# heimrih/polar_code

Hardware: AMD Instinct MI355X
Metric: decoded frames/sec, P(128,64)+CRC24 SCL L=8 @ Eb/N0=5 dB; FER match (higher is better)
Workload: dtype f64

## Files before the change

include/polar_scl.h:

```cpp
#ifndef POLAR_SCL_H
#define POLAR_SCL_H

#include <stdint.h>

#ifdef __cplusplus
extern "C" {
#endif

#define PSCL_ABI_VERSION 1

#define PSCL_OK 0
#define PSCL_EINVAL -1
#define PSCL_EDEVICE -2
#define PSCL_ENOMEM -3
#define PSCL_EPRUNED -4
#define PSCL_EUNSUP -5

#define PSCL_MAX_N 1024
#define PSCL_MAX_L 32
#define PSCL_MAX_CRC 32
#define PSCL_WORDS(K) (((K) + 63) / 64)

#define PSCL_FLAG_CRC_PASS 0x80u
#define PSCL_FLAG_IDX_MASK 0x3fu

#define PSCL_CNT_FRAMES 0
#define PSCL_CNT_FRAME_ERR 1
#define PSCL_CNT_BIT_ERR 2
#define PSCL_CNT_PAYLOAD_ERR 3
#define PSCL_CNT_PAYLOAD_BIT 4
#define PSCL_CNT_RETRIES 5
#define PSCL_CNT_ESCALATED 6
#define PSCL_NCOUNT 8

typedef struct pscl_handle pscl_handle;

const char* pscl_last_error(void);

int pscl_abi_version(void);

const char* pscl_build_hash(void);

int pscl_device_count(void);

int pscl_create(pscl_handle** out, int device, int N, const int32_t* info_set, int K, int L,
                uint64_t crc_poly);
int pscl_destroy(pscl_handle* h);

int pscl_set_stream(pscl_handle* h, void* hip_stream);
void* pscl_get_stream(pscl_handle* h);
int pscl_sync(pscl_handle* h);

int pscl_decode(pscl_handle* h, const double* llr, int64_t B, const int8_t* forced, int32_t* n_paths,
                int8_t* best_bits, uint8_t* crc_pass, int32_t* best_idx, double* metrics, int8_t* cands,
                double* info_llrs);

int pscl_sc_decode(pscl_handle* h, const double* llr, int64_t B, int8_t* bits);

int pscl_decode_device(pscl_handle* h, const double* d_llr, int64_t B, const uint64_t* d_force,
                       uint64_t* d_best, uint8_t* d_flags, double* d_metrics, uint64_t* d_cands,
                       double* d_info_llrs, const uint64_t* d_ref, int k_payload, int64_t* d_counters);

int pscl_channel_device(pscl_handle* h, uint64_t seed, uint32_t stream_id, double ebno_db, double rate,
                        int k_payload, int64_t frame0, int64_t B, double* d_llr, uint64_t* d_msg);

int pscl_uncoded_device(pscl_handle* h, uint64_t seed, uint32_t stream_id, double ebno_db, int k_payload,
                        int64_t frame0, int64_t B, int64_t* d_counters);

int pscl_set_rate_match(pscl_handle* h, int E);

int pscl_path_llrs_device(pscl_handle* h, const double* d_llr, int64_t B, const uint64_t* d_bits, double* d_out);

int pscl_set_beta(pscl_handle* h, const double* beta);

int pscl_dlscl_device(pscl_handle* h, const double* d_llr, int64_t B, int retries, uint64_t* d_best,
                      uint8_t* d_flags, int32_t* d_attempts, int32_t* d_tried, int tried_stride,
                      const uint64_t* d_ref, int k_payload, int64_t* d_counters_scl, int64_t* d_counters_dl);

int pscl_adaptive_device(pscl_handle* h, const double* d_llr, int64_t B, uint64_t* d_best, uint8_t* d_flags,
                         uint8_t* d_stage, const uint64_t* d_ref, int k_payload, int64_t* d_counters,
                         int64_t* n_escalated);

int pscl_sc_device(pscl_handle* h, const double* d_llr, int64_t B, uint64_t* d_best, uint8_t* d_flags,
                   uint8_t* d_stage, const uint64_t* d_ref, int k_payload, int64_t* d_counters);
int pscl_escalate_device(pscl_handle* h, const double* d_llr, int64_t B, uint64_t* d_best, uint8_t* d_flags,
                         uint8_t* d_stage, const uint64_t* d_ref, int k_payload, int64_t* d_counters,
                         int64_t* n_escalated);

int pscl_adaptive_async_device(pscl_handle* h, const double* d_llr, int64_t B, uint64_t* d_best, uint8_t* d_flags,
                               uint8_t* d_stage, const uint64_t* d_ref, int k_payload, int64_t* d_counters,
                               int32_t* d_n_escalated);

int pscl_f32_available(pscl_handle* h);
int pscl_decode_device_f32(pscl_handle* h, const float* d_llr, int64_t B, uint64_t* d_best, uint8_t* d_flags,
                           const uint64_t* d_ref, int k_payload, int64_t* d_counters);
int pscl_sc_device_f32(pscl_handle* h, const float* d_llr, int64_t B, uint64_t* d_best, uint8_t* d_flags,
                       uint8_t* d_stage, const uint64_t* d_ref, int k_payload, int64_t* d_counters);
int pscl_escalate_device_f32(pscl_handle* h, const float* d_llr, int64_t B, uint64_t* d_best, uint8_t* d_flags,
                             uint8_t* d_stage, const uint64_t* d_ref, int k_payload, int64_t* d_counters,
                             int64_t* n_escalated);
int pscl_adaptive_async_device_f32(pscl_handle* h, const float* d_llr, int64_t B, uint64_t* d_best, uint8_t* d_flags,
                                   uint8_t* d_stage, const uint64_t* d_ref, int k_payload, int64_t* d_counters,
                                   int32_t* d_n_escalated);

int pscl_simulate_adaptive_device(pscl_handle* h, uint64_t seed, uint32_t stream_id, double ebno_db, double rate,
                                  int k_payload, int64_t frame0, int64_t B, int include_uncoded, int64_t* d_counters);
int pscl_simulate_adaptive(pscl_handle* h, uint64_t seed, uint32_t stream_id, double ebno_db, double rate,
                           int k_payload, int64_t frame0, int64_t B, int include_uncoded, int64_t* counters);

int pscl_adaptive_stats(pscl_handle* h, int64_t* screened, int64_t* exact, int64_t* host_waits, int reset);

int pscl_retry_device(pscl_handle* h, const double* d_llr, int64_t B, int retries, uint64_t* d_best, uint8_t* d_flags,
                      uint8_t* d_stage, int32_t* d_attempts, int32_t* d_tried, int tried_stride, const uint64_t* d_ref,
                      int k_payload, int64_t* d_counters_dl);

int pscl_adaptive_dlscl_device(pscl_handle* h, const double* d_llr, int64_t B, int retries, uint64_t* d_best,
                               uint8_t* d_flags, uint8_t* d_stage, int32_t* d_attempts, int32_t* d_tried,
                               int tried_stride, const uint64_t* d_ref, int k_payload, int64_t* d_counters,
                               int32_t* d_n_escalated);

int pscl_simulate_adaptive_dl_device(pscl_handle* h, uint64_t seed, uint32_t stream_id, double ebno_db, double rate,
                                     int k_payload, int64_t frame0, int64_t B, int retries, int include_uncoded,
                                     int64_t* d_counters);
int pscl_simulate_adaptive_dl(pscl_handle* h, uint64_t seed, uint32_t stream_id, double ebno_db, double rate,
                              int k_payload, int64_t frame0, int64_t B, int retries, int include_uncoded,
                              int64_t* counters);

int pscl_simulate(pscl_handle* h, uint64_t seed, uint32_t stream_id, double ebno_db, double rate, int k_payload,
                  int64_t frame0, int64_t B, int retries, int include_uncoded, int64_t* counters);

int pscl_simulate_device(pscl_handle* h, uint64_t seed, uint32_t stream_id, double ebno_db, double rate, int k_payload,
                         int64_t frame0, int64_t B, int retries, int include_uncoded, int64_t* d_counters);

int pscl_device_alloc(pscl_handle* h, void** d_ptr, int64_t bytes);
int pscl_device_free(pscl_handle* h, void* d_ptr);
int pscl_memcpy_htod(pscl_handle* h, void* d_dst, const void* src, int64_t bytes);
int pscl_memcpy_dtoh(pscl_handle* h, void* dst, const void* d_src, int64_t bytes);
int pscl_memset_device(pscl_handle* h, void* d_dst, int value, int64_t bytes);

int pscl_set_screening(pscl_handle* h, int enable);

int pscl_screening_count(pscl_handle* h, int64_t* count);

int pscl_set_pipelined(pscl_handle* h, int enable);
int pscl_join(pscl_handle* h);

#define PSCL_TUNE_DL_SCREEN 1
#define PSCL_TUNE_DL_CHUNKS 2
#define PSCL_TUNE_DL_SPLIT 3
#define PSCL_TUNE_SIDE_PRIORITY 4
#define PSCL_TUNE_POST_GRID 5
#define PSCL_TUNE_RETRY_WPG 6
#define PSCL_TUNE_DL_LANE 7
#define PSCL_TUNE_DL_SCREEN_MIN 8
#define PSCL_TUNE_DL_RETRY_LANE 9
#define PSCL_TUNE_POST_PAIRS 10
#define PSCL_TUNE_DL_STREAMS 11
#define PSCL_TUNE_TX_FUSED 12
#define PSCL_TUNE_DL_FUSED_POST 13
#define PSCL_TUNE_POST_EPW 14
#define PSCL_TUNE_LANE_EXACT 15
#define PSCL_TUNE_DL_WARM_APX 16
#define PSCL_TUNE_DL_TAIL 17
#define PSCL_TUNE_ADAPT_GRID 18
#define PSCL_TUNE_COUNT 19
int pscl_set_tuning(pscl_handle* h, int knob, int64_t value);

int pscl_softplus_tails_device(pscl_handle* h, const double* d_v, int64_t n, double* d_exact, double* d_apx);

int pscl_tail_abs_scan_device(pscl_handle* h, uint32_t lo, uint32_t hi, uint64_t* d_out);

int pscl_tail2_scan_device(pscl_handle* h, uint32_t lo, uint32_t hi, uint64_t* d_out);

int pscl_timing_enable(pscl_handle* h, int enable);
int pscl_timing_read(pscl_handle* h, int64_t* launches, double* total_ms);
int pscl_timing_read_split(pscl_handle* h, int64_t* main_launches, double* main_ms, int64_t* side_launches,
                           double* side_ms);

int pscl_host_stats(pscl_handle* h, double* call_ms, double* wait_ms, int64_t* calls, int reset);

int pscl_path_stats(pscl_handle* h, int64_t* fused_post_rounds, int64_t* post_rounds, int64_t* fused_tx_blocks,
                    int64_t* post_epw4_launches, int64_t* lane_exact_launches);

int pscl_decode_cpu(int N, const int32_t* info_set, int K, int L, uint64_t crc_poly, const double* llr, int64_t B,
                    const int8_t* forced, int32_t* n_paths, int8_t* best_bits, uint8_t* crc_pass, int32_t* best_idx,
                    double* metrics, int8_t* cands, double* info_llrs, int threads);

int pscl_decode_adaptive_cpu(int N, const int32_t* info_set, int K, int L, uint64_t crc_poly, const double* llr,
                             int64_t B, int8_t* best_bits, uint8_t* crc_pass, int32_t* best_idx, uint8_t* stage,
                             int threads);

int pscl_launch_info(pscl_handle* h, int64_t B, int* waves_per_wg, int64_t* grid, int* lds_bytes);

#ifdef __cplusplus
}
#endif

#endif
```

polar_code_amd/_native.py:

```python
from __future__ import annotations

import ctypes as C
import functools
import importlib.util
import os
import sys
import threading
from pathlib import Path

import numpy as np

LIB_PATH = Path(os.environ.get("PSCL_LIB_PATH") or Path(__file__).resolve().parent / "libpolar_mi355x.so")

PSCL_OK = 0
PSCL_EINVAL = -1
PSCL_EDEVICE = -2
PSCL_ENOMEM = -3
PSCL_EPRUNED = -4
PSCL_EUNSUP = -5
PSCL_MAX_N = 1024
PSCL_REPLAY_MAX_N = 128
PSCL_MAX_L = 32
PSCL_FLAG_CRC_PASS = 0x80
PSCL_FLAG_IDX_MASK = 0x3F
PSCL_NCOUNT = 8
CNT_FRAMES, CNT_FRAME_ERR, CNT_BIT_ERR, CNT_PAYLOAD_ERR, CNT_PAYLOAD_BIT, CNT_RETRIES, CNT_ESCALATED = range(7)

EXPORTS = (
    "pscl_last_error", "pscl_abi_version", "pscl_device_count", "pscl_create", "pscl_destroy",
    "pscl_set_stream", "pscl_get_stream", "pscl_sync", "pscl_decode", "pscl_sc_decode",
    "pscl_decode_device", "pscl_channel_device", "pscl_device_alloc", "pscl_device_free",
    "pscl_memcpy_htod", "pscl_memcpy_dtoh", "pscl_memset_device", "pscl_timing_enable",
    "pscl_timing_read", "pscl_launch_info", "pscl_set_rate_match", "pscl_set_beta", "pscl_dlscl_device",
    "pscl_path_llrs_device", "pscl_uncoded_device", "pscl_simulate", "pscl_set_screening", "pscl_build_hash",
    "pscl_screening_count", "pscl_softplus_tails_device", "pscl_set_pipelined", "pscl_join",
    "pscl_tail_abs_scan_device", "pscl_tail2_scan_device", "pscl_set_tuning", "pscl_timing_read_split", "pscl_decode_cpu",
    "pscl_host_stats", "pscl_path_stats",
    "pscl_simulate_device", "pscl_adaptive_device", "pscl_decode_adaptive_cpu",
    "pscl_sc_device", "pscl_escalate_device",
    "pscl_adaptive_async_device", "pscl_simulate_adaptive", "pscl_simulate_adaptive_device", "pscl_adaptive_stats",
    "pscl_retry_device", "pscl_adaptive_dlscl_device", "pscl_simulate_adaptive_dl", "pscl_simulate_adaptive_dl_device",
    "pscl_f32_available", "pscl_decode_device_f32", "pscl_sc_device_f32", "pscl_escalate_device_f32",
    "pscl_adaptive_async_device_f32",
)

TUNE = {"dl_screen": 1, "dl_chunks": 2, "dl_split": 3, "side_priority": 4, "post_grid": 5, "retry_wpg": 6, "dl_lane": 7, "dl_screen_min": 8, "dl_retry_lane": 9, "post_pairs": 10, "dl_streams": 11, "tx_fused": 12,
        "dl_fused_post": 13, "post_epw": 14, "lane_exact": 15, "dl_warm_apx": 16, "dl_tail": 17, "adapt_grid": 18}

_vp, _i32, _i64, _u64, _dbl = C.c_void_p, C.c_int32, C.c_int64, C.c_uint64, C.c_double


class PolarNativeError(RuntimeError):
    """Device/runtime failure inside libpolar_mi355x.so."""


def _bind_hip_runtime() -> None:
    if os.environ.get("PSCL_HIP_RUNTIME", "") == "system" or "torch" in sys.modules:
        return
    spec = importlib.util.find_spec("torch")
    if spec is None or not spec.origin:
        return
    cand = Path(spec.origin).parent / "lib" / "libamdhip64.so"
    if cand.exists():
        C.CDLL(str(cand), mode=C.RTLD_GLOBAL)


def _check_fresh() -> None:
    from . import build

    if not all((build.CSRC / s).exists() for s in build.HIP_DEPS):
        return
    want, got = build.source_hash(), build.library_hash(LIB_PATH)
    if got != want:
        raise PolarNativeError(
            f"{LIB_PATH} is stale (built from sources {got}, tree has {want}): "
            "run `python -m polar_code_amd.build`")


@functools.lru_cache(maxsize=1)
def lib() -> C.CDLL:
    _bind_hip_runtime()
    if not LIB_PATH.exists():
        raise PolarNativeError(
            f"{LIB_PATH} not built: run `python -m polar_code_amd.build` (hipcc, gfx950). "
            "There is no CPU fallback for the decoder.")
    if not os.environ.get("PSCL_LIB_PATH"):
        _check_fresh()
    L = C.CDLL(str(LIB_PATH))
    P = C.POINTER
    sig = {
        "pscl_last_error": (C.c_char_p, []),
        "pscl_abi_version": (C.c_int, []),
        "pscl_build_hash": (C.c_char_p, []),
        "pscl_screening_count": (C.c_int, [_vp, P(_i64)]),
        "pscl_set_pipelined": (C.c_int, [_vp, C.c_int]),
        "pscl_join": (C.c_int, [_vp]),
        "pscl_softplus_tails_device": (C.c_int, [_vp, _vp, _i64, _vp, _vp]),
        "pscl_tail_abs_scan_device": (C.c_int, [_vp, C.c_uint32, C.c_uint32, _vp]),
        "pscl_tail2_scan_device": (C.c_int, [_vp, C.c_uint32, C.c_uint32, _vp]),
        "pscl_set_tuning": (C.c_int, [_vp, C.c_int, _i64]),
        "pscl_simulate_device": (C.c_int, [_vp, _u64, C.c_uint32, _dbl, _dbl, C.c_int, _i64, _i64, C.c_int, C.c_int,
                                           _vp]),
        "pscl_decode_cpu": (C.c_int, [C.c_int, P(_i32), C.c_int, C.c_int, _u64, _vp, _i64, _vp, _vp, _vp, _vp, _vp, _vp,
                                      _vp, _vp, C.c_int]),
        "pscl_adaptive_device": (C.c_int, [_vp, _vp, _i64, _vp, _vp, _vp, _vp, C.c_int, _vp, P(_i64)]),
        "pscl_sc_device": (C.c_int, [_vp, _vp, _i64, _vp, _vp, _vp, _vp, C.c_int, _vp]),
        "pscl_escalate_device": (C.c_int, [_vp, _vp, _i64, _vp, _vp, _vp, _vp, C.c_int, _vp, P(_i64)]),
        "pscl_decode_adaptive_cpu": (C.c_int, [C.c_int, P(_i32), C.c_int, C.c_int, _u64, _vp, _i64, _vp, _vp, _vp, _vp,
                                               C.c_int]),
        "pscl_adaptive_async_device": (C.c_int, [_vp, _vp, _i64, _vp, _vp, _vp, _vp, C.c_int, _vp, _vp]),
        "pscl_f32_available": (C.c_int, [_vp]),
        "pscl_decode_device_f32": (C.c_int, [_vp, _vp, _i64, _vp, _vp, _vp, C.c_int, _vp]),
        "pscl_sc_device_f32": (C.c_int, [_vp, _vp, _i64, _vp, _vp, _vp, _vp, C.c_int, _vp]),
        "pscl_escalate_device_f32": (C.c_int, [_vp, _vp, _i64, _vp, _vp, _vp, _vp, C.c_int, _vp, P(_i64)]),
        "pscl_adaptive_async_device_f32": (C.c_int, [_vp, _vp, _i64, _vp, _vp, _vp, _vp, C.c_int, _vp, _vp]),
        "pscl_simulate_adaptive_device": (C.c_int, [_vp, _u64, C.c_uint32, _dbl, _dbl, C.c_int, _i64, _i64, C.c_int, _vp]),
        "pscl_simulate_adaptive": (C.c_int, [_vp, _u64, C.c_uint32, _dbl, _dbl, C.c_int, _i64, _i64, C.c_int, _vp]),
        "pscl_adaptive_stats": (C.c_int, [_vp, P(_i64), P(_i64), P(_i64), C.c_int]),
        "pscl_retry_device": (C.c_int, [_vp, _vp, _i64, C.c_int, _vp, _vp, _vp, _vp, _vp, C.c_int, _vp, C.c_int, _vp]),
        "pscl_adaptive_dlscl_device": (C.c_int, [_vp, _vp, _i64, C.c_int, _vp, _vp, _vp, _vp, _vp, C.c_int, _vp, C.c_int,
                                                 _vp, _vp]),
        "pscl_simulate_adaptive_dl_device": (C.c_int, [_vp, _u64, C.c_uint32, _dbl, _dbl, C.c_int, _i64, _i64, C.c_int,
                                                       C.c_int, _vp]),
        "pscl_simulate_adaptive_dl": (C.c_int, [_vp, _u64, C.c_uint32, _dbl, _dbl, C.c_int, _i64, _i64, C.c_int, C.c_int,
                                                _vp]),
        "pscl_timing_read_split": (C.c_int, [_vp, P(_i64), P(_dbl), P(_i64), P(_dbl)]),
        "pscl_host_stats": (C.c_int, [_vp, P(_dbl), P(_dbl), P(_i64), C.c_int]),
        "pscl_path_stats": (C.c_int, [_vp, P(_i64), P(_i64), P(_i64), P(_i64), P(_i64)]),
        "pscl_device_count": (C.c_int, []),
        "pscl_create": (C.c_int, [P(_vp), C.c_int, C.c_int, P(_i32), C.c_int, C.c_int, _u64]),
        "pscl_destroy": (C.c_int, [_vp]),
        "pscl_set_stream": (C.c_int, [_vp, _vp]),
        "pscl_get_stream": (_vp, [_vp]),
        "pscl_sync": (C.c_int, [_vp]),
        "pscl_decode": (C.c_int, [_vp, _vp, _i64, _vp, _vp, _vp, _vp, _vp, _vp, _vp, _vp]),
        "pscl_sc_decode": (C.c_int, [_vp, _vp, _i64, _vp]),
        "pscl_decode_device": (C.c_int, [_vp, _vp, _i64, _vp, _vp, _vp, _vp, _vp, _vp, _vp, C.c_int, _vp]),
        "pscl_channel_device": (C.c_int, [_vp, _u64, C.c_uint32, _dbl, _dbl, C.c_int, _i64, _i64, _vp, _vp]),
        "pscl_device_alloc": (C.c_int, [_vp, P(_vp), _i64]),
        "pscl_device_free": (C.c_int, [_vp, _vp]),
        "pscl_memcpy_htod": (C.c_int, [_vp, _vp, _vp, _i64]),
        "pscl_memcpy_dtoh": (C.c_int, [_vp, _vp, _vp, _i64]),
        "pscl_memset_device": (C.c_int, [_vp, _vp, C.c_int, _i64]),
        "pscl_timing_enable": (C.c_int, [_vp, C.c_int]),
        "pscl_set_screening": (C.c_int, [_vp, C.c_int]),
        "pscl_timing_read": (C.c_int, [_vp, P(_i64), P(_dbl)]),
        "pscl_launch_info": (C.c_int, [_vp, _i64, P(C.c_int), P(_i64), P(C.c_int)]),
        "pscl_set_rate_match": (C.c_int, [_vp, C.c_int]),
        "pscl_set_beta": (C.c_int, [_vp, _vp]),
        "pscl_path_llrs_device": (C.c_int, [_vp, _vp, _i64, _vp, _vp]),
        "pscl_uncoded_device": (C.c_int, [_vp, _u64, C.c_uint32, _dbl, C.c_int, _i64, _i64, _vp]),
        "pscl_simulate": (C.c_int, [_vp, _u64, C.c_uint32, _dbl, _dbl, C.c_int, _i64, _i64, C.c_int, C.c_int, _vp]),
        "pscl_dlscl_device": (C.c_int, [_vp, _vp, _i64, C.c_int, _vp, _vp, _vp, _vp, C.c_int, _vp, C.c_int, _vp,
                                        _vp]),
    }
    for name, (res, args) in sig.items():
        if os.environ.get("PSCL_LIB_PATH") and not hasattr(L, name):
            continue
        fn = getattr(L, name)
        fn.restype = res
        fn.argtypes = args
    return L


def build_hash() -> str:
    fn = getattr(lib(), "pscl_build_hash", None)
    return fn().decode() if fn is not None else ""


def last_error() -> str:
    return lib().pscl_last_error().decode(errors="replace")


def check(rc: int) -> None:
    if rc == PSCL_OK:
        return
    msg = last_error()
    if rc == PSCL_EINVAL:
        raise ValueError(msg)
    if rc == PSCL_EPRUNED:
        raise RuntimeError("All paths pruned during decoding")
    if rc == PSCL_EUNSUP:
        raise NotImplementedError(msg)
    raise PolarNativeError(f"libpolar_mi355x error {rc}: {msg}")


def device_count() -> int:
    n = lib().pscl_device_count()
    if n < 0:
        raise PolarNativeError(last_error())
    return n


def _ptr(a: np.ndarray | None):
    return None if a is None else a.ctypes.data


def poly_value(crc) -> int:
    if crc is None:
        return 0
    if isinstance(crc, (int, np.integer)):
        return int(crc)
    if not crc:
        raise ValueError("CRC polynomial string must be non-empty")
    return int(str(crc), 16)


class Decoder:

    def __init__(self, N: int, info_set, L: int, crc=None, device: int = 0):
        info = np.ascontiguousarray(np.asarray(info_set).astype(np.int32).ravel())
        self.N, self.K, self.L = int(N), int(info.size), int(L)
        self.info_set = info
        self.crc_poly = poly_value(crc)
        self.crc_deg = max(self.crc_poly.bit_length() - 1, 0)
        self.W = (self.K + 63) // 64 if self.K else 1
        self.device = int(device)
        h = _vp()
        check(lib().pscl_create(C.byref(h), self.device, self.N, info.ctypes.data_as(C.POINTER(_i32)), self.K,
                                self.L, self.crc_poly))
        self._hraw = h
        self._lock = threading.Lock()
        self.E = 0
        self._beta = None

    def set_rate_match(self, E: int) -> None:
        check(lib().pscl_set_rate_match(self._h, int(E)))
        self.E = int(E)

    @property
    def _h(self):
        h = getattr(self, "_hraw", None)
        if h is None:
            raise RuntimeError("Decoder is closed (close(), or release_decoders() on a get_decoder() handle)")
        return h

    @property
    def handle(self):
        return self._h

    @property
    def closed(self) -> bool:
        return getattr(self, "_hraw", None) is None

    def close(self) -> None:
        if getattr(self, "_hraw", None):
            lib().pscl_destroy(self._hraw)
            self._hraw = None

    def __del__(self):
        try:
            self.close()
        except Exception:
            pass

    def decode(self, llr: np.ndarray, forced: np.ndarray | None = None, *, want_metrics=True,
               want_cands=True, want_info_llrs=True):
        llr = np.ascontiguousarray(llr, dtype=np.float64)
        if llr.ndim == 1:
            llr = llr[None, :]
        B = llr.shape[0]
        if llr.shape[1] != (self.E or self.N):
            raise ValueError("Channel LLR length must be a power of two" if not self.E
                             else f"expected {self.E} rate-matched LLRs per frame")
        if forced is not None:
            forced = np.ascontiguousarray(forced, dtype=np.int8).reshape(B, self.K)
        out = {
            "n_paths": np.zeros(B, np.int32),
            "best_bits": np.zeros((B, self.K), np.int8),
            "crc_pass": np.zeros(B, np.uint8),
            "best_idx": np.zeros(B, np.int32),
            "metrics": np.full((B, self.L), np.nan) if want_metrics else None,
            "cands": np.zeros((B, self.L, self.K), np.int8) if want_cands else None,
            "info_llrs": np.full((B, self.L, self.K), np.nan) if want_info_llrs else None,
        }
        with self._lock:
            check(lib().pscl_decode(self._h, _ptr(llr), B, _ptr(forced), _ptr(out["n_paths"]),
                                    _ptr(out["best_bits"]), _ptr(out["crc_pass"]), _ptr(out["best_idx"]),
                                    _ptr(out["metrics"]), _ptr(out["cands"]), _ptr(out["info_llrs"])))
        out["crc_pass"] = out["crc_pass"].astype(bool)
        return out

    def sc_decode(self, llr: np.ndarray) -> np.ndarray:
        llr = np.ascontiguousarray(llr, dtype=np.float64)
        if llr.ndim == 1:
            llr = llr[None, :]
        bits = np.zeros((llr.shape[0], self.K), np.int8)
        with self._lock:
            check(lib().pscl_sc_decode(self._h, _ptr(llr), llr.shape[0], _ptr(bits)))
        return bits

    def set_stream(self, stream_ptr: int | None) -> None:
        check(lib().pscl_set_stream(self._h, stream_ptr))

    def decode_device(self, d_llr: int, B: int, *, d_force=0, d_best=0, d_flags=0, d_metrics=0, d_cands=0,
                      d_info_llrs=0, d_ref=0, k_payload=0, d_counters=0) -> None:
        check(lib().pscl_decode_device(self._h, d_llr, B, d_force or None, d_best or None, d_flags or None,
                                       d_metrics or None, d_cands or None, d_info_llrs or None, d_ref or None,
                                       int(k_payload), d_counters or None))

# ... 128 lines not shown
            d_flags = mem.alloc(max(B, 8))
            d_stage = mem.alloc(max(B, 8))
            if B:
                mem.upload(d_llr, llr)
            self.sc_device(d_llr, B, d_best=d_best, d_flags=d_flags, d_stage=d_stage)
            if escalate:
                n = self.escalate_device(d_llr, B, d_best=d_best, d_flags=d_flags, d_stage=d_stage)
            words = mem.download(d_best, max(B * self.W * 8, 8), np.uint64)[:B * self.W].reshape(B, self.W)
            flags = mem.download(d_flags, max(B, 8), np.uint8)[:B]
            stage = mem.download(d_stage, max(B, 8), np.uint8)[:B]
        j = np.arange(self.K)
        bits = ((words[:, j >> 6] >> (j & 63).astype(np.uint64)) & np.uint64(1)).astype(np.int8)
        return {"best_bits": bits, "crc_pass": (flags & PSCL_FLAG_CRC_PASS) != 0,
                "best_idx": (flags & PSCL_FLAG_IDX_MASK).astype(np.int32), "stage": stage.copy(), "n_escalated": n}

    def decode_sc(self, llr: np.ndarray):
        out = self._staged_host(llr, escalate=False)
        return out["best_bits"], out["crc_pass"]

    def decode_staged(self, llr: np.ndarray) -> dict:
        return self._staged_host(llr, escalate=True)

    def channel_device(self, seed: int, stream_id: int, ebno_db: float, rate: float, k_payload: int, frame0: int,
                       B: int, d_llr: int, d_msg: int = 0) -> None:
        check(lib().pscl_channel_device(self._h, int(seed) & (2**64 - 1), int(stream_id) & 0xFFFFFFFF,
                                        float(ebno_db), float(rate), int(k_payload), int(frame0), int(B), d_llr,
                                        d_msg or None))

    def path_llrs_device(self, d_llr: int, B: int, d_bits: int, d_out: int) -> None:
        with self._lock:
            check(lib().pscl_path_llrs_device(self._h, d_llr, int(B), d_bits, d_out))

    def path_llrs(self, llr: np.ndarray, bits: np.ndarray) -> np.ndarray:
        llr = np.ascontiguousarray(llr, dtype=np.float64)
        if llr.ndim == 1:
            llr = llr[None, :]
        B = llr.shape[0]
        words = np.zeros((B, self.W), np.uint64)
        bits = np.asarray(bits, dtype=np.uint64).reshape(B, self.K)
        for j in range(self.K):
            words[:, j >> 6] |= bits[:, j] << np.uint64(j & 63)
        with DeviceArena(self) as mem:
            d_llr = mem.alloc(llr.nbytes)
            d_bits = mem.alloc(words.nbytes)
            d_out = mem.alloc(max(B * self.K * 8, 8))
            mem.upload(d_llr, llr)
            mem.upload(d_bits, words)
            self.path_llrs_device(d_llr, B, d_bits, d_out)
            return mem.download(d_out, B * self.K * 8, np.float64).reshape(B, self.K)

    def set_beta(self, beta: np.ndarray | None) -> None:
        if beta is None:
            if self._beta is not None:
                check(lib().pscl_set_beta(self._h, None))
            self._beta = None
            return
        b = np.asarray(beta)
        if b.ndim != 2 or b.shape[0] != b.shape[1] or b.shape[0] != self.K:
            raise ValueError("beta must be a square matrix matching abs_l0 length")
        b = np.ascontiguousarray(b, dtype=np.float64)
        if self._beta is not None and np.array_equal(self._beta, b):
            return
        check(lib().pscl_set_beta(self._h, _ptr(b)))
        self._beta = b.copy()

    def dlscl_device(self, d_llr: int, B: int, retries: int, *, beta=None, d_best: int, d_flags: int,
                     d_attempts=0, d_tried=0, tried_stride=0, d_ref=0, k_payload=0, d_counters_scl=0,
                     d_counters_dl=0) -> None:
        self.set_beta(beta)
        with self._lock:
            check(lib().pscl_dlscl_device(self._h, d_llr, int(B), int(retries), d_best, d_flags, d_attempts or None,
                                          d_tried or None, int(tried_stride), d_ref or None, int(k_payload),
                                          d_counters_scl or None, d_counters_dl or None))

    def retry_device(self, d_llr: int, B: int, retries: int, *, beta=None, d_best: int, d_flags: int, d_stage=0,
                     d_attempts=0, d_tried=0, tried_stride=0, d_ref=0, k_payload=0, d_counters_dl=0) -> None:
        self.set_beta(beta)
        with self._lock:
            check(lib().pscl_retry_device(self._h, d_llr or None, int(B), int(retries), d_best or None, d_flags or None,
                                          d_stage or None, d_attempts or None, d_tried or None, int(tried_stride),
                                          d_ref or None, int(k_payload), d_counters_dl or None))

    def adaptive_dlscl_device(self, d_llr: int, B: int, retries: int, *, beta=None, d_best: int, d_flags: int,
                              d_stage=0, d_attempts=0, d_tried=0, tried_stride=0, d_ref=0, k_payload=0, d_counters=0,
                              d_n_escalated=0) -> None:
        self.set_beta(beta)
        with self._lock:
            check(lib().pscl_adaptive_dlscl_device(self._h, d_llr or None, int(B), int(retries), d_best or None,
                                                   d_flags or None, d_stage or None, d_attempts or None, d_tried or None,
                                                   int(tried_stride), d_ref or None, int(k_payload), d_counters or None,
                                                   d_n_escalated or None))

    def uncoded_device(self, seed: int, stream_id: int, ebno_db: float, k_payload: int, frame0: int, B: int,
                       d_counters: int) -> None:
        check(lib().pscl_uncoded_device(self._h, int(seed) & (2**64 - 1), int(stream_id) & 0xFFFFFFFF,
                                        float(ebno_db), int(k_payload), int(frame0), int(B), d_counters))

    def sync(self) -> None:
        check(lib().pscl_sync(self._h))

    def simulate(self, seed: int, stream_id: int, ebno_db: float, rate: float, k_payload: int, frame0: int, B: int,
                 retries: int, include_uncoded: bool = False) -> np.ndarray:
        out = np.zeros((3, PSCL_NCOUNT), np.int64)
        with self._lock:
            check(lib().pscl_simulate(self._h, int(seed) & (2**64 - 1), int(stream_id) & 0xFFFFFFFF, float(ebno_db),
                                      float(rate), int(k_payload), int(frame0), int(B), int(retries),
                                      int(bool(include_uncoded)), out.ctypes.data))
        return out

    def simulate_device(self, seed: int, stream_id: int, ebno_db: float, rate: float, k_payload: int, frame0: int,
                        B: int, retries: int, include_uncoded: bool, d_counters: int) -> None:
        with self._lock:
            check(lib().pscl_simulate_device(self._h, int(seed) & (2**64 - 1), int(stream_id) & 0xFFFFFFFF,
                                             float(ebno_db), float(rate), int(k_payload), int(frame0), int(B),
                                             int(retries), int(bool(include_uncoded)), d_counters))

    def simulate_adaptive(self, seed: int, stream_id: int, ebno_db: float, rate: float, k_payload: int, frame0: int,
                          B: int, include_uncoded: bool = False) -> np.ndarray:
        out = np.zeros((3, PSCL_NCOUNT), np.int64)
        with self._lock:
            check(lib().pscl_simulate_adaptive(self._h, int(seed) & (2**64 - 1), int(stream_id) & 0xFFFFFFFF,
                                               float(ebno_db), float(rate), int(k_payload), int(frame0), int(B),
                                               int(bool(include_uncoded)), out.ctypes.data))
        return out

    def simulate_adaptive_device(self, seed: int, stream_id: int, ebno_db: float, rate: float, k_payload: int,
                                 frame0: int, B: int, include_uncoded: bool, d_counters: int) -> None:
        with self._lock:
            check(lib().pscl_simulate_adaptive_device(self._h, int(seed) & (2**64 - 1), int(stream_id) & 0xFFFFFFFF,
                                                      float(ebno_db), float(rate), int(k_payload), int(frame0), int(B),
                                                      int(bool(include_uncoded)), d_counters or None))

    def simulate_adaptive_dl(self, seed: int, stream_id: int, ebno_db: float, rate: float, k_payload: int, frame0: int,
                             B: int, retries: int, include_uncoded: bool = False) -> np.ndarray:
        out = np.zeros((4, PSCL_NCOUNT), np.int64)
        with self._lock:
            check(lib().pscl_simulate_adaptive_dl(self._h, int(seed) & (2**64 - 1), int(stream_id) & 0xFFFFFFFF,
                                                  float(ebno_db), float(rate), int(k_payload), int(frame0), int(B),
                                                  int(retries), int(bool(include_uncoded)), out.ctypes.data))
        return out

    def simulate_adaptive_dl_device(self, seed: int, stream_id: int, ebno_db: float, rate: float, k_payload: int,
                                    frame0: int, B: int, retries: int, include_uncoded: bool, d_counters: int) -> None:
        with self._lock:
            check(lib().pscl_simulate_adaptive_dl_device(self._h, int(seed) & (2**64 - 1), int(stream_id) & 0xFFFFFFFF,
                                                         float(ebno_db), float(rate), int(k_payload), int(frame0), int(B),
                                                         int(retries), int(bool(include_uncoded)), d_counters or None))

    def screening_count(self) -> int:
        n = _i64()
        check(lib().pscl_screening_count(self._h, C.byref(n)))
        return int(n.value)

    def softplus_tails(self, v: np.ndarray):
        v = np.ascontiguousarray(v, dtype=np.float64).ravel()
        with DeviceArena(self) as mem:
            d_v, d_e, d_a = mem.alloc(v.nbytes), mem.alloc(v.nbytes), mem.alloc(v.nbytes)
            mem.upload(d_v, v)
            check(lib().pscl_softplus_tails_device(self._h, d_v, v.size, d_e, d_a))
            return mem.download(d_e, v.nbytes, np.float64), mem.download(d_a, v.nbytes, np.float64)

    def tail_abs_scan(self, lo: int = 0, hi: int = 0x7F800000, bits: bool = False):
        fn = lib().pscl_tail2_scan_device if bits else lib().pscl_tail_abs_scan_device
        with DeviceArena(self) as mem:
            d = mem.alloc(16)
            mem.memset(d, 0, 16)
            check(fn(self._h, int(lo), int(hi), d))
            out = mem.download(d, 16, np.uint64)
        err = float(out[:1].view(np.float64)[0])
        x32 = float(np.array([int(out[1]) & 0xFFFFFFFF], np.uint32).view(np.float32)[0])
        return err, x32

    def set_pipelined(self, on: bool = True, depth: int = 2) -> None:
        if not 1 <= int(depth) <= 4:
            raise ValueError(f"pipelined depth must be 1..4 (got {depth})")
        check(lib().pscl_set_pipelined(self._h, (int(depth) if depth > 2 else 1) if on else 0))

    def join(self) -> None:
        check(lib().pscl_join(self._h))

    def set_tuning(self, **knobs) -> None:
        for k, v in knobs.items():
            if k not in TUNE:
                raise ValueError(f"unknown tuning knob {k!r}")
            check(lib().pscl_set_tuning(self._h, TUNE[k], int(v)))
            tun = self.__dict__.setdefault("_tuning", {})
            tun[k] = int(v)

    def get_tuning(self) -> dict:
        return dict(self.__dict__.get("_tuning", {}))

    def set_screening(self, on: bool = True) -> None:
        check(lib().pscl_set_screening(self._h, 1 if on else 0))

    def timing_enable(self, on: bool = True) -> None:
        check(lib().pscl_timing_enable(self._h, 1 if on else 0))

    def timing_read(self):
        n, ms = _i64(), _dbl()
        check(lib().pscl_timing_read(self._h, C.byref(n), C.byref(ms)))
        return int(n.value), float(ms.value)

    def timing_read_split(self):
        n0, t0, n1, t1 = _i64(), _dbl(), _i64(), _dbl()
        check(lib().pscl_timing_read_split(self._h, C.byref(n0), C.byref(t0), C.byref(n1), C.byref(t1)))
        return (int(n0.value), float(t0.value)), (int(n1.value), float(t1.value))

    def host_stats(self, reset: bool = False):
        c, w, n = _dbl(), _dbl(), _i64()
        check(lib().pscl_host_stats(self._h, C.byref(c), C.byref(w), C.byref(n), 1 if reset else 0))
        return float(c.value), float(w.value), int(n.value)

    def path_stats(self) -> dict:
        a, b, c, d, x = _i64(), _i64(), _i64(), _i64(), _i64()
        check(lib().pscl_path_stats(self._h, C.byref(a), C.byref(b), C.byref(c), C.byref(d), C.byref(x)))
        return {"fused_post_rounds": int(a.value), "post_rounds": int(b.value), "fused_tx_blocks": int(c.value),
                "post_epw4_launches": int(d.value), "lane_exact_launches": int(x.value)}

    def launch_info(self, B: int):
        w, g, lds = C.c_int(), _i64(), C.c_int()
        check(lib().pscl_launch_info(self._h, int(B), C.byref(w), C.byref(g), C.byref(lds)))
        return int(w.value), int(g.value), int(lds.value)


class CpuDecoder:

    def __init__(self, N: int, info_set, L: int, crc=None, threads: int = 0):
        info = np.ascontiguousarray(np.asarray(info_set).astype(np.int32).ravel())
        self.N, self.K, self.L = int(N), int(info.size), int(L)
        self.info_set = info
        self.crc_poly = poly_value(crc)
        self.crc_deg = max(self.crc_poly.bit_length() - 1, 0)
        self.W = (self.K + 63) // 64 if self.K else 1
        self.E = 0
        self.device = "cpu"
        self.threads = int(threads or os.environ.get("PSCL_CPU_THREADS", "0") or 0)
        if self.N < 2 or self.N & (self.N - 1) or self.N > PSCL_MAX_N:
            raise ValueError("Channel LLR length must be a power of two")
        if self.crc_poly and self.K <= self.crc_deg:
            raise ValueError("Message too short for the provided CRC polynomial")

    def decode(self, llr: np.ndarray, forced: np.ndarray | None = None, *, want_metrics=True,
               want_cands=True, want_info_llrs=True):
        llr = np.ascontiguousarray(llr, dtype=np.float64)
        if llr.ndim == 1:
            llr = llr[None, :]
        B = llr.shape[0]
        if llr.shape[1] != self.N:
            raise ValueError("Channel LLR length must be a power of two")
        if forced is not None:
            forced = np.ascontiguousarray(forced, dtype=np.int8).reshape(B, self.K)
            if np.any((forced < -1) | (forced > 1)):
                raise ValueError("force_info_bits entries must be -1, 0, or 1")
        out = {
            "n_paths": np.zeros(B, np.int32),
            "best_bits": np.zeros((B, self.K), np.int8),
            "crc_pass": np.zeros(B, np.uint8),
            "best_idx": np.zeros(B, np.int32),
            "metrics": np.full((B, self.L), np.nan) if want_metrics else None,
            "cands": np.zeros((B, self.L, self.K), np.int8) if want_cands else None,
            "info_llrs": np.full((B, self.L, self.K), np.nan) if want_info_llrs else None,
        }
        check(lib().pscl_decode_cpu(self.N, self.info_set.ctypes.data_as(C.POINTER(_i32)), self.K, self.L,
                                    self.crc_poly, _ptr(llr), B, _ptr(forced), _ptr(out["n_paths"]),
                                    _ptr(out["best_bits"]), _ptr(out["crc_pass"]), _ptr(out["best_idx"]),
                                    _ptr(out["metrics"]), _ptr(out["cands"]), _ptr(out["info_llrs"]), self.threads))
        out["crc_pass"] = out["crc_pass"].astype(bool)
        return out

    def decode_adaptive(self, llr: np.ndarray) -> dict:
        llr = np.ascontiguousarray(llr, dtype=np.float64)
        if llr.ndim == 1:
            llr = llr[None, :]
        B = llr.shape[0]
        if llr.shape[1] != self.N:
            raise ValueError("Channel LLR length must be a power of two")
        bits = np.zeros((B, self.K), np.int8)
        ok, idx, stage = np.zeros(B, np.uint8), np.zeros(B, np.int32), np.zeros(B, np.uint8)
        check(lib().pscl_decode_adaptive_cpu(self.N, self.info_set.ctypes.data_as(C.POINTER(_i32)), self.K, self.L,
                                             self.crc_poly, _ptr(llr), B, _ptr(bits), _ptr(ok), _ptr(idx), _ptr(stage),
                                             self.threads))
        return {"best_bits": bits, "crc_pass": ok.astype(bool), "best_idx": idx, "stage": stage,
                "n_escalated": int(np.count_nonzero(stage == 2))}

    def sync(self) -> None:
        pass

    def close(self) -> None:
        pass


_CACHE: dict = {}
_CACHE_LOCK = threading.Lock()


def get_decoder(N: int, info_set, L: int, crc=None, device: int = 0, E: int = 0, slot: int = 0) -> Decoder:
    info = np.asarray(info_set).astype(np.int64).ravel()
    cpu = isinstance(device, str) and device == "cpu"
    key = (int(N), info.tobytes(), int(L), poly_value(crc), "cpu" if cpu else int(device), int(E), int(slot))
    with _CACHE_LOCK:
        dec = _CACHE.get(key)
        if dec is None:
            if len(_CACHE) > 64:
                _CACHE.clear()
            if cpu:
                if E:
                    raise NotImplementedError("the CPU decoder takes internal (de-rate-matched) LLRs")
                dec = _CACHE[key] = CpuDecoder(N, info, L, crc)
                return dec
            dec = Decoder(N, info, L, crc, device)
            if E:
                dec.set_rate_match(E)
            _CACHE[key] = dec
        return dec


def release_decoders() -> None:
    with _CACHE_LOCK:
        decs = list(_CACHE.values())
        _CACHE.clear()
    for d in decs:
        d.close()


class DeviceArena:

    def __init__(self, dec: Decoder):
        self.dec = dec
        self.ptrs: list[int] = []

    def __enter__(self) -> "DeviceArena":
        return self

    def __exit__(self, *exc) -> None:
        self.dec.sync()
        for p in self.ptrs:
            lib().pscl_device_free(self.dec.handle, p)
        self.ptrs.clear()

    def alloc(self, nbytes: int) -> int:
        p = _vp()
        check(lib().pscl_device_alloc(self.dec.handle, C.byref(p), int(nbytes)))
        self.ptrs.append(p.value)
        return p.value

    def memset(self, d_ptr: int, value: int, nbytes: int) -> None:
        check(lib().pscl_memset_device(self.dec.handle, d_ptr, int(value), int(nbytes)))

    def upload(self, d_ptr: int, arr: np.ndarray) -> None:
        arr = np.ascontiguousarray(arr)
        check(lib().pscl_memcpy_htod(self.dec.handle, d_ptr, arr.ctypes.data, arr.nbytes))

    def download(self, d_ptr: int, nbytes: int, dtype) -> np.ndarray:
        out = np.empty(int(nbytes) // np.dtype(dtype).itemsize, dtype=dtype)
        check(lib().pscl_memcpy_dtoh(self.dec.handle, out.ctypes.data, d_ptr, out.nbytes))
        return out
```

polar_code_amd/csrc/capi.cpp:

```cpp
#include <hip/hip_runtime.h>
#include <math.h>

#include <cmath>
#include <stdarg.h>
#include <stdint.h>
#include <stdio.h>
#include <stdlib.h>
#include <string.h>

#include <chrono>
#include <string>
#include <utility>
#include <vector>

#include "polar_scl.h"
#include "scl_kernels.h"

namespace {

thread_local std::string g_err;

int fail(int code, const char* fmt, ...) {
    char buf[512];
    va_list ap;
    va_start(ap, fmt);
    vsnprintf(buf, sizeof(buf), fmt, ap);
    va_end(ap);
    g_err = buf;
    return code;
}

#define HIP_TRY(expr)                                                                     \
    do {                                                                                  \
        hipError_t _e = (expr);                                                           \
        if (_e != hipSuccess)                                                             \
            return fail(_e == hipErrorOutOfMemory ? PSCL_ENOMEM : PSCL_EDEVICE, "%s: %s", \
                        #expr, hipGetErrorString(_e));                                    \
    } while (0)

#ifndef PSCL_BUILD_HASH
#define PSCL_BUILD_HASH "unhashed"
#endif
__attribute__((used)) const char kBuildHash[] = "PSCL_BUILD_HASH=" PSCL_BUILD_HASH;

const uint64_t kExpTable[256] = {
#include "exp_table.inc"
};

int poly_degree(uint64_t poly) {
    int len = 0;
    for (uint64_t v = poly; v; v >>= 1) len++;
    return len - 1;
}

uint32_t crc_remainder(const std::vector<uint8_t>& in, uint64_t poly, int deg) {
    std::vector<uint8_t> buf(in);
    const int len = (int)buf.size();
    for (int i = 0; i + deg < len; ++i) {
        if (!buf[i]) continue;
        for (int k = 0; k <= deg; ++k) buf[i + k] ^= (uint8_t)((poly >> (deg - k)) & 1);
    }
    uint32_t r = 0;
    for (int i = 0; i < deg; ++i)
        if (buf[len - deg + i]) r |= 1u << i;
    return r;
}

struct DevBuf {
    void* p = nullptr;
    size_t n = 0;
};

}

struct pscl_dl_call {
    const double* d_llr = nullptr;
    int64_t B = 0;
    int rounds = 0;
    uint64_t* d_best = nullptr;
    uint8_t* d_flags = nullptr;
    int32_t* d_attempts = nullptr;
    int32_t* d_tried = nullptr;
    int tried_stride = 0;
    const uint64_t* d_ref = nullptr;
    int k_payload = 0;
    int64_t* d_counters_dl = nullptr;
    int64_t nch = 1, cap = 0;
    int nsplit = 2, pbase = 0;
    bool pipe = false;
    int mode = 0;
    uint8_t* d_stage = nullptr;
};

constexpr int kDlPar = 4;
constexpr int kChainSets = 2, kChainStreams = 2 * kChainSets;

struct pscl_handle {
    int device = 0;
    int N = 0, n = 0, K = 0, L = 0, W = 1, crc_deg = 0;
    uint64_t crc_poly = 0;
    uint64_t info_mask[2] = {0, 0};
    std::vector<uint64_t> info_words;
    uint64_t* d_info_words = nullptr;
    std::vector<int32_t> info_set;
    std::vector<uint32_t> check_cols;
    std::vector<uint32_t> attach_cols;
    hipStream_t own_stream = nullptr;
    hipStream_t stream = nullptr;
    uint32_t* d_check_cols = nullptr;
    uint32_t* d_attach_cols = nullptr;
    int32_t* d_info_set = nullptr;
    uint64_t* d_exp_table = nullptr;
    int rm_E = 0;
    int32_t* d_rm_src = nullptr;
    int32_t* d_rm_order = nullptr;
    DevBuf scratch[160];
    hipStream_t retry_stream[kChainStreams] = {};
    hipStream_t side_stream[kChainStreams] = {};
    hipStream_t stash_pipe = nullptr, stash_retry[kChainStreams] = {}, stash_side[kChainStreams] = {};
    hipEvent_t ev_scr[kChainStreams] = {}, ev_def[kChainStreams] = {};
    hipEvent_t ev_base[kDlPar] = {}, ev_retry[kDlPar] = {}, ev_join[kChainSets] = {};
    int32_t* h_count = nullptr;
    int32_t* h_adapt = nullptr;
    double* d_beta = nullptr;
    float* d_beta32g[2] = {nullptr, nullptr};
    std::vector<float> beta32g_host;
    double beta_absmax = 0.0;
    std::vector<double> beta_host;
    uint64_t* d_epi = nullptr;
    uint64_t* d_xtab = nullptr;
    uint32_t* d_crctab = nullptr;
    int epi_words = 0;
    bool timing = false;
    bool screen = true;
    bool screened = false;
    int screened_slot = 36;
    bool pipelined = false;
    hipStream_t pipe_stream = nullptr;
    hipEvent_t ev_pscr[2] = {nullptr, nullptr}, ev_px[2] = {nullptr, nullptr};
    bool px_pending[2] = {false, false};
    int pipe_par = 0;
    hipStream_t tail_stream = nullptr;
    hipEvent_t ev_tscr[2] = {nullptr, nullptr}, ev_tail[2] = {nullptr, nullptr};
    bool tail_pending[2] = {false, false};
    hipEvent_t ev_dl[kDlPar] = {};
    bool dl_pending[kDlPar] = {};
    int dl_par = 0;
    int dl_back = 2;
    pscl_dl_call dl_defer;
    int dl_last_mode = 0;
    bool dl_defer_valid = false;
    std::vector<hipEvent_t> ev_pool;
    std::vector<uint8_t> ev_main;
    size_t ev_used = 0;
    int64_t tune[PSCL_TUNE_COUNT] = {};
    double host_call_ms = 0.0, host_wait_ms = 0.0;
    int64_t host_calls = 0;
    int64_t n_fpost_rounds = 0, n_post_rounds = 0, n_fused_tx = 0, n_post_epw4 = 0, n_lane_exact = 0;
    hipStream_t ad_stream = nullptr;
    hipEvent_t ev_adc[2] = {nullptr, nullptr}, ev_ad[2] = {nullptr, nullptr};
    bool ad_pending[2] = {false, false};
    int ad_par = 0;
    int64_t n_regrow = 0;
    int64_t n_ad_screened = 0, n_ad_exact = 0, n_ad_waits = 0;
};

namespace {

void quiesce(pscl_handle* h);

int ensure(pscl_handle* h, int slot, size_t bytes, void** out) {
    DevBuf& b = h->scratch[slot];
    if (b.n < bytes) {
        if (b.p) {
            quiesce(h);
            hipFree(b.p);
            h->n_regrow++;
        }
        b.p = nullptr;
        b.n = 0;
        size_t want = bytes + bytes / 2;
        if (want < 4096) want = 4096;
        HIP_TRY(hipMalloc(&b.p, want));
        b.n = want;
    }
    *out = b.p;
    return PSCL_OK;
}

int set_device(pscl_handle* h) {
    HIP_TRY(hipSetDevice(h->device));
    return PSCL_OK;
}

int dl_enqueue_deferred(pscl_handle* h, bool beside = false);

int join_pipe(pscl_handle* h, int what = 3) {
    if (what & 2) {
        const int rc = dl_enqueue_deferred(h);
        if (rc) return rc;
    }
    for (int p = 0; p < 2; ++p)
        if ((what & 2) && h->tail_pending[p]) {
            HIP_TRY(hipStreamWaitEvent(h->stream, h->ev_tail[p], 0));
            h->tail_pending[p] = false;
        }
    for (int p = 0; p < 2; ++p)
        if ((what & 1) && !(what & 8) && h->ad_pending[p]) {
            HIP_TRY(hipStreamWaitEvent(h->stream, h->ev_ad[p], 0));
            h->ad_pending[p] = false;
        }
    for (int p = 0; p < kDlPar; ++p) {
        if ((what & 1) && p < 2 && h->px_pending[p]) {
            HIP_TRY(hipStreamWaitEvent(h->stream, h->ev_px[p], 0));
            h->px_pending[p] = false;
        }
        if ((what & 2) && h->dl_pending[p]) {
            HIP_TRY(hipStreamWaitEvent(h->stream, h->ev_dl[p], 0));
            h->dl_pending[p] = false;
        }
    }
    return PSCL_OK;
}

void quiesce(pscl_handle* h) {
    if (h->pipe_stream) hipStreamSynchronize(h->pipe_stream);
    if (h->tail_stream) hipStreamSynchronize(h->tail_stream);
    if (h->ad_stream) hipStreamSynchronize(h->ad_stream);
    for (int i = 0; i < kChainStreams; ++i) {
        if (h->retry_stream[i]) hipStreamSynchronize(h->retry_stream[i]);
        if (h->side_stream[i]) hipStreamSynchronize(h->side_stream[i]);
    }
}

void drop_side_streams(pscl_handle* h) {
    quiesce(h);
    if (h->stash_pipe) hipStreamDestroy(h->stash_pipe);
    h->stash_pipe = nullptr;
    for (int i = 0; i < kChainStreams; ++i) {
        if (h->stash_retry[i]) hipStreamDestroy(h->stash_retry[i]);
        if (h->stash_side[i]) hipStreamDestroy(h->stash_side[i]);
        h->stash_retry[i] = h->stash_side[i] = nullptr;
    }
    if (h->pipe_stream) hipStreamDestroy(h->pipe_stream);
    h->pipe_stream = nullptr;
    if (h->tail_stream) hipStreamDestroy(h->tail_stream);
    h->tail_stream = nullptr;
    if (h->ad_stream) hipStreamDestroy(h->ad_stream);
    h->ad_stream = nullptr;
    for (int i = 0; i < kChainStreams; ++i) {
        if (h->retry_stream[i]) hipStreamDestroy(h->retry_stream[i]);
        if (h->side_stream[i]) hipStreamDestroy(h->side_stream[i]);
        h->retry_stream[i] = h->side_stream[i] = nullptr;
    }
}

hipError_t create_priority_stream(pscl_handle* h, hipStream_t* s) {
    int least = 0, greatest = 0;
    if (hipDeviceGetStreamPriorityRange(&least, &greatest) != hipSuccess) greatest = least = 0;
    const bool plain = h->tune[PSCL_TUNE_SIDE_PRIORITY] == 1;
    return hipStreamCreateWithPriority(s, hipStreamNonBlocking, h->pipelined && !plain ? greatest : least);
}

int enter(pscl_handle* h) {
    const int rc = set_device(h);
    return rc ? rc : join_pipe(h);
}

void fill_decode_params(const pscl_handle* h, pscl_decode_params& P, int hist) {
    memset(&P, 0, sizeof(P));
    P.N = h->N;
    P.n = h->n;
    P.K = h->K;
    P.L = h->L;
    P.W = h->W;
    P.info_mask[0] = h->info_mask[0];
    P.info_mask[1] = h->info_mask[1];
    P.info_words = h->d_info_words;
    P.crc_cols = h->d_check_cols;
    P.info_set = h->d_info_set;
    P.has_crc = h->crc_poly != 0;
    P.exp_table = h->d_exp_table;
    P.epi_table = h->d_epi;
    P.epi_words = h->epi_words;
    P.rm_E = h->rm_E;
    P.rm_src = h->d_rm_src;
    pscl_decode_layout(P, hist);
}

int with_count_slots(pscl_handle* h, pscl_decode_params& P, int hist, int slot, hipStream_t st) {
    P.cpart = nullptr;
    const int64_t slots = pscl_decode_count_slots(P, hist);
    if (slots <= 0) return PSCL_OK;
    void* d;
    const size_t had = h->scratch[slot].n;
    const int rc = ensure(h, slot, (size_t)slots * 16, &d);
    if (rc) return rc;
    if (h->scratch[slot].n != had) HIP_TRY(hipMemsetAsync(d, 0, h->scratch[slot].n, st));
    P.cpart = (int32_t*)d;
    return PSCL_OK;
}

#ifndef PSCL_LANE_EXACT_DEFAULT
#define PSCL_LANE_EXACT_DEFAULT 0
#endif
bool lane_exact_on(const pscl_handle* h) {
    const int64_t lx = h->tune[PSCL_TUNE_LANE_EXACT];
    return lx == 1 || lx == 3 || (lx == 0 && PSCL_LANE_EXACT_DEFAULT);
}

const char* f32_unsupported(const pscl_handle* h) {
    if (h->N != PSCL_FAST_N) return "float32 rows are decoded at N = 128 only";
    if (h->L != 4 && h->L != 8) return "float32 rows are decoded at L = 4 and 8 only";
    if (!h->screen) return "float32 rows need the screening decode (pscl_set_screening is off)";
    if (h->tune[PSCL_TUNE_LANE_EXACT] == 3 || lane_exact_on(h))
        return "PSCL_TUNE_LANE_EXACT selects the exact lane-per-path instance, which has no float32 form";
    pscl_decode_params P;
    fill_decode_params(h, P, 0);
    if (!pscl_f32_decode_available(P))
        return h->rm_E ? "float32 rate-matched rows are decoded for the compiled-in (128,88) code only"
                       : "float32 plain rows are decoded for the compiled-in (128,64) code only (runtime information set)";
    return nullptr;
}

int launch_decode(pscl_handle* h, const pscl_decode_params& P0, int hist, hipStream_t st = nullptr, int scr_slot = 38,
                  bool pipe = false, hipStream_t tail = nullptr, int tail_par = 0) {
    if (!st) st = h->stream;
    pscl_decode_params P = P0;
    if (P.long_mode) {
        void* d_scr;
        const int rc = ensure(h, scr_slot, (size_t)pscl_decode_grid(P) * (size_t)P.long_block_bytes, &d_scr);
        if (rc) return rc;
        P.long_scratch = (unsigned char*)d_scr;
    }
    hipEvent_t e0 = nullptr, e1 = nullptr;
    if (h->timing) {
        while (h->ev_pool.size() < h->ev_used + 2) {
            hipEvent_t e;
            HIP_TRY(hipEventCreate(&e));
            h->ev_pool.push_back(e);
        }
        e0 = h->ev_pool[h->ev_used];
        e1 = h->ev_pool[h->ev_used + 1];
        if (h->ev_main.size() < h->ev_pool.size() / 2) h->ev_main.resize(h->ev_pool.size() / 2);
        h->ev_main[h->ev_used / 2] = st == h->stream ? 1 : 0;
        h->ev_used += 2;
        HIP_TRY(hipEventRecord(e0, st));
    }
    pscl_decode_params T = P;
    T.apx = 1;
    const int64_t lx = h->tune[PSCL_TUNE_LANE_EXACT];
    const bool screen = h->screen && lx != 3 && !hist && !P.metrics && !P.cands && !P.force && !P.sc_hard && !P.fidx &&
                        !P.d_count &&
                        (P.fast ? (pscl_screening_available(P) != 0 || pscl_lane_long128_available(T) != 0)
                                : pscl_lane_long_available(T) != 0);
    hipError_t err;
    if (!(screen && pipe)) {
        const int rc = join_pipe(h, 1);
        if (rc) return rc;
    }
    if (screen) {
        void *d_cnt, *d_list;
        int rc;
        const int p = pipe ? h->pipe_par : 0;
        const bool tl = tail && !pipe;
        const int s_cnt = tl ? (tail_par ? 126 : 124) : (p ? 64 : 36), s_list = tl ? (tail_par ? 127 : 125) : (p ? 65 : 37);
        if (tl && h->tail_pending[tail_par]) {
            if (h->scratch[s_list].n < (size_t)P.B * 8) HIP_TRY(hipEventSynchronize(h->ev_tail[tail_par]));
            HIP_TRY(hipStreamWaitEvent(st, h->ev_tail[tail_par], 0));
            h->tail_pending[tail_par] = false;
        }
        if (pipe) {
            if (!h->pipe_stream) HIP_TRY(create_priority_stream(h, &h->pipe_stream));
            if (!h->ev_pscr[0]) {
                for (int i = 0; i < 2; ++i) {
                    HIP_TRY(hipEventCreateWithFlags(&h->ev_pscr[i], hipEventDisableTiming));
                    HIP_TRY(hipEventCreateWithFlags(&h->ev_px[i], hipEventDisableTiming));
                }
            }
            if (h->px_pending[p]) {
                if (h->scratch[s_list].n < (size_t)P.B * 8) HIP_TRY(hipEventSynchronize(h->ev_px[p]));
                HIP_TRY(hipStreamWaitEvent(st, h->ev_px[p], 0));
                h->px_pending[p] = false;
            }
            h->pipe_par ^= 1;
        }
        if ((rc = ensure(h, s_cnt, 4, &d_cnt))) return rc;
        if ((rc = ensure(h, s_list, (size_t)P.B * 8, &d_list))) return rc;
        HIP_TRY(hipMemsetAsync(d_cnt, 0, 4, st));
        pscl_decode_params S = P;
        S.apx = 1;
        pscl_decode_layout(S, hist);
        S.amb_list = (int64_t*)d_list;
        S.amb_count = (int32_t*)d_cnt;
        if ((rc = with_count_slots(h, S, hist, tl ? 70 + tail_par : (pipe ? 92 + p : 92), st))) return rc;
        S.tx_upart = nullptr;
        if (S.tx && S.tx_unc_counters) {
            const int64_t slots = pscl_decode_count_slots(S, hist);
            void* du;
            const size_t had = h->scratch[94].n;
            if ((rc = ensure(h, 94, (size_t)(slots > 0 ? slots : 1) * 16, &du))) return rc;
            if (h->scratch[94].n != had) HIP_TRY(hipMemsetAsync(du, 0, h->scratch[94].n, st));
            S.tx_upart = (int32_t*)du;
        }
        err = pscl_launch_decode(S, hist, st);
        if (err == hipSuccess && S.tx_upart)
            err = pscl_launch_count_reduce(S.tx_upart, pscl_decode_count_slots(S, hist), S.tx_unc_counters, st);
        if (err == hipSuccess && S.tx)
            err = pscl_launch_tx_rows(S, (const int64_t*)d_list, (const int32_t*)d_cnt, S.B, S.tx_rows, S.tx_frame0, st);
        h->screened = true;
        h->screened_slot = s_cnt;
#ifdef PSCL_APX_ABLATE
        static const bool screen_only = getenv("PSCL_DIAG_SCREEN_ONLY") && atoi(getenv("PSCL_DIAG_SCREEN_ONLY")) == 1;
#else
        constexpr bool screen_only = false;
#endif
        if (err == hipSuccess && S.cpart && ((!pipe && !tl) || screen_only))
            err = pscl_launch_count_reduce(S.cpart, pscl_decode_count_slots(S, hist), S.counters, st);
        if (err == hipSuccess && !screen_only) {
            pscl_decode_params X = P;
            X.tx = 0;
            X.fidx = (const int64_t*)d_list;
            X.d_count = (const int32_t*)d_cnt;
            X.out_by_row = 1;
            X.lane_exact = lane_exact_on(h) ? 1 : 0;
            X.grid_cap = (int64_t)256 * 16 / (pscl_decode_wpg(X) > 0 ? pscl_decode_wpg(X) : 1);
            if (tl) {
                if (h->timing) HIP_TRY(hipEventRecord(e1, st));
                HIP_TRY(hipEventRecord(h->ev_tscr[tail_par], st));
                HIP_TRY(hipStreamWaitEvent(tail, h->ev_tscr[tail_par], 0));
                if (!hist && pscl_lane_exact_available(X)) h->n_lane_exact++;
                err = pscl_launch_decode(X, hist, tail);
                if (err == hipSuccess && S.cpart)
                    err = pscl_launch_count_reduce(S.cpart, pscl_decode_count_slots(S, hist), S.counters, tail);
                if (err != hipSuccess) return fail(PSCL_EDEVICE, "decode kernel launch: %s", hipGetErrorString(err));
                return PSCL_OK;
            }
            if (pipe) {
                if (h->timing) HIP_TRY(hipEventRecord(e1, st));
                HIP_TRY(hipEventRecord(h->ev_pscr[p], st));
                HIP_TRY(hipStreamWaitEvent(h->pipe_stream, h->ev_pscr[p], 0));
                if (!hist && pscl_lane_exact_available(X)) h->n_lane_exact++;
                err = pscl_launch_decode(X, hist, h->pipe_stream);
                if (err == hipSuccess && S.cpart)
                    err = pscl_launch_count_reduce(S.cpart, pscl_decode_count_slots(S, hist), S.counters, h->pipe_stream);
                if (err != hipSuccess) return fail(PSCL_EDEVICE, "decode kernel launch: %s", hipGetErrorString(err));
                HIP_TRY(hipEventRecord(h->ev_px[p], h->pipe_stream));
                h->px_pending[p] = true;
                return PSCL_OK;
            }
            if (!hist && pscl_lane_exact_available(X)) h->n_lane_exact++;
            err = pscl_launch_decode(X, hist, st);
        }
    } else {
        if (lx == 3) P.lane_exact = 1;
        const int rc = with_count_slots(h, P, hist, 92, st);
        if (rc) return rc;
        if (!hist && pscl_lane_exact_available(P)) h->n_lane_exact++;
        err = pscl_launch_decode(P, hist, st);
        if (err == hipSuccess && P.cpart) err = pscl_launch_count_reduce(P.cpart, pscl_decode_count_slots(P, hist), P.counters, st);
        if (err == hipSuccess && tail && !pipe) {
            HIP_TRY(hipEventRecord(h->ev_tscr[tail_par], st));
            HIP_TRY(hipStreamWaitEvent(tail, h->ev_tscr[tail_par], 0));
        }
    }
    if (err != hipSuccess) return fail(PSCL_EDEVICE, "decode kernel launch: %s", hipGetErrorString(err));
    if (h->timing) HIP_TRY(hipEventRecord(e1, st));
    return PSCL_OK;
}

}

extern "C" {

const char* pscl_last_error(void) { return g_err.c_str(); }

int pscl_abi_version(void) { return PSCL_ABI_VERSION; }

const char* pscl_build_hash(void) { return kBuildHash + 16; }

int pscl_device_count(void) {
    int n = 0;
    hipError_t e = hipGetDeviceCount(&n);
    if (e == hipErrorNoDevice) return 0;
    if (e != hipSuccess) return fail(PSCL_EDEVICE, "hipGetDeviceCount: %s", hipGetErrorString(e));
    return n;
}

int pscl_create(pscl_handle** out, int device, int N, const int32_t* info_set, int K, int L, uint64_t crc_poly) {
    if (!out) return fail(PSCL_EINVAL, "out is NULL");
    *out = nullptr;
    if (N <= 1 || (N & (N - 1))) return fail(PSCL_EINVAL, "Channel LLR length must be a power of two");
    if (N > PSCL_MAX_N) return fail(PSCL_EUNSUP, "N=%d exceeds PSCL_MAX_N=%d", N, PSCL_MAX_N);
    if (L <= 0) return fail(PSCL_EINVAL, "List size M must be positive");
    if (L > PSCL_MAX_L) return fail(PSCL_EUNSUP, "list size %d exceeds PSCL_MAX_L=%d", L, PSCL_MAX_L);
    if (K < 0 || K > N || (K > 0 && !info_set)) return fail(PSCL_EINVAL, "info_set must hold 0..N indices");
    pscl_handle tmp;
    tmp.N = N;
    while ((1 << tmp.n) < N) tmp.n++;
    tmp.K = K;
    tmp.L = L;
    tmp.W = K > 64 ? (K + 63) / 64 : 1;
    tmp.crc_poly = crc_poly;
    tmp.info_words.assign((size_t)(N >= 64 ? N / 64 : 1), 0ULL);
    for (int i = 0; i < K; ++i) {
        int p = info_set[i];
        if (p < 0 || p >= N) return fail(PSCL_EINVAL, "info_set indices out of range");
        uint64_t bit = 1ULL << (p & 63);
        if (tmp.info_words[(size_t)(p >> 6)] & bit) return fail(PSCL_EUNSUP, "duplicate info_set index %d", p);
        tmp.info_words[(size_t)(p >> 6)] |= bit;
        if (p < PSCL_FAST_N) tmp.info_mask[p >> 6] |= bit;
        tmp.info_set.push_back(p);
    }
    for (int i = 1; i < K; ++i)
        if (tmp.info_set[i] < tmp.info_set[i - 1]) return fail(PSCL_EUNSUP, "info_set must be sorted ascending");
    tmp.check_cols.assign((size_t)(K > 0 ? K : 1), 0u);
    if (crc_poly) {
        tmp.crc_deg = poly_degree(crc_poly);
        if (tmp.crc_deg <= 0) return fail(PSCL_EINVAL, "Polynomial degree must be positive");
        if (tmp.crc_deg > PSCL_MAX_CRC) return fail(PSCL_EUNSUP, "CRC degree %d > %d", tmp.crc_deg, PSCL_MAX_CRC);
        if (K <= tmp.crc_deg) return fail(PSCL_EINVAL, "Message too short for the provided CRC polynomial");
        for (int jj = 0; jj < K; ++jj) {
            std::vector<uint8_t> e((size_t)K, 0);
            e[(size_t)jj] = 1;
            tmp.check_cols[(size_t)jj] = crc_remainder(e, crc_poly, tmp.crc_deg);
        }
        const int kp = K - tmp.crc_deg;
        tmp.attach_cols.assign((size_t)(kp > 0 ? kp : 1), 0u);
        for (int jj = 0; jj < kp; ++jj) {
            std::vector<uint8_t> e((size_t)(kp + tmp.crc_deg), 0);
            e[(size_t)jj] = 1;
            tmp.attach_cols[(size_t)jj] = crc_remainder(e, crc_poly, tmp.crc_deg);
        }
    } else {
        tmp.attach_cols.assign((size_t)(K > 0 ? K : 1), 0u);
    }
    int ndev = 0;
    hipError_t e = hipGetDeviceCount(&ndev);
    if (e != hipSuccess || ndev == 0)
        return fail(PSCL_EDEVICE, "no HIP device available (%s)", e == hipSuccess ? "0 devices" : hipGetErrorString(e));
    if (device < 0 || device >= ndev) return fail(PSCL_EINVAL, "device %d out of range (%d devices)", device, ndev);
    pscl_handle* h = new pscl_handle(tmp);
    h->device = device;
    int rc = set_device(h);
    if (rc) {
        delete h;
        return rc;
    }
#define CREATE_TRY(expr)                                                         \
    do {                                                                         \
        hipError_t _e = (expr);                                                  \
        if (_e != hipSuccess) {                                                  \
            int _c = fail(PSCL_EDEVICE, "%s: %s", #expr, hipGetErrorString(_e)); \
            pscl_destroy(h);                                                     \
            return _c;                                                           \
        }                                                                        \
    } while (0)
    CREATE_TRY(hipStreamCreateWithFlags(&h->own_stream, hipStreamNonBlocking));
    h->stream = h->own_stream;
    CREATE_TRY(hipMalloc(&h->d_check_cols, h->check_cols.size() * 4));
    CREATE_TRY(hipMalloc(&h->d_attach_cols, h->attach_cols.size() * 4));
    CREATE_TRY(hipMalloc(&h->d_info_set, (size_t)(K > 0 ? K : 1) * 4));
    CREATE_TRY(hipMalloc(&h->d_exp_table, sizeof(kExpTable)));
    CREATE_TRY(hipMalloc(&h->d_info_words, h->info_words.size() * 8));
    CREATE_TRY(hipMemcpy(h->d_info_words, h->info_words.data(), h->info_words.size() * 8, hipMemcpyHostToDevice));
    CREATE_TRY(hipMemcpy(h->d_check_cols, h->check_cols.data(), h->check_cols.size() * 4, hipMemcpyHostToDevice));
    CREATE_TRY(hipMemcpy(h->d_attach_cols, h->attach_cols.data(), h->attach_cols.size() * 4, hipMemcpyHostToDevice));
    if (K > 0) CREATE_TRY(hipMemcpy(h->d_info_set, h->info_set.data(), (size_t)K * 4, hipMemcpyHostToDevice));
    CREATE_TRY(hipMemcpy(h->d_exp_table, kExpTable, sizeof(kExpTable), hipMemcpyHostToDevice));
    {
        std::vector<int32_t> order((size_t)N), src((size_t)N);
        const int nb = (N + 31) / 32;
        for (int k = 0; k < N; ++k) order[(size_t)k] = N >= 32 ? (k % 32) * nb + k / 32 : k;
        for (int k = 0; k < N; ++k) src[(size_t)order[(size_t)k]] = k;
        CREATE_TRY(hipMalloc(&h->d_rm_src, (size_t)N * 4));
        CREATE_TRY(hipMalloc(&h->d_rm_order, (size_t)N * 4));
        CREATE_TRY(hipMemcpy(h->d_rm_src, src.data(), (size_t)N * 4, hipMemcpyHostToDevice));
        CREATE_TRY(hipMemcpy(h->d_rm_order, order.data(), (size_t)N * 4, hipMemcpyHostToDevice));
    }
    {
        const int k4 = (K + 3) / 4, nby = N > 128 ? N / 8 : 16;
        std::vector<uint8_t> epi((size_t)nby * 256 + (size_t)k4 * 16 * 4, 0);
        for (int k = 0; k < nby; ++k)
            for (int v = 0; v < 256; ++v) {
                int c = 0, cntb = 0;
                for (int t = 0; t < 8; ++t) {
                    const int p = 8 * k + t;
                    if (p < N && ((h->info_words[p >> 6] >> (p & 63)) & 1ULL)) {
                        if ((v >> t) & 1) c |= 1 << cntb;
                        cntb++;
                    }
                }
                epi[(size_t)k * 256 + v] = (uint8_t)c;
            }
        uint32_t* syn = reinterpret_cast<uint32_t*>(epi.data() + (size_t)nby * 256);
        for (int m = 0; m < k4; ++m)
            for (int v = 0; v < 16; ++v) {
                uint32_t acc = 0;
                for (int t = 0; t < 4; ++t)
                    if (4 * m + t < K && ((v >> t) & 1)) acc ^= h->check_cols[(size_t)(4 * m + t)];
                syn[m * 16 + v] = acc;
// ... 327 lines not shown
namespace {
int sc_device_impl(pscl_handle* h, const double* d_llr, bool f32, int64_t B, uint64_t* d_best, uint8_t* d_flags,
                   uint8_t* d_stage, const uint64_t* d_ref, int k_payload, int64_t* d_counters) {
    if (!h) return fail(PSCL_EINVAL, "NULL handle");
    if (B < 0) return fail(PSCL_EINVAL, "B must be >= 0");
    if (d_ref && !d_counters) return fail(PSCL_EINVAL, "d_ref given without d_counters");
    if (k_payload < 0 || k_payload > h->K) return fail(PSCL_EINVAL, "k_payload out of range");
    if (h->N < 32) return fail(PSCL_EUNSUP, "the SC stage is implemented for N = 32 .. %d (N = %d)", PSCL_MAX_N, h->N);
    if (h->rm_E && h->N != PSCL_FAST_N)
        return fail(PSCL_EUNSUP, "the SC stage takes rate-matched rows at N = %d only (N = %d)", PSCL_FAST_N, h->N);
    if (f32 && h->N != PSCL_FAST_N)
        return fail(PSCL_EUNSUP, "float32 rows: the SC stage takes N = %d only (N = %d)", PSCL_FAST_N, h->N);
    if (B == 0) return PSCL_OK;
    if (!d_llr || !d_best || !d_flags) return fail(PSCL_EINVAL, "d_llr, d_best and d_flags are required");
    int rc = enter(h);
    if (rc) return rc;
    if ((rc = launch_sc_stage(h, d_llr, B, d_best, d_flags, d_stage, f32))) return rc;
    return count_final(h, d_best, d_flags, B, d_ref, k_payload, d_counters, 0);
}
}

int pscl_sc_device(pscl_handle* h, const double* d_llr, int64_t B, uint64_t* d_best, uint8_t* d_flags,
                   uint8_t* d_stage, const uint64_t* d_ref, int k_payload, int64_t* d_counters) {
    return sc_device_impl(h, d_llr, false, B, d_best, d_flags, d_stage, d_ref, k_payload, d_counters);
}

int pscl_sc_device_f32(pscl_handle* h, const float* d_llr, int64_t B, uint64_t* d_best, uint8_t* d_flags,
                       uint8_t* d_stage, const uint64_t* d_ref, int k_payload, int64_t* d_counters) {
    return sc_device_impl(h, (const double*)d_llr, true, B, d_best, d_flags, d_stage, d_ref, k_payload, d_counters);
}

namespace {
int escalate_device_impl(pscl_handle* h, const double* d_llr, bool f32, int64_t B, uint64_t* d_best, uint8_t* d_flags,
                         uint8_t* d_stage, const uint64_t* d_ref, int k_payload, int64_t* d_counters,
                         int64_t* n_escalated) {
    if (!h) return fail(PSCL_EINVAL, "NULL handle");
    if (n_escalated) *n_escalated = 0;
    if (B < 0) return fail(PSCL_EINVAL, "B must be >= 0");
    if (!h->crc_poly) return fail(PSCL_EINVAL, "escalation needs a CRC (without one every SC result passes)");
    if (d_ref && !d_counters) return fail(PSCL_EINVAL, "d_ref given without d_counters");
    if (k_payload < 0 || k_payload > h->K) return fail(PSCL_EINVAL, "k_payload out of range");
    if (B == 0) return PSCL_OK;
    if (!d_llr || !d_best || !d_flags) return fail(PSCL_EINVAL, "d_llr, d_best and d_flags are required");
    if (B > INT32_MAX) return fail(PSCL_EUNSUP, "B exceeds 2^31-1");
    if (f32) {
        if (const char* why = f32_unsupported(h)) return fail(PSCL_EUNSUP, "%s", why);
    }
    int rc = enter(h);
    if (rc) return rc;
    int64_t n = 0;
    if ((rc = escalate_failed(h, d_llr, B, d_best, d_flags, d_stage, &n, f32))) return rc;
    if (n_escalated) *n_escalated = n;
    return count_final(h, d_best, d_flags, B, d_ref, k_payload, d_counters, n);
}
}

int pscl_escalate_device(pscl_handle* h, const double* d_llr, int64_t B, uint64_t* d_best, uint8_t* d_flags,
                         uint8_t* d_stage, const uint64_t* d_ref, int k_payload, int64_t* d_counters,
                         int64_t* n_escalated) {
    return escalate_device_impl(h, d_llr, false, B, d_best, d_flags, d_stage, d_ref, k_payload, d_counters, n_escalated);
}

int pscl_escalate_device_f32(pscl_handle* h, const float* d_llr, int64_t B, uint64_t* d_best, uint8_t* d_flags,
                             uint8_t* d_stage, const uint64_t* d_ref, int k_payload, int64_t* d_counters,
                             int64_t* n_escalated) {
    return escalate_device_impl(h, (const double*)d_llr, true, B, d_best, d_flags, d_stage, d_ref, k_payload, d_counters,
                                n_escalated);
}

namespace {

constexpr int kAdSlot[2] = {128, 132};

int adaptive_begin(pscl_handle* h, bool pipe, int* par) {
    const int q = pipe ? h->ad_par : 0;
    if (pipe) {
        if (!h->pipe_stream) HIP_TRY(create_priority_stream(h, &h->pipe_stream));
        if (!h->ad_stream) HIP_TRY(create_priority_stream(h, &h->ad_stream));
        for (int i = 0; i < 2; ++i) {
            if (!h->ev_adc[i]) HIP_TRY(hipEventCreateWithFlags(&h->ev_adc[i], hipEventDisableTiming));
            if (!h->ev_ad[i]) HIP_TRY(hipEventCreateWithFlags(&h->ev_ad[i], hipEventDisableTiming));
        }
        h->ad_par ^= 1;
    }
    if (h->ad_pending[q]) {
        HIP_TRY(hipStreamWaitEvent(h->stream, h->ev_ad[q], 0));
        h->ad_pending[q] = false;
    }
    *par = q;
    return PSCL_OK;
}

int adaptive_escalate_enqueue(pscl_handle* h, int q, bool pipe, const double* d_llr, int64_t B, uint64_t* d_best,
                              uint8_t* d_flags, const uint64_t* d_ref, int k_payload, int64_t* d_counters,
                              int32_t* d_n_escalated, bool f32 = false) {
    hipStream_t s = h->stream;
    const int base = kAdSlot[q];
    const int64_t regrown = h->n_regrow;
    hipError_t e;
    int rc;
    void *d_cnt, *d_list, *d_amb;
    if ((rc = ensure(h, base, 128, &d_cnt))) return rc;
    if ((rc = ensure(h, base + 1, (size_t)B * 8, &d_list))) return rc;
    if ((rc = ensure(h, base + 2, (size_t)B * 8, &d_amb))) return rc;
    int32_t* const amb_cnt = (int32_t*)d_cnt;
    int32_t* const esc_cnt = amb_cnt + 16;
    pscl_decode_params P;
    fill_decode_params(h, P, 0);
    P.llr = d_llr;
    P.B = B;
    P.best = d_best;
    P.flags = d_flags;
    P.fidx = (const int64_t*)d_list;
    P.d_count = esc_cnt;
    P.out_by_row = 1;
    P.f32 = f32 ? 1 : 0;
    if (pscl_decode_wpg(P) < 1) return fail(PSCL_EUNSUP, "LDS budget exceeded (L=%d, K=%d)", h->L, h->K);
    pscl_decode_params S = P;
    S.apx = 1;
    pscl_decode_layout(S, 0);
    S.amb_list = (int64_t*)d_amb;
    S.amb_count = amb_cnt;
    S.grid_cap = h->tune[PSCL_TUNE_ADAPT_GRID];
    const bool screen = h->screen && h->tune[PSCL_TUNE_LANE_EXACT] != 3 &&
                        (S.long_mode ? pscl_lane_long_available(S) != 0
                                     : (pscl_lane_available(S) != 0 || pscl_lane_long128_available(S) != 0));
    pscl_decode_params X = P;
    X.lane_exact = lane_exact_on(h) ? 1 : 0;
    X.grid_cap = (int64_t)256 * 16 / (pscl_decode_wpg(X) > 0 ? pscl_decode_wpg(X) : 1);
    if (screen) {
        X.fidx = (const int64_t*)d_amb;
        X.d_count = amb_cnt;
    }
    if (X.long_mode) {
        void* d_scr;
        if ((rc = ensure(h, base + 3, (size_t)pscl_decode_grid(X) * (size_t)X.long_block_bytes, &d_scr))) return rc;
        X.long_scratch = (unsigned char*)d_scr;
    }
    h->n_ad_waits += h->n_regrow - regrown;
    HIP_TRY(hipMemsetAsync(d_cnt, 0, 128, s));
    if ((e = pscl_launch_dl_compact(d_flags, B, 0, (int64_t*)d_list, nullptr, esc_cnt, s)) != hipSuccess)
        return fail(PSCL_EDEVICE, "dl_compact launch: %s", hipGetErrorString(e));
    hipStream_t t = s;
    if (pipe) {
        t = q ? h->ad_stream : h->pipe_stream;
        HIP_TRY(hipEventRecord(h->ev_adc[q], s));
        HIP_TRY(hipStreamWaitEvent(t, h->ev_adc[q], 0));
    }
    if (screen) {
        if ((e = pscl_launch_decode(S, 0, t)) != hipSuccess)
            return fail(PSCL_EDEVICE, "row-list decode launch: %s", hipGetErrorString(e));
        h->screened = true;
        h->screened_slot = base;
        h->n_ad_screened++;
    } else {
        h->n_ad_exact++;
    }
    if (pscl_lane_exact_available(X)) h->n_lane_exact++;
    if ((e = pscl_launch_decode(X, 0, t)) != hipSuccess)
        return fail(PSCL_EDEVICE, "decode kernel launch: %s", hipGetErrorString(e));
    if (d_ref && (e = pscl_launch_dl_count(d_best, d_flags, d_ref, B, h->W, k_payload, d_counters, t)) != hipSuccess)
        return fail(PSCL_EDEVICE, "dl_count launch: %s", hipGetErrorString(e));
    if ((d_ref || d_n_escalated) &&
        (e = pscl_launch_publish_count(esc_cnt, d_ref ? d_counters : nullptr, PSCL_CNT_ESCALATED, d_n_escalated, t)) != hipSuccess)
        return fail(PSCL_EDEVICE, "counter launch: %s", hipGetErrorString(e));
    if (pipe) {
        HIP_TRY(hipEventRecord(h->ev_ad[q], t));
        h->ad_pending[q] = true;
    }
    return PSCL_OK;
}

int adaptive_async_args(pscl_handle* h, int64_t B, int k_payload) {
    if (!h) return fail(PSCL_EINVAL, "NULL handle");
    if (B < 0) return fail(PSCL_EINVAL, "B must be >= 0");
    if (!h->crc_poly) return fail(PSCL_EINVAL, "adaptive decoding needs a CRC (without one every SC result passes)");
    if (k_payload < 0 || k_payload > h->K) return fail(PSCL_EINVAL, "k_payload out of range");
    if (h->N < 32) return fail(PSCL_EUNSUP, "the SC stage is implemented for N = 32 .. %d (N = %d)", PSCL_MAX_N, h->N);
    if (h->rm_E && h->N != PSCL_FAST_N)
        return fail(PSCL_EUNSUP, "the SC stage takes rate-matched rows at N = %d only (N = %d)", PSCL_FAST_N, h->N);
    if (B > INT32_MAX) return fail(PSCL_EUNSUP, "B exceeds 2^31-1");
    return PSCL_OK;
}

}

namespace {
int adaptive_async_impl(pscl_handle* h, const double* d_llr, bool f32, int64_t B, uint64_t* d_best, uint8_t* d_flags,
                        uint8_t* d_stage, const uint64_t* d_ref, int k_payload, int64_t* d_counters,
                        int32_t* d_n_escalated) {
    int rc = adaptive_async_args(h, B, k_payload);
    if (rc) return rc;
    if (d_ref && !d_counters) return fail(PSCL_EINVAL, "d_ref given without d_counters");
    if (B > 0 && (!d_llr || !d_best || !d_flags)) return fail(PSCL_EINVAL, "d_llr, d_best and d_flags are required");
    if (f32) {
        if (const char* why = f32_unsupported(h)) return fail(PSCL_EUNSUP, "%s", why);
    }
    const bool pipe = h->pipelined;
    if ((rc = set_device(h)) || (rc = join_pipe(h, pipe ? 3 + 8 : 3))) return rc;
    if (B == 0) {
        if (d_n_escalated) HIP_TRY(hipMemsetAsync(d_n_escalated, 0, 4, h->stream));
        return PSCL_OK;
    }
    int q = 0;
    if ((rc = adaptive_begin(h, pipe, &q))) return rc;
    if ((rc = launch_sc_stage(h, d_llr, B, d_best, d_flags, d_stage, f32))) return rc;
    return adaptive_escalate_enqueue(h, q, pipe, d_llr, B, d_best, d_flags, d_ref, k_payload, d_counters, d_n_escalated, f32);
}
}

int pscl_adaptive_async_device(pscl_handle* h, const double* d_llr, int64_t B, uint64_t* d_best, uint8_t* d_flags,
                               uint8_t* d_stage, const uint64_t* d_ref, int k_payload, int64_t* d_counters,
                               int32_t* d_n_escalated) {
    return adaptive_async_impl(h, d_llr, false, B, d_best, d_flags, d_stage, d_ref, k_payload, d_counters, d_n_escalated);
}

int pscl_adaptive_async_device_f32(pscl_handle* h, const float* d_llr, int64_t B, uint64_t* d_best, uint8_t* d_flags,
                                   uint8_t* d_stage, const uint64_t* d_ref, int k_payload, int64_t* d_counters,
                                   int32_t* d_n_escalated) {
    return adaptive_async_impl(h, (const double*)d_llr, true, B, d_best, d_flags, d_stage, d_ref, k_payload, d_counters,
                               d_n_escalated);
}

int pscl_adaptive_stats(pscl_handle* h, int64_t* screened, int64_t* exact, int64_t* host_waits, int reset) {
    if (!h) return fail(PSCL_EINVAL, "NULL handle");
    if (screened) *screened = h->n_ad_screened;
    if (exact) *exact = h->n_ad_exact;
    if (host_waits) *host_waits = h->n_ad_waits;
    if (reset) h->n_ad_screened = h->n_ad_exact = h->n_ad_waits = 0;
    return PSCL_OK;
}

int pscl_join(pscl_handle* h) {
    if (!h) return fail(PSCL_EINVAL, "NULL handle");
    int rc = set_device(h);
    if (rc) return rc;
    return join_pipe(h);
}

int pscl_set_pipelined(pscl_handle* h, int enable) {
    if (!h) return fail(PSCL_EINVAL, "NULL handle");
    int rc = set_device(h);
    if (rc) return rc;
    if ((rc = join_pipe(h))) return rc;
    if (enable < 0 || enable > kDlPar) return fail(PSCL_EINVAL, "pipelined depth %d out of range 0..%d", enable, kDlPar);
    if (h->pipelined != (enable != 0)) {
        quiesce(h);
        std::swap(h->pipe_stream, h->stash_pipe);
        for (int i = 0; i < kChainStreams; ++i) {
            std::swap(h->retry_stream[i], h->stash_retry[i]);
            std::swap(h->side_stream[i], h->stash_side[i]);
        }
    }
    h->pipelined = enable != 0;
    h->dl_back = enable >= 2 ? enable : 2;
    return PSCL_OK;
}

int pscl_set_tuning(pscl_handle* h, int knob, int64_t value) {
    if (!h) return fail(PSCL_EINVAL, "NULL handle");
    static const int64_t lim[PSCL_TUNE_COUNT][2] = {{0, 0}, {0, 2}, {0, 64}, {0, 2}, {0, 1}, {0, 4096}, {0, PSCL_MAX_WAVES_PER_WG}, {0, 2},
                                                    {0, (int64_t)1 << 30}, {0, 2}, {0, 32}, {0, 3}, {0, 2}, {0, 2}, {0, 4}, {0, 3}, {0, 2}, {0, 1},
                                                    {0, (int64_t)1 << 20}};
    if (knob < 1 || knob >= PSCL_TUNE_COUNT) return fail(PSCL_EINVAL, "unknown tuning knob %d", knob);
    if (value < lim[knob][0] || value > lim[knob][1] || (knob == PSCL_TUNE_POST_GRID && value && value < 16))
        return fail(PSCL_EINVAL, "tuning knob %d: value %lld out of range", knob, (long long)value);
    if (knob == PSCL_TUNE_POST_EPW && value != 0 && value != 2 && value != 4)
        return fail(PSCL_EINVAL, "tuning knob %d: value %lld out of range", knob, (long long)value);
    int rc = set_device(h);
    if (rc) return rc;
    if ((rc = join_pipe(h))) return rc;
    if (knob == PSCL_TUNE_SIDE_PRIORITY && h->tune[knob] != value) drop_side_streams(h);
    h->tune[knob] = value;
    return PSCL_OK;
}

int pscl_path_llrs_device(pscl_handle* h, const double* d_llr, int64_t B, const uint64_t* d_bits, double* d_out) {
    if (!h) return fail(PSCL_EINVAL, "NULL handle");
    if (B < 0) return fail(PSCL_EINVAL, "B must be >= 0");
    if (B == 0) return PSCL_OK;
    if (!d_llr || !d_bits || !d_out) return fail(PSCL_EINVAL, "d_llr, d_bits and d_out are required");
    if (h->N > PSCL_FAST_N) return fail(PSCL_EUNSUP, "decision-LLR replay supports N <= %d", PSCL_FAST_N);
    if (B > INT32_MAX) return fail(PSCL_EUNSUP, "B exceeds 2^31-1");
    int rc = enter(h);
    if (rc) return rc;
    void *d_cnt, *d_rows;
    if ((rc = ensure(h, 25, 8, &d_cnt))) return rc;
    if ((rc = ensure(h, 26, (size_t)B * 8, &d_rows))) return rc;
    const int32_t nb = (int32_t)B;
    HIP_TRY(hipMemcpyAsync(d_cnt, &nb, 4, hipMemcpyHostToDevice, h->stream));
    hipError_t e = pscl_launch_iota64((int64_t*)d_rows, B, h->stream);
    if (e != hipSuccess) return fail(PSCL_EDEVICE, "iota launch: %s", hipGetErrorString(e));
    pscl_replay_params Rp;
    memset(&Rp, 0, sizeof(Rp));
    Rp.llr = d_llr;
    Rp.N = h->N;
    Rp.n = h->n;
    Rp.K = h->K;
    Rp.W = h->W;
    Rp.rm_E = h->rm_E;
    Rp.rm_src = h->d_rm_src;
    Rp.info_mask[0] = h->info_mask[0];
    Rp.info_mask[1] = h->info_mask[1];
    Rp.count = (const int32_t*)d_cnt;
    Rp.act = (const int64_t*)d_rows;
    Rp.bits = d_bits;
    Rp.bits_by_row = 1;
    Rp.out = d_out;
    if ((e = pscl_launch_replay(Rp, B, h->stream)) != hipSuccess)
        return fail(PSCL_EDEVICE, "replay launch: %s", hipGetErrorString(e));
    HIP_TRY(hipStreamSynchronize(h->stream));
    return PSCL_OK;
}

int pscl_set_beta(pscl_handle* h, const double* beta) {
    if (!h) return fail(PSCL_EINVAL, "NULL handle");
    int rc = enter(h);
    if (rc) return rc;
    if (!beta) {
        if (h->d_beta) HIP_TRY(hipFree(h->d_beta));
        h->d_beta = nullptr;
        for (int i = 0; i < 2; ++i) {
            if (h->d_beta32g[i]) HIP_TRY(hipFree(h->d_beta32g[i]));
            h->d_beta32g[i] = nullptr;
        }
        return PSCL_OK;
    }
    if (h->K == 0) return fail(PSCL_EINVAL, "beta must be a square matrix matching abs_l0 length");
    const size_t n = (size_t)h->K * h->K;
    if (!h->d_beta) HIP_TRY(hipMalloc(&h->d_beta, n * 8));
    HIP_TRY(hipStreamSynchronize(h->stream));
    h->beta_host.assign(beta, beta + n);
    HIP_TRY(hipMemcpyAsync(h->d_beta, h->beta_host.data(), n * 8, hipMemcpyHostToDevice, h->stream));
    if (h->K == 64) {
        const int K = h->K;
        h->beta32g_host.assign(2 * n, 0.0f);
        for (int gi = 0; gi < 2; ++gi) {
            const int G = gi ? 4 : 8, NC = K / G;
            for (int k = 0; k < K; ++k)
                for (int pp = 0; pp < G; ++pp)
                    for (int i = 0; i < NC; ++i)
                        h->beta32g_host[(size_t)gi * n + ((size_t)k * G + pp) * NC + i] = (float)beta[(size_t)k * K + pp + G * i];
            if (!h->d_beta32g[gi]) HIP_TRY(hipMalloc(&h->d_beta32g[gi], n * 4));
            HIP_TRY(hipMemcpyAsync(h->d_beta32g[gi], h->beta32g_host.data() + (size_t)gi * n, n * 4, hipMemcpyHostToDevice,
                                   h->stream));
        }
    }
    double mx = 0.0;
    bool nan = false;
    for (size_t i = 0; i < n; ++i) {
        const double a = fabs(beta[i]);
        if (std::isnan(a))
            nan = true;
        else if (a > mx)
            mx = a;
    }
    h->beta_absmax = nan ? INFINITY : mx;
    return PSCL_OK;
}

#ifndef PSCL_DL_FUSED_POST_DEFAULT
#define PSCL_DL_FUSED_POST_DEFAULT 0
#endif
namespace {
struct DlState {
    int64_t* act;
    int32_t* bcnt;
    int32_t *list0, *list1;
    uint64_t *tried, *force, *warm_u, *ob;
    int32_t* nt;
    double* warm_metric;
    uint8_t* of;
    int32_t *dcnt, *dlist;
    uint64_t* ob2;
    uint8_t* of2;
};

#ifndef PSCL_DL_WARM_APX_DEFAULT
#define PSCL_DL_WARM_APX_DEFAULT 1
#endif

hipError_t launch_post(pscl_handle* h, const pscl_post_params& Q, int64_t A, hipStream_t s) {
    if (pscl_post_epw(Q) == 4) h->n_post_epw4++;
    return pscl_launch_dl_post(Q, A, s);
}

int dl_retry_chunk(pscl_handle* h, const DlState& S, int A, int rounds, const double* d_llr, uint64_t* d_best,
                   uint8_t* d_flags, int32_t* d_attempts, int32_t* d_tried, int tried_stride, int64_t* d_cnt_dl,
                   hipStream_t st, hipStream_t side, hipEvent_t ev_s, hipEvent_t ev_d, bool narrow, bool beside) {
    const int K = h->K, W = h->W;
    hipError_t e;
    const size_t bstride = (size_t)PSCL_DL_NSEG * PSCL_DL_CSTRIDE;
    HIP_TRY(hipMemsetAsync(S.bcnt, 0, (size_t)(rounds + 1) * bstride * 4, st));
    pscl_post_params Q;
    memset(&Q, 0, sizeof(Q));
    Q.llr = d_llr;
    Q.N = h->N;
    Q.n = h->n;
    Q.K = K;
    Q.W = W;
    Q.rm_E = h->rm_E;
    Q.rm_src = h->d_rm_src;
    Q.info_mask[0] = h->info_mask[0];
    Q.info_mask[1] = h->info_mask[1];
    Q.info_set = h->d_info_set;
    Q.exp_table = h->d_exp_table;
    Q.rounds = rounds;
    Q.narrow = narrow ? 1 : 0;
    Q.grid_cap = h->tune[PSCL_TUNE_POST_GRID];
    Q.pairs = h->tune[PSCL_TUNE_POST_PAIRS];
    Q.epw = (int)h->tune[PSCL_TUNE_POST_EPW];
    Q.cap = A;
    Q.act = S.act;
    Q.tried = S.tried;
    Q.ntried = S.nt;
    Q.beta = h->d_beta;
// ... 950 lines not shown
    }
    return PSCL_OK;
}
}

int pscl_simulate_adaptive_device(pscl_handle* h, uint64_t seed, uint32_t stream_id, double ebno_db, double rate,
                                  int k_payload, int64_t frame0, int64_t B, int include_uncoded, int64_t* d_counters) {
    int rc = adaptive_async_args(h, B < 0 ? B : 0, k_payload);
    if (rc) return rc;
    if (!d_counters) return fail(PSCL_EINVAL, "d_counters is NULL");
    if (frame0 < 0) return fail(PSCL_EINVAL, "B and frame0 must be >= 0");
    if (B == 0) return PSCL_OK;
    if ((rc = enter(h))) return rc;
    return simulate_adaptive_enqueue(h, seed, stream_id, ebno_db, rate, k_payload, frame0, B, include_uncoded, d_counters);
}

int pscl_simulate_adaptive(pscl_handle* h, uint64_t seed, uint32_t stream_id, double ebno_db, double rate,
                           int k_payload, int64_t frame0, int64_t B, int include_uncoded, int64_t* counters) {
    int rc = adaptive_async_args(h, B < 0 ? B : 0, k_payload);
    if (rc) return rc;
    if (!counters) return fail(PSCL_EINVAL, "counters is NULL");
    if (frame0 < 0) return fail(PSCL_EINVAL, "B and frame0 must be >= 0");
    memset(counters, 0, sizeof(int64_t) * 3 * PSCL_NCOUNT);
    if (B == 0) return PSCL_OK;
    if ((rc = enter(h))) return rc;
    void* d_cnt;
    if ((rc = ensure(h, 140, sizeof(int64_t) * 3 * PSCL_NCOUNT, &d_cnt))) return rc;
    HIP_TRY(hipMemsetAsync(d_cnt, 0, sizeof(int64_t) * 3 * PSCL_NCOUNT, h->stream));
    if ((rc = simulate_adaptive_enqueue(h, seed, stream_id, ebno_db, rate, k_payload, frame0, B, include_uncoded,
                                        (int64_t*)d_cnt)))
        return rc;
    HIP_TRY(hipMemcpyAsync(counters, d_cnt, sizeof(int64_t) * 3 * PSCL_NCOUNT, hipMemcpyDeviceToHost, h->stream));
    HIP_TRY(hipStreamSynchronize(h->stream));
    return PSCL_OK;
}

namespace {
int channel_launch(pscl_handle* h, uint64_t seed, uint32_t stream_id, double ebno_db, double rate, int k_payload,
                   int64_t frame0, int64_t B, double* d_llr, uint64_t* d_msg, int64_t* d_unc, bool no_enter) {
    if (!h) return fail(PSCL_EINVAL, "NULL handle");
    if (B < 0 || frame0 < 0) return fail(PSCL_EINVAL, "B and frame0 must be >= 0");
    if (B == 0) return PSCL_OK;
    if (!d_llr) return fail(PSCL_EINVAL, "d_llr is NULL");
    if (!(rate > 0)) return fail(PSCL_EINVAL, "rate must be positive");
    if (k_payload + h->crc_deg != h->K || k_payload < 0)
        return fail(PSCL_EINVAL, "k_payload (%d) + crc degree (%d) must equal K (%d)", k_payload, h->crc_deg, h->K);
    int rc = no_enter ? set_device(h) : enter(h);
    if (rc) return rc;
    pscl_channel_params P;
    memset(&P, 0, sizeof(P));
    P.seed = seed;
    P.stream_id = stream_id;
    P.N = h->N;
    P.K = h->K;
    P.W = h->W;
    P.k_payload = k_payload;
    P.crc_deg = h->crc_deg;
    P.xtab = h->d_xtab;
    P.crctab = h->d_crctab;
    const double ebno = pow(10.0, ebno_db / 10.0);
    P.noise_var = 1.0 / (2.0 * rate * ebno);
    P.sigma = sqrt(P.noise_var);
    P.llr_scale = 2.0 / P.noise_var;
    P.frame0 = frame0;
    P.B = B;
    P.llr = d_llr;
    P.msg = d_msg;
    P.rm_E = h->rm_E;
    P.rm_order = h->d_rm_order;
    if (d_unc) {
        P.unc_counters = d_unc;
        P.unc_sigma = sqrt(1.0 / (2.0 * ebno));
    }
    hipError_t e = pscl_launch_channel(P, h->stream);
    if (e != hipSuccess) return fail(PSCL_EDEVICE, "channel kernel launch: %s", hipGetErrorString(e));
    return PSCL_OK;
}
}

int pscl_channel_device(pscl_handle* h, uint64_t seed, uint32_t stream_id, double ebno_db, double rate, int k_payload,
                        int64_t frame0, int64_t B, double* d_llr, uint64_t* d_msg) {
    return channel_launch(h, seed, stream_id, ebno_db, rate, k_payload, frame0, B, d_llr, d_msg, nullptr);
}

int pscl_set_rate_match(pscl_handle* h, int E) {
    if (!h) return fail(PSCL_EINVAL, "NULL handle");
    if (E < 0) return fail(PSCL_EINVAL, "E must be >= 0");
    if (E > 0 && E > h->N && h->N < 32)
        return fail(PSCL_EUNSUP, "repetition (E > N) needs N >= 32 (sub-block interleaver without padding)");
    if (E == h->rm_E) return PSCL_OK;
    const int rc = enter(h);
    if (rc) return rc;
    h->rm_E = E;
    return PSCL_OK;
}

int pscl_device_alloc(pscl_handle* h, void** d_ptr, int64_t bytes) {
    if (!h || !d_ptr || bytes < 0) return fail(PSCL_EINVAL, "bad arguments");
    int rc = enter(h);
    if (rc) return rc;
    HIP_TRY(hipMalloc(d_ptr, (size_t)(bytes > 0 ? bytes : 1)));
    return PSCL_OK;
}

int pscl_device_free(pscl_handle* h, void* d_ptr) {
    if (!h) return fail(PSCL_EINVAL, "NULL handle");
    int rc = enter(h);
    if (rc) return rc;
    HIP_TRY(hipStreamSynchronize(h->stream));
    quiesce(h);
    if (d_ptr) HIP_TRY(hipFree(d_ptr));
    return PSCL_OK;
}

int pscl_memcpy_htod(pscl_handle* h, void* d_dst, const void* src, int64_t bytes) {
    if (!h) return fail(PSCL_EINVAL, "NULL handle");
    int rc = enter(h);
    if (rc) return rc;
    HIP_TRY(hipMemcpyAsync(d_dst, src, (size_t)bytes, hipMemcpyHostToDevice, h->stream));
    HIP_TRY(hipStreamSynchronize(h->stream));
    return PSCL_OK;
}

int pscl_memcpy_dtoh(pscl_handle* h, void* dst, const void* d_src, int64_t bytes) {
    if (!h) return fail(PSCL_EINVAL, "NULL handle");
    int rc = enter(h);
    if (rc) return rc;
    HIP_TRY(hipMemcpyAsync(dst, d_src, (size_t)bytes, hipMemcpyDeviceToHost, h->stream));
    HIP_TRY(hipStreamSynchronize(h->stream));
    return PSCL_OK;
}

int pscl_memset_device(pscl_handle* h, void* d_dst, int value, int64_t bytes) {
    if (!h) return fail(PSCL_EINVAL, "NULL handle");
    int rc = enter(h);
    if (rc) return rc;
    HIP_TRY(hipMemsetAsync(d_dst, value, (size_t)bytes, h->stream));
    return PSCL_OK;
}

int pscl_set_screening(pscl_handle* h, int enable) {
    if (!h) return fail(PSCL_EINVAL, "NULL handle");
    h->screen = enable != 0;
    return PSCL_OK;
}

int pscl_screening_count(pscl_handle* h, int64_t* count) {
    if (!h || !count) return fail(PSCL_EINVAL, "bad arguments");
    *count = 0;
    if (!h->screened || !h->scratch[h->screened_slot].p) return PSCL_OK;
    int rc = enter(h);
    if (rc) return rc;
    int32_t c = 0;
    HIP_TRY(hipMemcpyAsync(&c, h->scratch[h->screened_slot].p, 4, hipMemcpyDeviceToHost, h->stream));
    HIP_TRY(hipStreamSynchronize(h->stream));
    *count = c;
    return PSCL_OK;
}

int pscl_softplus_tails_device(pscl_handle* h, const double* d_v, int64_t n, double* d_exact, double* d_apx) {
    if (!h) return fail(PSCL_EINVAL, "NULL handle");
    if (n < 0) return fail(PSCL_EINVAL, "n must be >= 0");
    if (n == 0) return PSCL_OK;
    if (!d_v || !d_exact || !d_apx) return fail(PSCL_EINVAL, "d_v, d_exact and d_apx are required");
    int rc = enter(h);
    if (rc) return rc;
    hipError_t e = pscl_launch_softplus_tails(d_v, n, h->d_exp_table, d_exact, d_apx, h->stream);
    if (e != hipSuccess) return fail(PSCL_EDEVICE, "softplus tails launch: %s", hipGetErrorString(e));
    return PSCL_OK;
}

namespace {
int tail_scan(pscl_handle* h, uint32_t lo, uint32_t hi, uint64_t* d_out, int bits) {
    if (!h) return fail(PSCL_EINVAL, "NULL handle");
    if (!d_out) return fail(PSCL_EINVAL, "d_out is required");
    if (lo > hi) return fail(PSCL_EINVAL, "lo > hi");
    int rc = enter(h);
    if (rc) return rc;
    hipError_t e =
        pscl_launch_tail_abs_scan(lo, hi, h->d_exp_table, reinterpret_cast<unsigned long long*>(d_out), h->stream, bits);
    if (e != hipSuccess) return fail(PSCL_EDEVICE, "tail scan launch: %s", hipGetErrorString(e));
    return PSCL_OK;
}
}

int pscl_tail_abs_scan_device(pscl_handle* h, uint32_t lo, uint32_t hi, uint64_t* d_out) {
    return tail_scan(h, lo, hi, d_out, 0);
}

int pscl_tail2_scan_device(pscl_handle* h, uint32_t lo, uint32_t hi, uint64_t* d_out) {
    return tail_scan(h, lo, hi, d_out, 1);
}

int pscl_timing_enable(pscl_handle* h, int enable) {
    if (!h) return fail(PSCL_EINVAL, "NULL handle");
    h->timing = enable != 0;
    h->ev_used = 0;
    return PSCL_OK;
}

int pscl_timing_read_split(pscl_handle* h, int64_t* main_launches, double* main_ms, int64_t* side_launches,
                           double* side_ms) {
    if (!h) return fail(PSCL_EINVAL, "NULL handle");
    int rc = enter(h);
    if (rc) return rc;
    HIP_TRY(hipStreamSynchronize(h->stream));
    quiesce(h);
    double tot[2] = {0.0, 0.0};
    int64_t cnt[2] = {0, 0};
    for (size_t i = 0; i + 1 < h->ev_used; i += 2) {
        float ms = 0.f;
        HIP_TRY(hipEventElapsedTime(&ms, h->ev_pool[i], h->ev_pool[i + 1]));
        const int m = h->ev_main[i / 2] ? 0 : 1;
        tot[m] += ms;
        ++cnt[m];
    }
    if (main_launches) *main_launches = cnt[0];
    if (main_ms) *main_ms = tot[0];
    if (side_launches) *side_launches = cnt[1];
    if (side_ms) *side_ms = tot[1];
    return PSCL_OK;
}

int pscl_timing_read(pscl_handle* h, int64_t* launches, double* total_ms) {
    if (!h || !launches || !total_ms) return fail(PSCL_EINVAL, "bad arguments");
    int64_t n0 = 0, n1 = 0;
    double t0 = 0.0, t1 = 0.0;
    const int rc = pscl_timing_read_split(h, &n0, &t0, &n1, &t1);
    if (rc) return rc;
    *launches = n0 + n1;
    *total_ms = t0 + t1;
    return PSCL_OK;
}

int pscl_host_stats(pscl_handle* h, double* call_ms, double* wait_ms, int64_t* calls, int reset) {
    if (!h) return fail(PSCL_EINVAL, "NULL handle");
    if (call_ms) *call_ms = h->host_call_ms;
    if (wait_ms) *wait_ms = h->host_wait_ms;
    if (calls) *calls = h->host_calls;
    if (reset) {
        h->host_call_ms = h->host_wait_ms = 0.0;
        h->host_calls = 0;
    }
    return PSCL_OK;
}

int pscl_path_stats(pscl_handle* h, int64_t* fused_post_rounds, int64_t* post_rounds, int64_t* fused_tx_blocks,
                    int64_t* post_epw4_launches, int64_t* lane_exact_launches) {
    if (!h) return fail(PSCL_EINVAL, "NULL handle");
    if (lane_exact_launches) *lane_exact_launches = h->n_lane_exact;
    if (post_epw4_launches) *post_epw4_launches = h->n_post_epw4;
    if (fused_post_rounds) *fused_post_rounds = h->n_fpost_rounds;
    if (post_rounds) *post_rounds = h->n_post_rounds;
    if (fused_tx_blocks) *fused_tx_blocks = h->n_fused_tx;
    return PSCL_OK;
}

int pscl_launch_info(pscl_handle* h, int64_t B, int* waves_per_wg, int64_t* grid, int* lds_bytes) {
    if (!h) return fail(PSCL_EINVAL, "NULL handle");
    pscl_decode_params P;
    fill_decode_params(h, P, 0);
    P.B = B;
    if (waves_per_wg) *waves_per_wg = pscl_decode_wpg(P);
    if (grid) *grid = pscl_decode_grid(P);
    if (lds_bytes) *lds_bytes = pscl_decode_lds(P, 0);
    return PSCL_OK;
}

}
```

polar_code_amd/csrc/scl128_lane.hip:

```cpp
#ifndef PSCL_LANE_REMAP
#define PSCL_LANE_REMAP 0
#endif
#if PSCL_LANE_REMAP
#define PSCL_LANE_FRAME_MIRROR 0x140
#endif
#include "scl_lane.h"

#ifdef PSCL_LANE_F32_UNIT
using lane_llr_t = float;
#define scl_lane_kernel scl_lane_kernel_f32
#else
using lane_llr_t = double;
#endif

namespace {

#ifndef PSCL_LANE_REG56
#define PSCL_LANE_REG56 1
#endif

#ifndef PSCL_LANE_FRES8
#define PSCL_LANE_FRES8 8
#endif
#ifndef PSCL_LANE_FRES4
#define PSCL_LANE_FRES4 24
#endif

template <int LMAX>
struct LaneLayout {
    static constexpr int G = LMAX;
    static constexpr int F = 64 / G;
    static constexpr int LOG_G = __builtin_ctz(G);
    static constexpr int OFF3 = 0;
    static constexpr int OFF4 = OFF3 + 16 * LMAX;
    static constexpr int OFF5 = OFF4 + 8 * LMAX;
    static constexpr int OFF6 = OFF5 + 4 * LMAX;
    static constexpr int OFFX = PSCL_LANE_REG56 ? OFF4 : OFF6;
    static constexpr int RAW = PSCL_LANE_REG56 ? OFF5 : OFF6 + 2 * LMAX;
    static constexpr int FRES = LMAX == 8 ? PSCL_LANE_FRES8 : PSCL_LANE_FRES4;
    static constexpr int FSTRIDE = RAW + (((FRES - RAW) % 32) + 32) % 32;
    static constexpr int FSTRIDE_FS = FSTRIDE >= 128 ? FSTRIDE : FSTRIDE + 32;
    static constexpr int FSTRIDE_EX = FSTRIDE + 8;
};

__device__ __forceinline__ uint64_t flip_order_key(double q) {
    if (q == 0.0) q = 0.0;
    const uint64_t u = pscl_asu64(q);
    return (u >> 63) ? ~u : (u | 0x8000000000000000ULL);
}

#ifndef PSCL_LANE_CREG4
#define PSCL_LANE_CREG4 1
#endif

#ifndef PSCL_LANE_ABL
#define PSCL_LANE_ABL 0
#endif

#ifndef PSCL_LANE_WAVES_PER_EU
#define PSCL_LANE_WAVES_PER_EU 2
#endif

#ifndef PSCL_LANE_U0T
#define PSCL_LANE_U0T 1
#endif
#ifndef PSCL_LANE_GSPLIT
#define PSCL_LANE_GSPLIT 1
#endif

__device__ __forceinline__ void tx_frame_words(const pscl_decode_params& P, uint64_t fr, uint64_t (&m)[2],
                                               uint64_t (&raw)[2], uint64_t (&x)[2]) {
    const u32x4 rb = philox4x32(u32x4{(uint32_t)fr, (uint32_t)(fr >> 32), 0xffffffffu, 0u}, P.tx_k0, P.tx_k1);
    raw[0] = ((uint64_t)rb.y << 32) | rb.x;
    raw[1] = ((uint64_t)rb.w << 32) | rb.z;
    const int kp = P.tx_kp, nbp = (kp + 7) >> 3, nb = (P.K + 7) >> 3;
    m[0] = kp >= 64 ? raw[0] : (raw[0] & ((1ULL << kp) - 1));
    m[1] = kp > 64 ? (raw[1] & ((kp >= 128) ? ~0ULL : ((1ULL << (kp - 64)) - 1))) : 0;
    uint32_t rem = 0;
    for (int k = 0; k < nbp; ++k) rem ^= P.tx_crctab[k * 256 + (uint32_t)((m[k >> 3] >> (8 * (k & 7))) & 255u)];
    if (P.tx_crc_deg) {
        const uint64_t rw = (uint64_t)rem;
        if (kp < 64) {
            m[0] |= rw << kp;
            if (kp + P.tx_crc_deg > 64) m[1] |= rw >> (64 - kp);
        } else {
            m[1] |= rw << (kp - 64);
        }
    }
    x[0] = x[1] = 0;
    for (int k = 0; k < nb; ++k) {
        const uint32_t v = (uint32_t)((m[k >> 3] >> (8 * (k & 7))) & 255u);
        x[0] ^= P.tx_xtab[(k * 256 + v) * 2];
        x[1] ^= P.tx_xtab[(k * 256 + v) * 2 + 1];
    }
}

#ifndef PSCL_FS_WAVES
#define PSCL_FS_WAVES 3
#endif
#ifndef PSCL_TX_WAVES
#define PSCL_TX_WAVES 3
#endif
template <int LMAX, int CODE, bool FS = false, bool TXF = false, bool FP = false, bool EX = false, bool RL = false>
__global__ void __launch_bounds__(64, TXF ? (LMAX == 8 ? PSCL_TX_WAVES : 2)
                                           : (FS && !FP && !EX && LMAX == 8) ? PSCL_FS_WAVES : PSCL_LANE_WAVES_PER_EU)
scl_lane_kernel(const pscl_decode_params P) {
    static_assert(LMAX == 4 || LMAX == 8, "the lane-per-path decoder is built for L = 4 and 8");
    static_assert(!TXF || (!FS && CODE == 1), "fused TX: plain decodes of the (128,64) code");
    static_assert(!FP || (FS && CODE == 1), "fused post pass: the FS instance of the (128,64) code");
    static_assert(!EX || (!TXF && !FP), "the exact instance: plain re-decodes and forced-bit retry decodes");
    static_assert(!RL || (!FS && !TXF && !FP && !EX), "the row-list form: plain screening decodes");
    using Ly = LaneLayout<LMAX>;
    constexpr int G = Ly::G, F = Ly::F, LOG_G = Ly::LOG_G;
    constexpr int EPL = 16 / G;
    constexpr uint32_t GM = (1u << G) - 1u;
    constexpr int K = kSpecK[CODE], PW = (K + 63) / 64;
    constexpr uint64_t info0 = kSpecInfo[CODE][0], info1 = kSpecInfo[CODE][1];
    extern __shared__ __attribute__((aligned(16))) unsigned char smem[];
    double* const A = reinterpret_cast<double*>(smem);
    const int lane = threadIdx.x & 63;
    constexpr bool REMAP = PSCL_LANE_REMAP && G == 8 && !EX;
    const int rq = (lane >> 2) & 3, inner = (rq == 1 || rq == 2) ? 1 : 0;
    const int fl = REMAP ? 2 * (lane >> 4) + inner : lane >> LOG_G;
    const int p = REMAP ? (lane & 3) + 4 * (rq & 1) : lane & (G - 1);
    const int lane_lo = REMAP ? (lane & ~15) + (inner ? 8 : 0) : lane & ~(G - 1);
    const int lane_hi = REMAP ? (lane & ~15) + (inner ? 4 : 12) : lane_lo + 4;
    auto lane_of = [&](uint32_t q) -> int { return REMAP ? (q < 4u ? lane_lo + (int)q : lane_hi + (int)q - 4) : lane_lo + (int)q; };
    double* const Af = A + fl * (FP ? Ly::FSTRIDE_FS : EX ? Ly::FSTRIDE_EX : Ly::FSTRIDE);
    int* const sl = reinterpret_cast<int*>(Af + Ly::FSTRIDE);
    const uint8_t* const GT = reinterpret_cast<const uint8_t*>(P.epi_table);
    const uint32_t* const ST = reinterpret_cast<const uint32_t*>(GT + 16 * 256);
    auto hiw = [](double m) { return (uint32_t)(pscl_asu64(m) >> 32); };
    constexpr bool BITS = !FS && !EX && PSCL_LANE_BITS;
    constexpr bool PLAIN = !FS && !EX && !TXF;
    constexpr bool U0T = PLAIN && PSCL_LANE_U0T;
    constexpr bool GSPLIT = PLAIN && PSCL_LANE_GSPLIT && (LMAX == 8 || PSCL_LANE_CREG4);
    constexpr double MARGIN = BITS ? PSCL_TAIL2_MARGIN : PSCL_TAIL_ABS_MARGIN;
    auto hiw_up = [&](double m) {
        double r;
        asm("v_fma_f64 %0, %1, %2, %3" : "=v"(r) : "v"(m), "s"(1.0 + 0x1p-40), "v"(MARGIN));
        return hiw(r);
    };
    auto frame_bits = [&](uint64_t m) -> uint32_t {
        if constexpr (REMAP) return ((uint32_t)(m >> lane_lo) & 15u) | (((uint32_t)(m >> lane_hi) & 15u) << 4);
        return (uint32_t)(m >> lane_lo) & GM;
    };

    int cfe = 0, cbe = 0, cpe = 0, cpb = 0;
    int tufe = 0, tube = 0;
    int pdecodes = 0;
    int bpre[PSCL_DL_NSEG + 1];
    int64_t Bn = P.B;
    if constexpr (FS) {
        const int64_t tot = pscl_bucket_prefix(P.bcount, P.bcap, bpre);
        Bn = tot < P.B ? tot : P.B;
    } else if constexpr (EX) {
        if (P.d_count) Bn = *P.d_count < P.B ? (int64_t)*P.d_count : P.B;
    } else if constexpr (RL) {
        Bn = *P.d_count < P.B ? (int64_t)*P.d_count : P.B;
    }
    for (int64_t f0 = (int64_t)blockIdx.x * F; f0 < Bn; f0 += (int64_t)gridDim.x * F) {
        const int64_t fi = f0 + fl;
        const bool fvalid = fi < Bn;
        const int64_t fsafe = fvalid ? fi : f0;
        int64_t f = fi, frow = fsafe;
        int seg0 = 0;
        if constexpr (FS) {
            f = pscl_elist_entry(P, fsafe, bpre);
            seg0 = pscl_bucket_of(f0, bpre);
            frow = P.fidx[f];
        } else if constexpr (EX) {
            if (P.fidx) frow = P.fidx[fsafe];
        } else if constexpr (RL) {
            frow = P.fidx[fsafe];
        }
        constexpr bool RM = CODE == 2;
        const lane_llr_t* chan = reinterpret_cast<const lane_llr_t*>(P.llr) + frow * (RM ? (int64_t)P.rm_E : (int64_t)kN);
        auto chan_at = [&](int i) -> double { return RM ? nr_stage(chan, P.rm_src[i], P.rm_E, kN) : (double)chan[i]; };
        constexpr bool CREG = G == 8 || PSCL_LANE_CREG4 || TXF;
        double c[8 * EPL];
        uint64_t tm[2] = {0, 0}, traw[2] = {0, 0}, tx[2] = {0, 0};
        const uint64_t tfr = TXF ? (uint64_t)(P.tx_frame0 + fsafe) : 0ULL;
        if constexpr (TXF) tx_frame_words(P, tfr, tm, traw, tx);
        auto gen_chan = [&](double* v, uint64_t fr) {
#pragma unroll
            for (int k = 0; k < EPL; ++k)
#pragma unroll
                for (int j = 0; j < 4; ++j) {
                    const uint32_t blk = (uint32_t)(p + G * k + 16 * j);
                    const u32x4 rn = philox4x32(u32x4{(uint32_t)fr, (uint32_t)(fr >> 32), blk, 0u}, P.tx_k0, P.tx_k1);
                    double z[2];
                    bm_pair(((uint64_t)rn.y << 32) | rn.x, ((uint64_t)rn.w << 32) | rn.z, z[0], z[1]);
#pragma unroll
                    for (int h = 0; h < 2; ++h) {
                        const double sym = ((tx[h] >> blk) & 1ULL) ? -1.0 : 1.0;
                        v[8 * k + j + 4 * h] = (sym + P.tx_sigma * z[h]) * P.tx_scale;
                    }
                    __builtin_amdgcn_sched_barrier(0);
                }
        };
        auto load_chan = [&]() {
            if constexpr (TXF) {
                gen_chan(c, tfr);
                if constexpr (BITS)
#pragma unroll
                    for (int m = 0; m < 8 * EPL; ++m) c[m] = c[m] * PSCL_LOG2E_F64;
            } else {
#pragma unroll
                for (int k = 0; k < EPL; ++k)
#pragma unroll
                    for (int m = 0; m < 8; ++m) c[8 * k + m] = BITS ? chan_at(p + G * k + 16 * m) * PSCL_LOG2E_F64
                                                                    : chan_at(p + G * k + 16 * m);
            }
        };
        load_chan();
        uint32_t ah[4 * EPL];
#pragma unroll
        for (int m = 0; m < 4 * EPL; ++m) {
            ah[m] = GSPLIT ? hiw(c[8 * (m >> 2) + (m & 3)]) : 0u;
            if constexpr (GSPLIT) asm volatile("" : "+v"(ah[m]));
        }
        if constexpr (TXF) {
            if (P.tx_upart) {
                uint32_t berr = 0;
                for (int cb = p; 2 * cb < P.tx_kp; cb += G) {
                    const u32x4 rn = philox4x32(u32x4{(uint32_t)tfr, (uint32_t)(tfr >> 32), 0x40000000u + (uint32_t)cb, 0u},
                                                P.tx_k0, P.tx_k1);
                    double z[2];
                    bm_pair(((uint64_t)rn.y << 32) | rn.x, ((uint64_t)rn.w << 32) | rn.z, z[0], z[1]);
#pragma unroll
                    for (int h = 0; h < 2; ++h) {
                        const int q = 2 * cb + h;
                        if (q < P.tx_kp) {
                            const uint32_t bit = (uint32_t)((traw[q >> 6] >> (q & 63)) & 1ULL);
                            const double y = (bit ? -1.0 : 1.0) + P.tx_unc_sigma * z[h];
                            berr += ((y < 0.0) ? 1u : 0u) != bit ? 1u : 0u;
                        }
                    }
                }
                berr = frame_sum<G>(berr);
                if (fvalid && p == 0) {
                    tufe += berr ? 1 : 0;
                    tube += (int)berr;
                }
            }
        }
        double cs = fabs(c[0]);
#pragma unroll
        for (int m = 1; m < 8 * EPL; ++m) cs = cs + fabs(c[m]);
        uint64_t amb = EX ? 0ULL : wmask(!(cs < (BITS ? PSCL_TAIL2_CHAN_SUM : 0x1p25)));
        const uint64_t vmask = wmask(fvalid);

        double metric = 0.0;
        uint64_t u0 = 0, u1 = 0;
        uint32_t tab = 0;
        uint32_t lastbit = 0;
        double r5[4] = {0.0, 0.0, 0.0, 0.0}, r6[2] = {0.0, 0.0};
        uint64_t fm0 = 0, fm1 = 0, fv0 = 0, fv1 = 0;
        int lcnt = 0;
        if constexpr (FS) {
            const uint64_t* fr = P.force + f * 2 * PW;
            fm0 = fr[0];
            fv0 = fr[PW];
            if (PW > 1) {
                fm1 = fr[1];
                fv1 = fr[PW + 1];
            }
            if (seg0 > 0) {
                metric = P.warm_metric[f * PSCL_DL_NSEG + seg0];
                const int lo = 16 * seg0;
                u0 = P.warm_u[2 * f];
                u1 = P.warm_u[2 * f + 1];
                if (lo < 64) {
                    u0 &= (1ULL << lo) - 1ULL;
                    u1 = 0;
                } else {
                    u1 = lo == 64 ? 0ULL : (u1 & ((1ULL << (lo - 64)) - 1ULL));
                }
            }
        }

        auto phase = [&](auto PC) {
            constexpr int phi = decltype(PC)::value;
            constexpr int t = phi & 15;
            constexpr int start = t ? kn - __builtin_ctz((unsigned)t) : ((phi >> 4) ? 3 - __builtin_ctz((unsigned)(phi >> 4)) : 1);
            constexpr bool is_info = ((phi < 64 ? info0 : info1) >> (phi & 63)) & 1;
            constexpr int jb = phi < 64 ? __builtin_popcountll(info0 & ((1ULL << (phi & 63)) - 1))
                                        : __builtin_popcountll(info0) + __builtin_popcountll(info1 & ((1ULL << (phi & 63)) - 1));
            constexpr int cnt = jb >= LOG_G ? LMAX : (1 << jb);
#ifdef PSCL_PHASE_MARKERS
            asm volatile("; PHASE %0" ::"n"(t));
#endif

            if constexpr (start <= 3 && !(PSCL_LANE_ABL & 4)) {
                constexpr bool r1 = phi >= 64, r2 = (phi >> 5) & 1, r3 = (phi >> 4) & 1;
                if constexpr (!CREG && phi > 0) load_chan();
                uint4* const xs = reinterpret_cast<uint4*>(Af + Ly::OFFX);
                if constexpr (r1 || r2 || r3) {
                    uint64_t X1 = 0;
                    uint32_t X2 = 0, X3 = 0;
                    if constexpr (U0T && phi == 64) u0 = polar_transform64(u0);
                    if (r1) X1 = U0T ? u0 : polar_transform64(u0);
                    if (r2) {
                        constexpr int lo = phi - (phi & 31) - 32;
                        X2 = polar_transform32((uint32_t)((lo >= 64 ? u1 : u0) >> (lo & 63)));
                    }
                    if (r3) {
                        constexpr int lo = phi - 16;
                        X3 = polar_transform16((uint32_t)((lo >= 64 ? u1 : u0) >> (lo & 63)) & 0xffffu);
                    }
                    xs[p] = make_uint4((uint32_t)X1, (uint32_t)(X1 >> 32), X2, (X2 >> 16) | (X3 << 16));
                    wave_lds_fence();
                }
                constexpr bool shared2 = !r1 && !r2;
                double d1l[EPL][4], d2s[EPL][2];
#pragma unroll
                for (int h = 0; h < EPL; ++h) {
#pragma unroll
                    for (int m = 0; m < 4; ++m) d1l[h][m] = r1 ? 0.0 : f_minsum(c[8 * h + m], c[8 * h + m + 4]);
#pragma unroll
                    for (int s2 = 0; s2 < 2; ++s2) d2s[h][s2] = shared2 ? f_minsum(d1l[h][s2], d1l[h][s2 + 2]) : 0.0;
                }
                constexpr int npaths = FS ? LMAX : cnt;
#pragma unroll
                for (int q0 = 0; q0 < npaths; ++q0) {
                    const int q = npaths == LMAX ? ((q0 + p) & (LMAX - 1)) : q0;
                    uint64_t x1 = 0, x23 = 0;
                    if constexpr (r1 || r2 || r3) {
                        const uint4 xv = xs[q];
                        x1 = ((uint64_t)xv.y << 32) | xv.x;
                        x23 = ((uint64_t)xv.w << 32) | xv.z;
                    }
                    double d3[EPL];
#pragma unroll
                    for (int h = 0; h < EPL; ++h) {
                        const uint32_t e = (uint32_t)(p + G * h);
                        const uint64_t s1[2] = {r1 ? x1 << (31u - e) : 0ULL, r1 ? x1 << (15u - e) : 0ULL};
                        const uint64_t s2w = r2 ? x23 << (31u - e) : 0ULL;
                        double d1[4];
#pragma unroll
                        for (int m = 0; m < 4; ++m)
                            d1[m] = !r1 ? d1l[h][m]
                                    : GSPLIT ? g_node_bit31_split(c[8 * h + m], ah[4 * h + m], c[8 * h + m + 4],
                                                                  (uint32_t)(s1[m & 1] >> (32 * (m >> 1))))
                                             : g_node_bit31(c[8 * h + m], c[8 * h + m + 4], (uint32_t)(s1[m & 1] >> (32 * (m >> 1))));
                        double d2[2];
#pragma unroll
                        for (int s2 = 0; s2 < 2; ++s2)
                            d2[s2] = shared2 ? d2s[h][s2]
                                             : (r2 ? g_node_bit31(d1[s2], d1[s2 + 2], (uint32_t)(s2w >> (32 * s2))) : f_minsum(d1[s2], d1[s2 + 2]));
                        d3[h] = r3 ? g_node_wbit(d2[0], d2[1], (uint32_t)(x23 >> 32), e + 16) : f_minsum(d2[0], d2[1]);
                    }
#pragma unroll
                    for (int h = 0; h < EPL / 2; ++h)
                        *reinterpret_cast<double2*>(Af + Ly::OFF3 + ((p + G * h) * LMAX + q) * 2) = make_double2(d3[h], d3[h + EPL / 2]);
                }
                wave_lds_fence();
            }
            if constexpr (start <= 6) {
                uint32_t xsb = 0;
                if constexpr (phi && start >= 4) {
                    constexpr int w = 1 << (kn - start), lo = phi - w;
                    static_assert(phi <= 64 || lo >= 64, "u0 is not read bit-wise after phase 64 (PSCL_LANE_U0T)");
                    xsb = polar_transform8((uint32_t)((lo >= 64 ? u1 : u0) >> (lo & 63)) & ((1u << w) - 1u));
                }
                static_for<3>([&](auto DI) {
                    constexpr int D = 4 + decltype(DI)::value;
                    if constexpr (D >= start) {
// ... 180 lines not shown
                        const uint32_t kg = hiw(mg);
                        bool keep_g, win_b;
                        select_survivors<G, LMAX>(kg, kb, keep_g, win_b);
                        const uint32_t kbu = hiw_up(mb);
                        const uint32_t su = keep_g ? (win_b ? kbu : kgu) : (win_b ? kbu : 0u);
                        const uint32_t nmk = keep_g ? (win_b ? 0xffffffffu : kb) : kg;
                        const uint32_t nsurv = frame_sum<G>((keep_g ? 1u : 0u) + (win_b ? 1u : 0u));
                        const uint32_t smax = frame_max<G>(su), nmin = frame_min<G>(nmk);
                        amb |= wmask(full && !(nsurv == (uint32_t)LMAX && nmin > smax)) & vmask;
                        const uint32_t f8 = frame_bits(wmask(!keep_g)), w8 = frame_bits(wmask(win_b));
                        const uint32_t jj = __builtin_popcount(f8 & ((1u << p) - 1u));
                        const int rsrc = lane_of(nth_set_bit8(w8, jj));
                        if (full && !keep_g) {
                            pull = true;
                            src = rsrc;
                        }
                    }
                }
                if (wmask(pull) != 0) {
                    const uint64_t pubm = pscl_asu64(full ? mb : m1);
                    const uint32_t tw = tab | ((full ? (gbit ^ 1u) : 1u) << 31);
                    const uint64_t pm = shfl_u64(pubm, src);
                    const uint64_t pu0 = shfl_u64(u0, src);
                    const uint64_t pu1 = phi >= 64 ? shfl_u64(u1, src) : 0ULL;
                    const uint32_t ptw = bperm32(tw, src);
                    double q5[4], q6[2];
                    carry(src, q5, q6);
                    if (pull) {
                        nm = pscl_asf64(pm);
                        u0 = pu0;
                        u1 = pu1;
                        tab = ptw & 0x7fffffffu;
                        b = ptw >> 31;
                        take(q5, q6);
                    }
                }
                metric = nm;
                if (phi < 64) u0 |= (uint64_t)b << phi; else u1 |= (uint64_t)b << (phi - 64);
                lastbit = b;
                lcnt += grow ? 1 : 0;
                return;
            }
            if constexpr (cnt < LMAX) {
                const double m0 = gbit ? mb : mg, m1 = gbit ? mg : mb;
                const int src = lane_of((uint32_t)(p & (cnt - 1)));
                const uint32_t b = (p & cnt) ? 1u : 0u;
                const uint64_t pm1 = shfl_u64(pscl_asu64(m1), src);
                metric = b ? pscl_asf64(pm1) : m0;
                u0 = shfl_u64(u0, src);
                if (phi >= 64) u1 = shfl_u64(u1, src);
                tab = bperm32(tab, src);
                double q5[4], q6[2];
                carry(src, q5, q6);
                take(q5, q6);
                if (phi < 64) u0 |= (uint64_t)b << phi; else u1 |= (uint64_t)b << (phi - 64);
                lastbit = b;
                return;
            }
            const uint32_t kgu = hiw_up(mg), kb = hiw(mb);
            const uint32_t mx = frame_max<G>(kgu);
            const bool bad = kb <= mx;
            const uint64_t badm = wmask(bad);
#ifdef PSCL_STATS
            const bool one = (wmask(__builtin_popcount(frame_bits(badm)) > 1) & vmask) == 0;
            if (lane == 0 && P.counters) {
                atomicAdd(reinterpret_cast<unsigned long long*>(P.counters) + ((badm & vmask) == 0 ? 12 : (one ? 13 : 14)), 1ULL);
            }
#endif
            metric = mg;
            uint32_t b = gbit;
            if (!(PSCL_LANE_ABL & 2) && ((badm & vmask) != 0 || (PSCL_LANE_ABL & 1))) {
                const uint32_t bad8 = frame_bits(badm);
                bool pull;
                int src;
#if PSCL_LANE_SWAP
                if (!(PSCL_LANE_ABL & 1) && (wmask(__builtin_popcount(bad8) > 1) & vmask) == 0) {
                    const uint32_t kg = hiw(mg);
                    const uint32_t gmaxh = frame_max<G>(kg);
                    const bool ismax = kg == gmaxh;
                    const uint32_t nmax = frame_sum<G>(ismax ? 1u : 0u);
                    const uint32_t g2u = frame_max<G>(ismax ? 0u : kgu);
                    const uint32_t wu = frame_max<G>(bad ? hiw_up(mb) : 0u);
                    const bool swap = bad8 != 0;
                    amb |= wmask(swap && !(nmax == 1u && g2u < gmaxh && wu < gmaxh)) & vmask;
                    src = lane_of(__builtin_ctz(bad8 | (1u << G)) & (G - 1));
                    pull = swap && ismax;
                } else
#endif
                {
                    const uint32_t kg = hiw(mg);
                    uint32_t rg, rbb;
                    rank_children<G>(kg, kb, rg, rbb);
                    const bool keep_g = rg < (uint32_t)LMAX;
                    const uint32_t f8 = frame_bits(wmask(!keep_g));
                    const uint32_t d = __builtin_popcount(f8);
                    const bool win_b = rbb < d;
                    const uint32_t w8 = frame_bits(wmask(win_b));
#if defined(PSCL_STATS) && PSCL_STATS == 2
                    {
                        const uint32_t dw = frame_sum<G>(win_b ? 1u : 0u);
                        const uint32_t nb = __builtin_popcount(bad8);
                        unsigned long long* C = reinterpret_cast<unsigned long long*>(P.counters);
                        if (p == 0 && fvalid && C) {
                            atomicAdd(C + 16 + (dw > 8u ? 8u : dw), 1ULL);
                            atomicAdd(C + 25 + nb, 1ULL);
                        }
                        uint32_t md = 0;
                        for (uint32_t k = 1; k <= 8; ++k)
                            if (wmask(dw >= k) & vmask) md = k;
                        if (lane == 0 && C) atomicAdd(C + 34 + md, 1ULL);
                    }
#endif
                    const uint32_t kbu = hiw_up(mb);
                    const uint32_t su = keep_g ? (win_b ? kbu : kgu) : (win_b ? kbu : 0u);
                    const uint32_t nm = keep_g ? (win_b ? 0xffffffffu : kb) : kg;
                    const uint32_t smax = frame_max<G>(su), nmin = frame_min<G>(nm);
                    amb |= wmask(!((uint32_t)__builtin_popcount(w8) == d && nmin > smax)) & vmask;
                    const uint32_t j = __builtin_popcount(f8 & ((1u << p) - 1u));
                    src = lane_of(nth_set_bit8(w8, j));
                    pull = !keep_g;
                }
                const int srce = pull ? src : lane;
                const uint64_t pmb = shfl_u64(pscl_asu64(mb), srce);
                const uint32_t ptw = bperm32(tab | ((gbit ^ 1u) << 31), srce);
                u0 = shfl_u64(u0, srce);
                if constexpr (phi >= 64) u1 = shfl_u64(u1, srce);
                tab = ptw & 0x7fffffffu;
                double q5[4], q6[2];
                carry(srce, q5, q6);
                take(q5, q6);
                if (pull) {
                    metric = pscl_asf64(pmb);
                    b = ptw >> 31;
                }
            }
            if (phi < 64) u0 |= (uint64_t)b << phi; else u1 |= (uint64_t)b << (phi - 64);
            lastbit = b;
        };
        if constexpr (FS) {
            auto seg = [&](auto SB) {
                static_for<16>([&](auto TC) { phase(std::integral_constant<int, decltype(SB)::value * 16 + decltype(TC)::value>{}); });
            };
            using std::integral_constant;
            switch (seg0) {
                case 0: seg(integral_constant<int, 0>{}); [[fallthrough]];
                case 1: seg(integral_constant<int, 1>{}); [[fallthrough]];
                case 2: seg(integral_constant<int, 2>{}); [[fallthrough]];
                case 3: seg(integral_constant<int, 3>{}); [[fallthrough]];
                case 4: seg(integral_constant<int, 4>{}); [[fallthrough]];
                case 5: seg(integral_constant<int, 5>{}); [[fallthrough]];
                case 6: seg(integral_constant<int, 6>{}); [[fallthrough]];
                default: seg(integral_constant<int, 7>{});
            }
        } else {
            static_for<kN>([&](auto PC) { phase(PC); });
        }

        auto fused_post = [&](bool x_amb, bool x_live, uint32_t x_keyb, uint32_t x_kbest, uint64_t x_ib0, uint64_t x_ib1,
                              uint64_t x_u0, uint64_t x_u1, int64_t x_frow, int64_t e, bool x_valid) {
            static_assert(!REMAP, "the fused post pass assumes frames of G consecutive lanes");
            const pscl_post_params& Q = P.fp;
            constexpr int NC = K / G;
            const uint32_t fl = (x_kbest < (uint32_t)LMAX ? PSCL_FLAG_CRC_PASS : 0u) | (x_kbest & (uint32_t)(LMAX - 1));
            const bool mine = x_valid && !x_amb;
            int nt = 0;
            uint64_t t0 = 0, t1 = 0;
            if (mine) {
                nt = Q.ntried[e];
                t0 = Q.tried[2 * e];
                t1 = Q.tried[2 * e + 1];
            }
            const uint32_t bfb = frame_bits(wmask(x_live && x_keyb == x_kbest));
            const int bsrc = lane_lo + (bfb ? __builtin_ctz(bfb) : 0);
            const uint64_t bi0 = shfl_u64(x_ib0, bsrc), bi1 = PW > 1 ? shfl_u64(x_ib1, bsrc) : 0ULL;
            const uint64_t bu0 = shfl_u64(x_u0, bsrc), bu1 = shfl_u64(x_u1, bsrc);
            if (mine && p == 0) {
                Q.best[x_frow * PW] = bi0;
                if (PW > 1) Q.best[x_frow * PW + 1] = bi1;
                Q.flags[x_frow] = (uint8_t)fl;
                if (Q.attempts) Q.attempts[x_frow] = nt + 1;
                ++pdecodes;
            }
            const bool more = mine && !(fl & PSCL_FLAG_CRC_PASS) && nt < Q.rounds;
            if (wmask(more) == 0) return;
            wave_lds_fence();
            {
                const double* crow = P.llr + x_frow * kN;
#pragma unroll
                for (int j = 0; j < kN / G; ++j) Af[p + G * j] = crow[p + G * j];
            }
            wave_lds_fence();
            auto stage = [](uint64_t x, int st) {
                const uint64_t M = st == 1 ? 0x5555555555555555ULL : st == 2 ? 0x3333333333333333ULL
                                 : st == 4 ? 0x0f0f0f0f0f0f0f0fULL : st == 8 ? 0x00ff00ff00ff00ffULL
                                 : st == 16 ? 0x0000ffff0000ffffULL : 0x00000000ffffffffULL;
                return x ^ ((x >> st) & M);
            };
            uint64_t X0 = bu0, X1 = bu1;
#pragma unroll
            for (int mm = 1; mm < kn; ++mm) {
                X0 = stage(X0, 1 << (mm - 1));
                X1 = stage(X1, 1 << (mm - 1));
            }
            static_for<kn>([&](auto DC) {
                constexpr int lw2 = kn - 1 - decltype(DC)::value, w2 = 1 << lw2;
                const bool act_l = w2 >= G || (p & w2) == 0;
                if (act_l) {
#pragma unroll 2
                    for (int j = 0; j < kN / G; ++j) {
                        const int q = p + G * j;
                        if (w2 >= G && (q & w2)) continue;
                        const double a = Af[q], b = Af[q + w2];
                        const uint32_t bit = (uint32_t)(((q >> 6) ? X1 : X0) >> (q & 63)) & 1u;
                        Af[q] = f_minsum(a, b);
                        Af[q + w2] = g_node(a, b, bit);
                    }
                }
                wave_lds_fence();
                if constexpr (lw2 > 0) {
                    X0 = stage(X0, w2 >> 1);
                    X1 = stage(X1, w2 >> 1);
                }
            });
            float qv[NC];
            double as = 0.0;
            uint64_t bk = ~0ULL;
            int bj = 0x7fffffff;
            auto seen_j = [&](int j) { return (((j < 64 ? t0 : t1) >> (j & 63)) & 1ULL) != 0; };
            auto argmin = [&]() {
                bk = ~0ULL;
                bj = 0x7fffffff;
#pragma unroll
                for (int i = 0; i < NC; ++i) {
                    const int j = p + G * i;
                    const uint64_t key = seen_j(j) ? ~0ULL : flip_order_key((double)qv[i]);
                    if (key < bk) {
                        bk = key;
                        bj = j;
                    }
                }
#pragma unroll
                for (int sft = 1; sft < G; sft <<= 1) {
                    const uint64_t ok = shfl_u64(bk, lane ^ sft);
                    const int oj = __shfl(bj, lane ^ sft);
                    if (ok < bk || (ok == bk && oj < bj)) {
                        bk = ok;
                        bj = oj;
                    }
                }
            };
            auto argmin_exact = [&]() {
                bk = ~0ULL;
                bj = 0x7fffffff;
#pragma unroll 1
                for (int i = 0; i < NC; ++i) {
                    const int j = p + G * i;
                    double qx = 0.0;
#pragma unroll 1
                    for (int k = 0; k < K; ++k) qx = qx + fabs(Af[Q.info_set[k]]) * Q.beta[k * K + j];
                    const uint64_t key = seen_j(j) ? ~0ULL : flip_order_key(qx);
                    if (key < bk) {
                        bk = key;
                        bj = j;
                    }
                }
#pragma unroll
                for (int sft = 1; sft < G; sft <<= 1) {
                    const uint64_t ok = shfl_u64(bk, lane ^ sft);
                    const int oj = __shfl(bj, lane ^ sft);
                    if (ok < bk || (ok == bk && oj < bj)) {
                        bk = ok;
                        bj = oj;
                    }
                }
            };
            if (Q.beta) {
                typedef float f2 __attribute__((ext_vector_type(2)));
                constexpr int CB = NC < 8 ? NC : 8;
                const f2* bg = reinterpret_cast<const f2*>(P.fp_beta32g) + p * (NC / 2);
#pragma unroll
                for (int cb = 0; cb < NC / CB; ++cb) {
                    f2 acc[CB / 2];
#pragma unroll
                    for (int i = 0; i < CB / 2; ++i) acc[i] = (f2){0.0f, 0.0f};
#pragma unroll 2
                    for (int k = 0; k < K; ++k) {
                        const double ad = fabs(Af[Q.info_set[k]]);
                        if (cb == 0) as = as + ad;
                        const float a32 = (float)ad;
#pragma unroll
                        for (int i = 0; i < CB / 2; ++i)
                            acc[i] = __builtin_elementwise_fma((f2){a32, a32}, bg[k * G * (NC / 2) + cb * (CB / 2) + i], acc[i]);
                    }
#pragma unroll
                    for (int i = 0; i < CB / 2; ++i) {
                        qv[cb * CB + 2 * i] = acc[i].x;
                        qv[cb * CB + 2 * i + 1] = acc[i].y;
                    }
                }
                argmin();
                const double gk = (4.0 * (double)K + 8.0) * 0x1p-53;
                const double e2 = (as < 0x1p100 && as * Q.beta_absmax < 0x1p100)
                                      ? 2.04 * (as * Q.beta_absmax * (((double)K + 2.01) * 0x1p-24 + 0.5 * gk)
                                                + (double)K * 0x1p-149 + as * 0x1p-150 + (double)K * Q.beta_absmax * 0x1p-150)
                                      : __builtin_inf();
                double qmine = qv[0];
// ... 88 lines not shown
                if (mm == 0) continue;
                int base = 0;
                if (lane == (int)__builtin_ctzll(mm)) base = atomicAdd(Q.out_count + sg * PSCL_DL_CSTRIDE, __popcll(mm));
                base = __shfl(base, (int)__builtin_ctzll(mm));
                if ((mm >> lane) & 1ULL)
                    Q.out_list[(int64_t)sg * Q.cap + base + __popcll(mm & ((1ULL << lane) - 1ULL))] = (int32_t)e;
            }
            wave_lds_fence();
        };
        uint64_t tfr2 = tfr;
        if constexpr (TXF) {
            asm volatile("" : "+v"(tfr2));
            tx_frame_words(P, tfr2, tm, traw, tx);
        }
        uint64_t ib0 = 0, ib1 = 0;
        if constexpr (U0T) u0 = polar_transform64(u0);
        {
            int off = 0;
#pragma unroll
            for (int k = 0; k < 16; ++k) {
                const uint32_t byte = (uint32_t)(((k < 8 ? u0 : u1) >> (8 * (k & 7))) & 255u);
                const uint64_t cb = (PSCL_LANE_ABL & 8) ? (uint64_t)byte : GT[k * 256 + byte];
                if (off < 64) {
                    ib0 |= cb << off;
                    if (off > 56) ib1 |= cb >> (64 - off);
                } else {
                    ib1 |= cb << (off - 64);
                }
                off += __builtin_popcount((uint32_t)(((k < 8 ? info0 : info1) >> (8 * (k & 7))) & 255u));
            }
        }
        uint32_t syn = 0;
        if (P.has_crc) {
            constexpr int k4 = (K + 3) >> 2;
#pragma unroll
            for (int m = 0; m < k4; ++m)
                syn ^= (PSCL_LANE_ABL & 8) ? (uint32_t)(((m < 16 ? ib0 : ib1) >> (4 * (m & 15))) & 15u) << m
                                           : ST[m * 16 + (uint32_t)(((m < 16 ? ib0 : ib1) >> (4 * (m & 15))) & 15u)];
        }
        const bool live = !FS || p < (1 << lcnt);
        const uint32_t kh = live ? hiw(metric) : 0xffffffffu, ku = live ? hiw_up(metric) : 0xffffffffu;
        uint32_t r = 0;
        bool near = false;
        auto cmp_perm = [&](uint32_t oh, uint32_t ou) {
            r += oh < kh ? 1u : 0u;
            near = near || !(ku < oh || ou < kh);
        };
        if constexpr (EX) {
            r = (uint32_t)p;
        } else {
            cmp_perm(dpp32<kQX1>(kh), dpp32<kQX1>(ku));
            cmp_perm(dpp32<kQX2>(kh), dpp32<kQX2>(ku));
            cmp_perm(dpp32<kQX3>(kh), dpp32<kQX3>(ku));
            if constexpr (G == 8) {
                const uint32_t mh = dpp32<kFMIR>(kh), mu = dpp32<kFMIR>(ku);
                cmp_perm(mh, mu);
                cmp_perm(dpp32<kQX1>(mh), dpp32<kQX1>(mu));
                cmp_perm(dpp32<kQX2>(mh), dpp32<kQX2>(mu));
                cmp_perm(dpp32<kQX3>(mh), dpp32<kQX3>(mu));
            }
        }
        amb |= wmask(near && live) & vmask;
        const bool famb = frame_bits(amb) != 0;
        if (famb && p == 0 && fvalid) {
            if constexpr (FS) {
                const int fseg = (FP || P.warm_apx) ? 0 : pscl_bucket_of(fsafe, bpre);
                const int slot = atomicAdd(P.amb_count + fseg * PSCL_DL_CSTRIDE, 1);
                P.amb_elist[(int64_t)fseg * P.bcap + slot] = (int32_t)f;
                P.flags[f] = PSCL_DL_DEFERRED;
            } else {
                P.amb_list[atomicAdd(P.amb_count, 1)] = RL ? frow : fi;
            }
        }
        const uint32_t pass = P.has_crc ? (syn == 0 ? 1u : 0u) : 1u;
        const uint32_t keyb = live ? (pass ? r : (uint32_t)LMAX + r) : 0xffffu;
        const uint32_t kbest = frame_min<G>(keyb);
        if (fvalid && !famb && keyb == kbest) {
            const int best = (int)(kbest & (uint32_t)(LMAX - 1));
            const bool bpass = kbest < (uint32_t)LMAX;
            const int64_t fo = (RL || (EX && !FS && P.out_by_row)) ? frow : f;
            if (P.best) {
                P.best[fo * PW] = ib0;
                if (PW > 1) P.best[fo * PW + 1] = ib1;
            }
            if (P.flags) P.flags[fo] = (uint8_t)((bpass ? PSCL_FLAG_CRC_PASS : 0u) | (uint32_t)best);
            if (P.n_paths) P.n_paths[fo] = FS ? (1 << lcnt) : LMAX;
            if (!FS && !RL && P.ref) {
                const uint64_t ibw[2] = {ib0, ib1};
                tally_errors(ibw, TXF ? tm : P.ref + fo * PW, PW, P.k_payload, bpass, cfe, cbe, cpe, cpb);
            }
        }
        if constexpr (FS) {
            if constexpr (FP) fused_post(famb, live, keyb, kbest, ib0, ib1, u0, u1, frow, f, fvalid);
        }
        if constexpr (TXF) {
            if (fvalid && p == 0) {
                P.tx_msg[fi * PW] = tm[0];
                if (PW > 1) P.tx_msg[fi * PW + 1] = tm[1];
            }
        }
        wave_lds_fence();
    }
    if (!FS && !RL && P.ref) {
        flush_counts_p(P, blockIdx.x, cfe, cbe, cpe, cpb);
        if (blockIdx.x == 0 && threadIdx.x == 0 && !(EX && P.out_by_row))
            atomicAdd(reinterpret_cast<unsigned long long*>(P.counters) + PSCL_CNT_FRAMES, (unsigned long long)P.B);
    }
    if constexpr (FS) {
        if (FP && P.fp.counters && __builtin_amdgcn_ballot_w64(pdecodes != 0)) {
            const int d = wave_sum(pdecodes);
            if (lane == 0) atomicAdd(reinterpret_cast<unsigned long long*>(P.fp.counters) + PSCL_CNT_RETRIES, (unsigned long long)d);
        }
    }
    if constexpr (TXF) {
        if (P.tx_upart && __builtin_amdgcn_ballot_w64((tufe | tube) != 0)) {
            const int fe = wave_sum(tufe), be = wave_sum(tube);
            if (lane == 0) reinterpret_cast<int4*>(P.tx_upart)[blockIdx.x] = make_int4(fe, be, 0, 0);
        }
        if (P.tx_unc_counters && blockIdx.x == 0 && threadIdx.x == 0)
            atomicAdd(reinterpret_cast<unsigned long long*>(P.tx_unc_counters) + PSCL_CNT_FRAMES, (unsigned long long)P.B);
    }
}

}

#ifndef PSCL_LANE_LDS_PAD
#define PSCL_LANE_LDS_PAD 0
#endif

#ifdef PSCL_LANE_RL_UNIT
#ifdef PSCL_LANE_F32_UNIT
#define PSCL_LANE_RL_LAUNCH pscl_launch_lane_rowlist_f32
#else
#define PSCL_LANE_RL_LAUNCH pscl_launch_lane_rowlist
#endif
hipError_t PSCL_LANE_RL_LAUNCH(const pscl_decode_params& P, int64_t grid, hipStream_t s) {
    const int lds8 = LaneLayout<8>::F * LaneLayout<8>::FSTRIDE * 8 + PSCL_LANE_LDS_PAD,
              lds4 = LaneLayout<4>::F * LaneLayout<4>::FSTRIDE * 8 + PSCL_LANE_LDS_PAD;
    if (!pscl_rowlist(P) || (P.f32 != 0) != (sizeof(lane_llr_t) == 4)) return hipErrorInvalidValue;
    const dim3 g((unsigned)grid), b(64);
    if (P.L == 8 && !P.rm_E)
        hipLaunchKernelGGL((scl_lane_kernel<8, 1, false, false, false, false, true>), g, b, lds8, s, P);
    else if (P.L == 8)
        hipLaunchKernelGGL((scl_lane_kernel<8, 2, false, false, false, false, true>), g, b, lds8, s, P);
    else if (P.L == 4 && !P.rm_E)
        hipLaunchKernelGGL((scl_lane_kernel<4, 1, false, false, false, false, true>), g, b, lds4, s, P);
    else if (P.L == 4)
        hipLaunchKernelGGL((scl_lane_kernel<4, 2, false, false, false, false, true>), g, b, lds4, s, P);
    else
        return hipErrorInvalidValue;
    return hipGetLastError();
}
#elif defined(PSCL_LANE_F32_UNIT)
hipError_t pscl_launch_lane_f32(const pscl_decode_params& P, int64_t grid, hipStream_t s) {
    const int lds8 = LaneLayout<8>::F * LaneLayout<8>::FSTRIDE * 8 + PSCL_LANE_LDS_PAD,
              lds4 = LaneLayout<4>::F * LaneLayout<4>::FSTRIDE * 8 + PSCL_LANE_LDS_PAD;
    if (!P.f32 || P.tx) return hipErrorInvalidValue;
    if (pscl_rowlist(P)) return pscl_launch_lane_rowlist_f32(P, grid, s);
    if (P.L == 8 && !P.rm_E)
        hipLaunchKernelGGL((scl_lane_kernel<8, 1>), dim3((unsigned)grid), dim3(64), lds8, s, P);
    else if (P.L == 8)
        hipLaunchKernelGGL((scl_lane_kernel<8, 2>), dim3((unsigned)grid), dim3(64), lds8, s, P);
    else if (P.L == 4 && !P.rm_E)
        hipLaunchKernelGGL((scl_lane_kernel<4, 1>), dim3((unsigned)grid), dim3(64), lds4, s, P);
    else if (P.L == 4)
        hipLaunchKernelGGL((scl_lane_kernel<4, 2>), dim3((unsigned)grid), dim3(64), lds4, s, P);
    else
        return hipErrorInvalidValue;
    return hipGetLastError();
}
#else

int pscl_lane_frames_per_wg(int L) { return 64 / L; }

hipError_t pscl_launch_lane(const pscl_decode_params& P, int64_t grid, hipStream_t s) {
    const int lds8 = LaneLayout<8>::F * LaneLayout<8>::FSTRIDE * 8 + PSCL_LANE_LDS_PAD,
              lds4 = LaneLayout<4>::F * LaneLayout<4>::FSTRIDE * 8 + PSCL_LANE_LDS_PAD;
    if (P.f32) return hipErrorInvalidValue;
    if (pscl_rowlist(P)) return pscl_launch_lane_rowlist(P, grid, s);
    if (P.tx) {
        if (P.rm_E) return hipErrorInvalidValue;
        if (P.L == 8)
            hipLaunchKernelGGL((scl_lane_kernel<8, 1, false, true>), dim3((unsigned)grid), dim3(64), lds8, s, P);
        else if (P.L == 4)
            hipLaunchKernelGGL((scl_lane_kernel<4, 1, false, true>), dim3((unsigned)grid), dim3(64), lds4, s, P);
        else
            return hipErrorInvalidValue;
        return hipGetLastError();
    }
    if (P.L == 8 && !P.rm_E)
        hipLaunchKernelGGL((scl_lane_kernel<8, 1>), dim3((unsigned)grid), dim3(64), lds8, s, P);
    else if (P.L == 8)
        hipLaunchKernelGGL((scl_lane_kernel<8, 2>), dim3((unsigned)grid), dim3(64), lds8, s, P);
    else if (P.L == 4 && !P.rm_E)
        hipLaunchKernelGGL((scl_lane_kernel<4, 1>), dim3((unsigned)grid), dim3(64), lds4, s, P);
    else if (P.L == 4)
        hipLaunchKernelGGL((scl_lane_kernel<4, 2>), dim3((unsigned)grid), dim3(64), lds4, s, P);
    else
        return hipErrorInvalidValue;
    return hipGetLastError();
}

int64_t pscl_lane_exact_grid(const pscl_decode_params& P) {
    const int F = 64 / P.L;
    const int64_t grid = (P.B + F - 1) / F, cap = P.grid_cap > 0 ? P.grid_cap : (1 << 20);
    return grid < 1 ? 1 : (grid > cap ? cap : grid);
}

hipError_t pscl_launch_lane_exact(const pscl_decode_params& P, hipStream_t s) {
    const int64_t grid = pscl_lane_exact_grid(P);
    const int lds8 = LaneLayout<8>::F * LaneLayout<8>::FSTRIDE_EX * 8, lds4 = LaneLayout<4>::F * LaneLayout<4>::FSTRIDE_EX * 8;
    if (P.f32) return hipErrorInvalidValue;
    const dim3 g((unsigned)grid), b(64);
    if (P.force) {
        if (P.L == 8)
            hipLaunchKernelGGL((scl_lane_kernel<8, 1, true, false, false, true>), g, b, lds8, s, P);
        else if (P.L == 4)
            hipLaunchKernelGGL((scl_lane_kernel<4, 1, true, false, false, true>), g, b, lds4, s, P);
        else
            return hipErrorInvalidValue;
    } else if (P.L == 8) {
        if (P.rm_E)
            hipLaunchKernelGGL((scl_lane_kernel<8, 2, false, false, false, true>), g, b, lds8, s, P);
        else
            hipLaunchKernelGGL((scl_lane_kernel<8, 1, false, false, false, true>), g, b, lds8, s, P);
    } else if (P.L == 4) {
        if (P.rm_E)
            hipLaunchKernelGGL((scl_lane_kernel<4, 2, false, false, false, true>), g, b, lds4, s, P);
        else
            hipLaunchKernelGGL((scl_lane_kernel<4, 1, false, false, false, true>), g, b, lds4, s, P);
    } else {
        return hipErrorInvalidValue;
    }
    return hipGetLastError();
}

hipError_t pscl_launch_lane_fs(const pscl_decode_params& P, int64_t grid, hipStream_t s) {
    const int lds8 = LaneLayout<8>::F * (P.fpost ? LaneLayout<8>::FSTRIDE_FS : LaneLayout<8>::FSTRIDE) * 8,
              lds4 = LaneLayout<4>::F * (P.fpost ? LaneLayout<4>::FSTRIDE_FS : LaneLayout<4>::FSTRIDE) * 8;
    if (P.f32) return hipErrorInvalidValue;
    if (P.fpost && (P.K != 64 || (P.fp.beta && !P.fp_beta32g))) return hipErrorInvalidValue;
    if (P.L == 8)
        if (P.fpost)
            hipLaunchKernelGGL((scl_lane_kernel<8, 1, true, false, true>), dim3((unsigned)grid), dim3(64), lds8, s, P);
        else
            hipLaunchKernelGGL((scl_lane_kernel<8, 1, true>), dim3((unsigned)grid), dim3(64), lds8, s, P);
    else if (P.L == 4)
        if (P.fpost)
            hipLaunchKernelGGL((scl_lane_kernel<4, 1, true, false, true>), dim3((unsigned)grid), dim3(64), lds4, s, P);
        else
            hipLaunchKernelGGL((scl_lane_kernel<4, 1, true>), dim3((unsigned)grid), dim3(64), lds4, s, P);
    else
        return hipErrorInvalidValue;
    return hipGetLastError();
}
#endif
```

polar_code_amd/csrc/scl_kernels.h:

```cpp
#ifndef PSCL_SCL_KERNELS_H
#define PSCL_SCL_KERNELS_H

#include <hip/hip_runtime.h>
#include <stddef.h>
#include <stdint.h>

#include "polar_scl.h"

#define PSCL_MAX_WAVES_PER_WG 4
#define PSCL_FAST_N 128
#ifndef PSCL_EPI_LDS
#define PSCL_EPI_LDS 1
#endif

struct pscl_post_params {
    const double* llr;
    int N, n, K, W, rm_E;
    const int32_t* rm_src;
    uint64_t info_mask[2];
    const int32_t* info_set;
    const uint64_t* exp_table;
    int rounds;
    int narrow;
    int epw;
// ... 98 lines not shown
#define PSCL_DL_NSEG 8
#define PSCL_DL_CSTRIDE 16
#define PSCL_DL_DEFERRED 0xFF

__device__ __forceinline__ int pscl_bucket_of(int64_t i, const int* pre) {
    int k = 0;
#pragma unroll
    for (int q = 1; q < PSCL_DL_NSEG; ++q) k += i >= pre[q] ? 1 : 0;
    return k;
}
__device__ __forceinline__ int64_t pscl_elist_entry(const pscl_decode_params& P, int64_t i, const int* pre) {
    const int k = pscl_bucket_of(i, pre);
    return P.elist[(int64_t)k * P.bcap + (i - pre[k])];
}
__device__ __forceinline__ int64_t pscl_bucket_prefix(const int32_t* bcount, int64_t cap, int* pre) {
    int acc = 0;
    pre[0] = 0;
#pragma unroll
    for (int k = 0; k < PSCL_DL_NSEG; ++k) {
        const int c = bcount[k * PSCL_DL_CSTRIDE];
        acc += c < cap ? c : (int)cap;
        pre[k + 1] = acc;
    }
    return acc;
}

struct pscl_replay_params {
    const double* llr;
    int N, n, K, W, rm_E;
    const int32_t* rm_src;
    uint64_t info_mask[2];
    const int32_t* count;
    const int32_t* list;
    const int64_t* act;
    const uint64_t* bits;
    int bits_by_row;
    double* out;
};

struct pscl_post_long_params {
    int K, W, rounds, init;
    int64_t cap;
    const int32_t* in_count;
    int32_t* out_count;
    const int64_t* act_in;
    int64_t* act_out;
    const uint64_t* tried_in;
    uint64_t* tried_w_out;
    const int32_t* nt_in;
    int32_t* nt_out;
    const uint64_t* ob;
    const uint8_t* of;
    const double* l0;
    uint64_t* force;
    const double* beta;
    uint64_t* best;
    uint8_t* flags;
    int32_t* attempts;
    int32_t* tried_out;
    int tried_stride;
    int64_t* counters;
};

struct pscl_channel_params {
    uint64_t seed;
    uint32_t stream_id;
    int N, K, W, k_payload, crc_deg;
    const uint64_t* xtab;
    const uint32_t* crctab;
    double sigma, noise_var;
    double llr_scale;
    double unc_sigma;
    int64_t* unc_counters;
    int64_t frame0, B;
    double* llr;
    uint64_t* msg;
    int rm_E;
    const int32_t* rm_order;
};

struct pscl_sc_params {
    const double* llr;
    int64_t B;
    int K, W;
    uint64_t info_mask[2];
    const uint64_t* epi_table;
    int epi_words;
    int rm_E;
    const int32_t* rm_src;
    uint64_t* best;
    uint8_t* flags;
    uint8_t* stage;
};
int pscl_sc_lane_lds(const pscl_sc_params& P);
int64_t pscl_sc_lane_grid(const pscl_sc_params& P);
hipError_t pscl_launch_sc_lane(const pscl_sc_params& P, hipStream_t s);
hipError_t pscl_launch_sc_lane_f32(const pscl_sc_params& P, hipStream_t s);
hipError_t pscl_launch_gather_rows_f32(const float* llr, int64_t row, const int64_t* act, int64_t n, double* out,
                                       hipStream_t s);
hipError_t pscl_launch_gather_rows(const double* llr, int64_t row, const int64_t* act, int64_t n, double* out,
                                   hipStream_t s);
hipError_t pscl_launch_scatter_results(const int64_t* act, int64_t n, int W, const uint64_t* best_in,
                                       const uint8_t* flags_in, uint64_t* best, uint8_t* flags, hipStream_t s);
hipError_t pscl_launch_add_counter(int64_t* counters, int slot, int64_t v, hipStream_t s);
hipError_t pscl_launch_publish_count(const int32_t* count, int64_t* counters, int slot, int32_t* out, hipStream_t s);

struct pscl_scn_params {
    const double* llr;
    int64_t B;
    int N, K, W;
    uint64_t info_mask[16];
    const uint64_t* epi_table;
    int epi_words;
    uint64_t* best;
    uint8_t* flags;
    uint8_t* stage;
};
int pscl_scn_lane_available(int N);
int pscl_scn_lane_lds(const pscl_scn_params& P);
int64_t pscl_scn_lane_grid(const pscl_scn_params& P);
hipError_t pscl_launch_scn_lane(const pscl_scn_params& P, hipStream_t s);
hipError_t pscl_launch_mark_stage(const int64_t* act, int64_t n, uint8_t* stage, hipStream_t s);

int pscl_decode_lmax(int L);
int64_t pscl_long_block_bytes(int N, int L, int K, int hist);
int64_t pscl_long_grid(int64_t B, int L);
hipError_t pscl_launch_long(const pscl_decode_params& P, int hist, hipStream_t s);
void pscl_decode_layout(pscl_decode_params& P, int hist);
int pscl_fast128_fstride(int L, int ch);
int pscl_screening_available(const pscl_decode_params& P);
#ifndef PSCL_LANE
#define PSCL_LANE 1
#endif
#ifndef PSCL_LANE_NR
#define PSCL_LANE_NR 1
#endif
#ifndef PSCL_LANE_FS
#define PSCL_LANE_FS 1
#endif
#ifndef PSCL_LANE4
#define PSCL_LANE4 1
#endif
inline int pscl_rowlist(const pscl_decode_params& P) {
    return P.apx && P.fidx && P.d_count && P.out_by_row && P.amb_list && P.amb_count && !P.force && !P.elist &&
           !P.ref && !P.tx && !P.sc_hard;
}
int pscl_lane_available(const pscl_decode_params& P);
int pscl_lane_frames_per_wg(int L);
hipError_t pscl_launch_lane(const pscl_decode_params& P, int64_t grid, hipStream_t s);
hipError_t pscl_launch_lane_rowlist(const pscl_decode_params& P, int64_t grid, hipStream_t s);
hipError_t pscl_launch_lane_f32(const pscl_decode_params& P, int64_t grid, hipStream_t s);
hipError_t pscl_launch_lane_rowlist_f32(const pscl_decode_params& P, int64_t grid, hipStream_t s);
int pscl_f32_decode_available(const pscl_decode_params& P);
#ifndef PSCL_LANE_COUNT_GRID
#define PSCL_LANE_COUNT_GRID 32768
#endif
#ifndef PSCL_COUNT_GRID
#define PSCL_COUNT_GRID 8192
#endif
int64_t pscl_decode_count_slots(const pscl_decode_params& P, int hist);
hipError_t pscl_launch_count_reduce(int32_t* cpart, int64_t slots, int64_t* counters, hipStream_t s);
#ifndef PSCL_DL_LANE_DEFAULT
#define PSCL_DL_LANE_DEFAULT 1
#endif
int pscl_lane_long_available(const pscl_decode_params& P);
int pscl_lane_long128_available(const pscl_decode_params& P);
hipError_t pscl_launch_lane_long(const pscl_decode_params& P, hipStream_t s);
int64_t pscl_lane_long_grid(const pscl_decode_params& P);
int pscl_screening_fs_available(const pscl_decode_params& P);
int pscl_lane_fs_available(const pscl_decode_params& P);
hipError_t pscl_launch_lane_fs(const pscl_decode_params& P, int64_t grid, hipStream_t s);
int pscl_lane_exact_available(const pscl_decode_params& P);
hipError_t pscl_launch_lane_exact(const pscl_decode_params& P, hipStream_t s);
int64_t pscl_lane_exact_grid(const pscl_decode_params& P);
hipError_t pscl_launch_decode128(const pscl_decode_params& P, int hist, int wpg, int64_t grid, int lds, hipStream_t s);
int64_t pscl_decode_grid(const pscl_decode_params& P);
int pscl_decode_wpg(const pscl_decode_params& P);
int pscl_decode_lds(const pscl_decode_params& P, int hist);
hipError_t pscl_launch_decode(const pscl_decode_params& P, int hist, hipStream_t s);
hipError_t pscl_launch_channel(const pscl_channel_params& P, hipStream_t s);
hipError_t pscl_launch_tx_rows(const pscl_decode_params& P, const int64_t* list, const int32_t* count, int64_t cap,
                               double* rows, int64_t frame0, hipStream_t s);
hipError_t pscl_launch_uncoded(const pscl_channel_params& P, int64_t* counters, hipStream_t s);
hipError_t pscl_launch_dl_compact(const uint8_t* flags, int64_t B, int64_t base, int64_t* act, int32_t* list,
                                  int32_t* count, hipStream_t s);
hipError_t pscl_launch_iota64(int64_t* out, int64_t n, hipStream_t s);
hipError_t pscl_launch_dl_mark_stage(const int64_t* act, int64_t n, uint8_t* stage, int value, hipStream_t s);
hipError_t pscl_launch_replay(const pscl_replay_params& R, int64_t cap, hipStream_t s);
hipError_t pscl_launch_tail_abs_scan(uint32_t lo, uint32_t hi, const uint64_t* exp_table, unsigned long long* out,
                                     hipStream_t s, int bits);
hipError_t pscl_launch_softplus_tails(const double* v, int64_t n, const uint64_t* exp_table, double* exact,
                                     double* apx, hipStream_t s);
hipError_t pscl_launch_dl_post(const pscl_post_params& Q, int64_t entries, hipStream_t s);
int pscl_post_epw(const pscl_post_params& Q);
hipError_t pscl_launch_dl_post_long(const pscl_post_long_params& Q, hipStream_t s);
hipError_t pscl_launch_dl_count(const uint64_t* best, const uint8_t* flags, const uint64_t* ref, int64_t B, int W,
                                int k_payload, int64_t* counters, hipStream_t s);

#endif
```

polar_code_amd/csrc/scl_kernels.hip:

```cpp
#include <hip/hip_runtime.h>
#include <stdint.h>
#include <stdlib.h>

#include "glibc_softplus.h"
#include "scl_device.h"
#include "scl_kernels.h"

namespace {

using namespace pscl;

template <int LMAX, bool HIST>
__global__ void __launch_bounds__(PSCL_MAX_WAVES_PER_WG * kWave)
    scl_decode_kernel(const pscl_decode_params P) {
    constexpr int G = 2 * LMAX;
    constexpr int F = kWave / G;
    constexpr int LOG_G = __builtin_ctz(G);
    extern __shared__ __attribute__((aligned(16))) unsigned char smem[];
    uint64_t* T = reinterpret_cast<uint64_t*>(smem);
    for (int i = threadIdx.x; i < PSCL_EXP_TABLE_WORDS; i += blockDim.x) T[i] = P.exp_table[i];
    __syncthreads();

    const int wave = threadIdx.x >> 6;
    const int lane = threadIdx.x & 63;
// ... 360 lines not shown
            part[wave][0] = fe;
            part[wave][1] = be;
        }
        __syncthreads();
        if (threadIdx.x == 0) {
            const int tf = part[0][0] + part[1][0] + part[2][0] + part[3][0];
            const int tb = part[0][1] + part[1][1] + part[2][1] + part[3][1];
            unsigned long long* C = reinterpret_cast<unsigned long long*>(P.unc_counters);
            if (tf) atomicAdd(C + PSCL_CNT_FRAME_ERR, (unsigned long long)tf);
            if (tb) atomicAdd(C + PSCL_CNT_BIT_ERR, (unsigned long long)tb);
        }
    }
}

}

__global__ void __launch_bounds__(256) tx_rows_kernel(const pscl_decode_params P, const int64_t* __restrict__ list,
                                                      const int32_t* __restrict__ count, int64_t cap, double* rows,
                                                      int64_t frame0) {
    const int wave = threadIdx.x >> 6, lane = threadIdx.x & 63;
    int64_t n = *count;
    if (n > cap) n = cap;
    for (int64_t i = (int64_t)blockIdx.x * 4 + wave; i < n; i += (int64_t)gridDim.x * 4) {
        const int64_t b = list[i];
        const uint64_t fr = (uint64_t)(frame0 + b);
        const u32x4 rb = philox4x32(u32x4{(uint32_t)fr, (uint32_t)(fr >> 32), 0xffffffffu, 0u}, P.tx_k0, P.tx_k1);
        const uint64_t r0 = ((uint64_t)rb.y << 32) | rb.x, r1 = ((uint64_t)rb.w << 32) | rb.z;
        const int kp = P.tx_kp, nbp = (kp + 7) >> 3, nb = (P.K + 7) >> 3;
        uint64_t m0 = kp >= 64 ? r0 : (r0 & ((1ULL << kp) - 1));
        uint64_t m1 = kp > 64 ? (r1 & ((kp >= 128) ? ~0ULL : ((1ULL << (kp - 64)) - 1))) : 0;
        uint32_t rem = 0;
        for (int k = 0; k < nbp; ++k) rem ^= P.tx_crctab[k * 256 + (uint32_t)(((k < 8 ? m0 : m1) >> (8 * (k & 7))) & 255u)];
        if (P.tx_crc_deg) {
            const uint64_t rw = (uint64_t)rem;
            if (kp < 64) {
                m0 |= rw << kp;
                if (kp + P.tx_crc_deg > 64) m1 |= rw >> (64 - kp);
            } else {
                m1 |= rw << (kp - 64);
            }
        }
        uint64_t x0 = 0, x1 = 0;
        for (int k = 0; k < nb; ++k) {
            const uint32_t v = (uint32_t)(((k < 8 ? m0 : m1) >> (8 * (k & 7))) & 255u);
            x0 ^= P.tx_xtab[(k * 256 + v) * 2];
            x1 ^= P.tx_xtab[(k * 256 + v) * 2 + 1];
        }
        const u32x4 rn = philox4x32(u32x4{(uint32_t)fr, (uint32_t)(fr >> 32), (uint32_t)lane, 0u}, P.tx_k0, P.tx_k1);
        double z[2];
        bm_pair(((uint64_t)rn.y << 32) | rn.x, ((uint64_t)rn.w << 32) | rn.z, z[0], z[1]);
        double* row = rows + b * 128;
#pragma unroll
        for (int h = 0; h < 2; ++h) {
            const double sym = (((h ? x1 : x0) >> lane) & 1ULL) ? -1.0 : 1.0;
            row[lane + 64 * h] = (sym + P.tx_sigma * z[h]) * P.tx_scale;
        }
    }
}


hipError_t pscl_launch_tx_rows(const pscl_decode_params& P, const int64_t* list, const int32_t* count, int64_t cap,
                               double* rows, int64_t frame0, hipStream_t s) {
    if (cap <= 0) return hipSuccess;
    int64_t grid = (cap + 3) / 4;
    if (grid > 1024) grid = 1024;
    hipLaunchKernelGGL(tx_rows_kernel, dim3((unsigned)grid), dim3(256), 0, s, P, list, count, cap, rows, frame0);
    return hipGetLastError();
}

int pscl_decode_wpg(const pscl_decode_params& P) {
    if (P.long_mode) return 1;
    const int cu_lds = 160 * 1024, tbl = P.wg_fixed_bytes;
    int best = 0, best_res = 0;
    const int wmax = P.wpg_cap >= 1 && P.wpg_cap < PSCL_MAX_WAVES_PER_WG ? P.wpg_cap : PSCL_MAX_WAVES_PER_WG;
    for (int w = 1; w <= wmax; ++w) {
        const int wg = tbl + w * P.wave_bytes;
        if (wg > cu_lds) break;
        int res = (cu_lds / wg) * w;
        if (res > 32) res = 32;
        if (res >= best_res) {
            best_res = res;
            best = w;
        }
    }
    return best;
}

static int decode_lds_bytes(const pscl_decode_params& P, int hist) {
    (void)hist;
    return P.wg_fixed_bytes + pscl_decode_wpg(P) * P.wave_bytes;
}

template <int LMAX>
static hipError_t launch_l(const pscl_decode_params& P, int hist, int64_t grid, hipStream_t s) {
    const int lds = decode_lds_bytes(P, hist);
    const int threads = pscl_decode_wpg(P) * kWave;
    if (hist) {
        hipLaunchKernelGGL((scl_decode_kernel<LMAX, true>), dim3((unsigned)grid), dim3(threads), lds, s, P);
    } else {
        hipLaunchKernelGGL((scl_decode_kernel<LMAX, false>), dim3((unsigned)grid), dim3(threads), lds, s, P);
    }
    return hipGetLastError();
}

int pscl_decode_lmax(int L) {
    if (L <= 1) return 1;
    if (L <= 2) return 2;
    if (L <= 4) return 4;
    if (L <= 8) return 8;
    if (L <= 16) return 16;
    return 32;
}

int64_t pscl_decode_grid(const pscl_decode_params& P) {
    if (P.long_mode) return pscl_long_grid(P.grid_cap > 0 && P.grid_cap < P.B ? P.grid_cap : P.B, P.L);
    const int per_wg = pscl_decode_wpg(P) * (32 / pscl_decode_lmax(P.L));
    int64_t g = (P.B + per_wg - 1) / per_wg;
    const int64_t cmax = P.ref && !P.cpart ? PSCL_COUNT_GRID : (1 << 20);
    const int64_t cap = P.grid_cap > 0 && P.grid_cap < cmax ? P.grid_cap : cmax;
    return g < 1 ? 1 : (g > cap ? cap : g);
}

void pscl_decode_layout(pscl_decode_params& P, int hist) {
    const int lmax = pscl_decode_lmax(P.L);
    P.long_mode = P.N > PSCL_FAST_N ? 1 : 0;
    if (P.long_mode) {
        P.fast = 0;
        P.wg_fixed_bytes = P.wave_bytes = P.a_bytes = 0;
        P.long_block_bytes = pscl_long_block_bytes(P.N, P.L, P.K, hist);
        return;
    }
    const int F = 32 / lmax;
    P.fast = (P.N == 128 && P.L <= 8) ? 1 : 0;
    P.wg_fixed_bytes = (P.apx ? 0 : PSCL_EXP_TABLE_WORDS * 8) + (P.fast && PSCL_EPI_LDS ? P.epi_words * 8 : 0);
    if (P.fast) P.wg_fixed_bytes = (P.wg_fixed_bytes + 255) & ~255;
    if (P.fast) {
        P.a_bytes = F * pscl_fast128_fstride(P.L, P.rm_E != 0) * 8;
        const int wb = P.a_bytes + (hist ? F * P.K * P.L * 9 : 0);
        P.wave_bytes = (wb + 15) & ~15;
    } else {
        const int fstride = P.N + (P.N >= 8 ? P.L * (P.N / 2 - 2) : 0);
        P.a_bytes = F * fstride * 8;
        const int wb = P.a_bytes + 64 + (hist ? F * (P.K * P.L * 8 + P.N * P.L) : 0);
        P.wave_bytes = (wb + 15) & ~15;
    }
}

static bool lane_long128(const pscl_decode_params& P) {
    return P.N == 128 && !P.long_mode && P.apx && !pscl_screening_available(P) && pscl_lane_long_available(P);
}

int pscl_lane_long128_available(const pscl_decode_params& P) { return lane_long128(P) ? 1 : 0; }

hipError_t pscl_launch_decode(const pscl_decode_params& P, int hist, hipStream_t s) {
    if (P.f32 && (hist || P.long_mode || !P.fast || !pscl_f32_decode_available(P))) return hipErrorInvalidValue;
    if (P.long_mode) {
        if (!hist && P.apx) return pscl_launch_lane_long(P, s);
        return pscl_launch_long(P, hist, s);
    }
    if (!hist && pscl_lane_available(P)) {
        const int fw = pscl_lane_frames_per_wg(P.L);
        const int64_t g = (P.B + fw - 1) / fw;
        int64_t cap = P.ref && !P.cpart ? PSCL_LANE_COUNT_GRID : (1 << 20);
        if (P.grid_cap > 0 && P.grid_cap < cap) cap = P.grid_cap;
        return P.f32 ? pscl_launch_lane_f32(P, g < 1 ? 1 : (g > cap ? cap : g), s)
                     : pscl_launch_lane(P, g < 1 ? 1 : (g > cap ? cap : g), s);
    }
    if (P.f32 && (P.apx || P.force || P.lane_exact)) return hipErrorInvalidValue;
    if (!hist && pscl_lane_fs_available(P)) {
        const int fw = pscl_lane_frames_per_wg(P.L);
        const int64_t g = (P.B + fw - 1) / fw;
        return pscl_launch_lane_fs(P, g < 1 ? 1 : (g > (1 << 20) ? (1 << 20) : g), s);
    }
    if (!hist && lane_long128(P)) return pscl_launch_lane_long(P, s);
    if (!hist && pscl_lane_exact_available(P)) return pscl_launch_lane_exact(P, s);
    if (pscl_decode_wpg(P) < 1) return hipErrorInvalidValue;
    const int64_t grid = pscl_decode_grid(P);
    if (P.fast) return pscl_launch_decode128(P, hist, pscl_decode_wpg(P), grid, decode_lds_bytes(P, hist), s);
    switch (pscl_decode_lmax(P.L)) {
        case 1: return launch_l<1>(P, hist, grid, s);
        case 2: return launch_l<2>(P, hist, grid, s);
        case 4: return launch_l<4>(P, hist, grid, s);
        case 8: return launch_l<8>(P, hist, grid, s);
        case 16: return launch_l<16>(P, hist, grid, s);
        default: return launch_l<32>(P, hist, grid, s);
    }
}

int pscl_decode_lds(const pscl_decode_params& P, int hist) { return decode_lds_bytes(P, hist); }

int64_t pscl_decode_count_slots(const pscl_decode_params& P0, int hist) {
    if (!P0.ref || P0.out_by_row || hist) return 0;
    pscl_decode_params P = P0;
    P.cpart = reinterpret_cast<int32_t*>(16);
    if (P.long_mode) return P.apx && pscl_lane_long_available(P) ? pscl_lane_long_grid(P) : 0;
    if (pscl_lane_available(P)) {
        const int fw = pscl_lane_frames_per_wg(P.L);
        const int64_t g = (P.B + fw - 1) / fw;
        return g < 1 ? 1 : (g > (1 << 20) ? (1 << 20) : g);
    }
    if (lane_long128(P)) return pscl_lane_long_grid(P);
    if (pscl_lane_exact_available(P)) return pscl_lane_exact_grid(P);
    if (!P.fast || pscl_decode_wpg(P) < 1) return 0;
    return pscl_decode_grid(P) * pscl_decode_wpg(P);
}

namespace {
__global__ void __launch_bounds__(256) count_reduce_kernel(int4* __restrict__ part, int64_t n, int64_t* counters) {
    __shared__ long long acc[4][4];
    long long a = 0, b = 0, c = 0, d = 0;
    for (int64_t i = (int64_t)blockIdx.x * 256 + threadIdx.x; i < n; i += (int64_t)gridDim.x * 256) {
        const int4 v = part[i];
        a += v.x;
        b += v.y;
        c += v.z;
        d += v.w;
        if (v.x | v.y | v.z | v.w) part[i] = make_int4(0, 0, 0, 0);
    }
#pragma unroll
    for (int sft = 32; sft >= 1; sft >>= 1) {
        a += __shfl_xor(a, sft);
        b += __shfl_xor(b, sft);
        c += __shfl_xor(c, sft);
        d += __shfl_xor(d, sft);
    }
    const int wave = threadIdx.x >> 6;
    if ((threadIdx.x & 63) == 0) {
        acc[wave][0] = a;
        acc[wave][1] = b;
        acc[wave][2] = c;
        acc[wave][3] = d;
    }
    __syncthreads();
    if (threadIdx.x < 4) {
        const long long t = acc[0][threadIdx.x] + acc[1][threadIdx.x] + acc[2][threadIdx.x] + acc[3][threadIdx.x];
        static constexpr int idx[4] = {PSCL_CNT_FRAME_ERR, PSCL_CNT_BIT_ERR, PSCL_CNT_PAYLOAD_ERR, PSCL_CNT_PAYLOAD_BIT};
        if (t) atomicAdd(reinterpret_cast<unsigned long long*>(counters) + idx[threadIdx.x], (unsigned long long)t);
    }
}
}

hipError_t pscl_launch_count_reduce(int32_t* cpart, int64_t slots, int64_t* counters, hipStream_t s) {
    if (slots <= 0) return hipSuccess;
    int64_t g = (slots + 2047) / 2048;
    if (g > 256) g = 256;
    hipLaunchKernelGGL(count_reduce_kernel, dim3((unsigned)g), dim3(256), 0, s, reinterpret_cast<int4*>(cpart), slots,
                       counters);
    return hipGetLastError();
}

__global__ void __launch_bounds__(256) channel_long_kernel(const pscl_channel_params P) {
    const int wave = threadIdx.x >> 6, lane = threadIdx.x & 63;
    const uint32_t k0 = (uint32_t)P.seed, k1 = (uint32_t)(P.seed >> 32) ^ (P.stream_id * 0x85EBCA6Bu);
    const int E = P.rm_E ? P.rm_E : P.N;
    const int kp = P.k_payload, W = P.W, NW = P.N >> 6;
    const int nb = (P.K + 7) >> 3, nbp = (kp + 7) >> 3;
    for (int64_t idx = (int64_t)blockIdx.x * 4 + wave; idx < P.B; idx += (int64_t)gridDim.x * 4) {
        const uint64_t fr = (uint64_t)(P.frame0 + idx);
        uint64_t m = 0;
        if (lane < W) {
            const u32x4 rb = philox4x32(u32x4{(uint32_t)fr, (uint32_t)(fr >> 32), 0xffffffffu - (uint32_t)(lane >> 1), 0u},
                                        k0, k1);
            m = (lane & 1) ? (((uint64_t)rb.w << 32) | rb.z) : (((uint64_t)rb.y << 32) | rb.x);
            const int nbits = kp - 64 * lane;
            m = nbits >= 64 ? m : (nbits > 0 ? (m & ((1ULL << nbits) - 1)) : 0ULL);
        }
        uint32_t rem = 0;
        if (lane < W)
            for (int t = 0; t < 8; ++t) {
                const int k = 8 * lane + t;
                if (k < nbp) rem ^= P.crctab[k * 256 + (uint32_t)((m >> (8 * t)) & 255u)];
            }
        for (int sft = 1; sft < 64; sft <<= 1) rem ^= (uint32_t)__shfl_xor((int)rem, sft);
        if (P.crc_deg) {
            const int w0 = kp >> 6, o = kp & 63;
            if (lane == w0) m |= (uint64_t)rem << o;
            if (lane == w0 + 1 && o + P.crc_deg > 64) m |= (uint64_t)rem >> (64 - o);
        }
        uint64_t x = 0;
        for (int k = 0; k < nb; ++k) {
            const uint64_t mw = pscl::shfl_u64(m, k >> 3);
            const uint32_t v = (uint32_t)((mw >> (8 * (k & 7))) & 255u);
            if (lane < NW) x ^= P.xtab[((size_t)k * 256 + v) * NW + lane];
        }
        if (P.msg && lane < W) P.msg[idx * W + lane] = m;
        double* row = P.llr + idx * E;
        for (int q = 0; q * 128 < E; ++q) {
            const u32x4 rn = philox4x32(u32x4{(uint32_t)fr, (uint32_t)(fr >> 32), (uint32_t)(lane + 64 * q), 0u}, k0, k1);
            double z[2];
            bm_pair(((uint64_t)rn.y << 32) | rn.x, ((uint64_t)rn.w << 32) | rn.z, z[0], z[1]);
#pragma unroll
            for (int h = 0; h < 2; ++h) {
                const int p = lane + 64 * h + 128 * q;
                const int pos = p < E ? (P.rm_E ? P.rm_order[p % P.N] : p) : 0;
                const uint64_t xw = pscl::shfl_u64(x, pos >> 6);
                if (p < E) {
                    const double sym = ((xw >> (pos & 63)) & 1) ? -1.0 : 1.0;
                    row[p] = (sym + P.sigma * z[h]) * P.llr_scale;
                }
            }
        }
    }
}

__global__ void __launch_bounds__(256) uncoded_kernel(const pscl_channel_params P, int64_t* counters) {
    __shared__ long long part[4][2];
    const int wave = threadIdx.x >> 6, lane = threadIdx.x & 63;
    const uint32_t k0 = (uint32_t)P.seed, k1 = (uint32_t)(P.seed >> 32) ^ (P.stream_id * 0x85EBCA6Bu);
    const int kp = P.k_payload;
    const int64_t idx = (int64_t)blockIdx.x * blockDim.x + threadIdx.x;
    int ferr = 0, berr = 0;
    if (idx < P.B) {
        const uint64_t fr = (uint64_t)(P.frame0 + idx);
        u32x4 rb = philox4x32(u32x4{(uint32_t)fr, (uint32_t)(fr >> 32), 0xffffffffu, 0u}, k0, k1);
        uint64_t r0 = ((uint64_t)rb.y << 32) | rb.x, r1 = ((uint64_t)rb.w << 32) | rb.z;
        for (int c = 0; 2 * c < kp; ++c) {
            if (c && (c & 63) == 0) {
                rb = philox4x32(u32x4{(uint32_t)fr, (uint32_t)(fr >> 32), 0xffffffffu - (uint32_t)(c >> 6), 0u}, k0, k1);
                r0 = ((uint64_t)rb.y << 32) | rb.x;
                r1 = ((uint64_t)rb.w << 32) | rb.z;
            }
            const u32x4 rn = philox4x32(u32x4{(uint32_t)fr, (uint32_t)(fr >> 32), 0x40000000u + (uint32_t)c, 0u}, k0, k1);
            double z[2];
            bm_pair(((uint64_t)rn.y << 32) | rn.x, ((uint64_t)rn.w << 32) | rn.z, z[0], z[1]);
#pragma unroll
            for (int h = 0; h < 2; ++h) {
                const int q = 2 * c + h;
                if (q < kp) {
                    const int bit = (int)((((q & 127) < 64 ? r0 : r1) >> (q & 63)) & 1ULL);
                    const double y = (bit ? -1.0 : 1.0) + P.sigma * z[h];
                    berr += (y < 0.0 ? 1 : 0) != bit;
                }
            }
        }
        ferr = berr ? 1 : 0;
    }
    ferr = pscl::wave_sum(ferr);
    berr = pscl::wave_sum(berr);
    if (lane == 0) {
        part[wave][0] = ferr;
        part[wave][1] = berr;
    }
    __syncthreads();
    if (threadIdx.x < 2) {
        long long t = 0;
        for (int w = 0; w < 4; ++w) t += part[w][threadIdx.x];
        unsigned long long* C = reinterpret_cast<unsigned long long*>(counters);
        if (t) atomicAdd(C + (threadIdx.x == 0 ? PSCL_CNT_FRAME_ERR : PSCL_CNT_BIT_ERR), (unsigned long long)t);
        if (threadIdx.x == 0 && blockIdx.x == 0) atomicAdd(C + PSCL_CNT_FRAMES, (unsigned long long)P.B);
    }
}

hipError_t pscl_launch_uncoded(const pscl_channel_params& P, int64_t* counters, hipStream_t s) {
    hipLaunchKernelGGL(uncoded_kernel, dim3((unsigned)((P.B + 255) / 256)), dim3(256), 0, s, P, counters);
    return hipGetLastError();
}

__global__ void __launch_bounds__(256) softplus_tails_kernel(const double* v, int64_t n, const uint64_t* exp_table,
                                                              double* exact, double* apx) {
    __shared__ uint64_t T[PSCL_EXP_TABLE_WORDS];
    for (int i = threadIdx.x; i < PSCL_EXP_TABLE_WORDS; i += blockDim.x) T[i] = exp_table[i];
    __syncthreads();
    for (int64_t i = (int64_t)blockIdx.x * blockDim.x + threadIdx.x; i < n; i += (int64_t)gridDim.x * blockDim.x) {
        const double x = v[i];
        exact[i] = pscl_softplus_tail_bf(x, T);
        apx[i] = PSCL_TAIL_ABS ? pscl_softplus_tail_abs(x) : pscl_softplus_tail_scr(x);
    }
}

__global__ void __launch_bounds__(256) tail_abs_scan_kernel(uint32_t lo, uint32_t hi, const uint64_t* exp_table,
                                                             unsigned long long* out, int bits) {
    __shared__ uint64_t T[PSCL_EXP_TABLE_WORDS];
    for (int i = threadIdx.x; i < PSCL_EXP_TABLE_WORDS; i += blockDim.x) T[i] = exp_table[i];
    __syncthreads();
    unsigned long long best = 0, key = 0;
    const uint64_t stride = (uint64_t)gridDim.x * blockDim.x;
    for (uint64_t i = (uint64_t)lo + (uint64_t)blockIdx.x * blockDim.x + threadIdx.x; i <= hi; i += stride) {
        const float x32 = __uint_as_float((uint32_t)i);
        const double ex = bits ? pscl_softplus_tail_bf((double)x32 * PSCL_LOGE2, T) / PSCL_LOGE2
                               : pscl_softplus_tail_bf((double)x32, T);
        const double ap = bits ? (double)pscl_tail2_f32(x32) : (double)pscl_tail_abs_f32(x32);
        const unsigned long long eb = (unsigned long long)pscl_asu64(fabs(ap - ex));
        if (eb > best) {
            best = eb;
            key = ((eb >> 32) << 32) | (uint32_t)i;
        }
    }
#pragma unroll
    for (int s = 32; s >= 1; s >>= 1) {
        const unsigned long long ob = __shfl_xor(best, s), ok = __shfl_xor(key, s);
        best = ob > best ? ob : best;
        key = ok > key ? ok : key;
    }
    if ((threadIdx.x & 63) == 0) {
        atomicMax(out, best);
        atomicMax(out + 1, key);
    }
}

hipError_t pscl_launch_tail_abs_scan(uint32_t lo, uint32_t hi, const uint64_t* exp_table, unsigned long long* out,
// ... 29 lines not shown
```

Before: 598.0 million.

## Prefetch next frame's channel LLRs in lane kernel and drop per-call count memset

In the lane SCL kernel, the next grid-stride frame's channel LLRs are now loaded into registers partway through the current frame's decode (after phase 113), so global-load latency overlaps with compute. The pipelined path also keeps a two-word ambiguity counter that the count-reduce kernel publishes and clears, which removes a hipMemsetAsync per call. A persistent-grid cap knob (scr_grid, default off) plus introspection APIs are added. The prefetch costs extra VGPRs, which may reduce occupancy.

```diff
diff --git a/include/polar_scl.h b/include/polar_scl.h
--- a/include/polar_scl.h
+++ b/include/polar_scl.h
@@ -141,6 +141,7 @@
 int pscl_set_screening(pscl_handle* h, int enable);
 
 int pscl_screening_count(pscl_handle* h, int64_t* count);
+int pscl_screening_list(pscl_handle* h, int64_t* list, int64_t cap, int64_t* count);
 
 int pscl_set_pipelined(pscl_handle* h, int enable);
 int pscl_join(pscl_handle* h);
@@ -163,7 +164,8 @@
 #define PSCL_TUNE_DL_WARM_APX 16
 #define PSCL_TUNE_DL_TAIL 17
 #define PSCL_TUNE_ADAPT_GRID 18
-#define PSCL_TUNE_COUNT 19
+#define PSCL_TUNE_SCR_GRID 19
+#define PSCL_TUNE_COUNT 20
 int pscl_set_tuning(pscl_handle* h, int knob, int64_t value);
 
 int pscl_softplus_tails_device(pscl_handle* h, const double* d_v, int64_t n, double* d_exact, double* d_apx);
@@ -192,6 +194,12 @@
 
 int pscl_launch_info(pscl_handle* h, int64_t B, int* waves_per_wg, int64_t* grid, int* lds_bytes);
 
+int pscl_screen_launch_info(pscl_handle* h, int64_t B, int f32, int64_t* grid, int64_t* resident, int64_t* count_slots);
+
+int64_t pscl_screen_grid_rule(int64_t groups, int64_t resident, int64_t knob);
+
+int64_t pscl_lane_walk(int64_t B, int64_t grid, int F, int32_t* visits);
+
 #ifdef __cplusplus
 }
 #endif
diff --git a/polar_code_amd/_native.py b/polar_code_amd/_native.py
--- a/polar_code_amd/_native.py
+++ b/polar_code_amd/_native.py
@@ -42,10 +42,11 @@
     "pscl_retry_device", "pscl_adaptive_dlscl_device", "pscl_simulate_adaptive_dl", "pscl_simulate_adaptive_dl_device",
     "pscl_f32_available", "pscl_decode_device_f32", "pscl_sc_device_f32", "pscl_escalate_device_f32",
     "pscl_adaptive_async_device_f32",
+    "pscl_screen_launch_info", "pscl_screen_grid_rule", "pscl_lane_walk", "pscl_screening_list",
 )
 
 TUNE = {"dl_screen": 1, "dl_chunks": 2, "dl_split": 3, "side_priority": 4, "post_grid": 5, "retry_wpg": 6, "dl_lane": 7, "dl_screen_min": 8, "dl_retry_lane": 9, "post_pairs": 10, "dl_streams": 11, "tx_fused": 12,
-        "dl_fused_post": 13, "post_epw": 14, "lane_exact": 15, "dl_warm_apx": 16, "dl_tail": 17, "adapt_grid": 18}
+        "dl_fused_post": 13, "post_epw": 14, "lane_exact": 15, "dl_warm_apx": 16, "dl_tail": 17, "adapt_grid": 18, "scr_grid": 19}
 
 _vp, _i32, _i64, _u64, _dbl = C.c_void_p, C.c_int32, C.c_int64, C.c_uint64, C.c_double
 
@@ -93,6 +94,7 @@
         "pscl_abi_version": (C.c_int, []),
         "pscl_build_hash": (C.c_char_p, []),
         "pscl_screening_count": (C.c_int, [_vp, P(_i64)]),
+        "pscl_screening_list": (C.c_int, [_vp, _vp, _i64, P(_i64)]),
         "pscl_set_pipelined": (C.c_int, [_vp, C.c_int]),
         "pscl_join": (C.c_int, [_vp]),
         "pscl_softplus_tails_device": (C.c_int, [_vp, _vp, _i64, _vp, _vp]),
@@ -146,6 +148,9 @@
         "pscl_set_screening": (C.c_int, [_vp, C.c_int]),
         "pscl_timing_read": (C.c_int, [_vp, P(_i64), P(_dbl)]),
         "pscl_launch_info": (C.c_int, [_vp, _i64, P(C.c_int), P(_i64), P(C.c_int)]),
+        "pscl_screen_launch_info": (C.c_int, [_vp, _i64, C.c_int, P(_i64), P(_i64), P(_i64)]),
+        "pscl_screen_grid_rule": (_i64, [_i64, _i64, _i64]),
+        "pscl_lane_walk": (_i64, [_i64, _i64, C.c_int, _vp]),
         "pscl_set_rate_match": (C.c_int, [_vp, C.c_int]),
         "pscl_set_beta": (C.c_int, [_vp, _vp]),
         "pscl_path_llrs_device": (C.c_int, [_vp, _vp, _i64, _vp, _vp]),
@@ -580,6 +585,11 @@
         check(lib().pscl_screening_count(self._h, C.byref(n)))
         return int(n.value)
 
+    def screening_list(self, cap: int) -> np.ndarray:
+        out, n = np.empty(max(int(cap), 1), np.int64), _i64()
+        check(lib().pscl_screening_list(self._h, out.ctypes.data, int(cap), C.byref(n)))
+        return out[:min(int(n.value), int(cap))]
+
     def softplus_tails(self, v: np.ndarray):
         v = np.ascontiguousarray(v, dtype=np.float64).ravel()
         with DeviceArena(self) as mem:
@@ -644,6 +654,11 @@
         check(lib().pscl_path_stats(self._h, C.byref(a), C.byref(b), C.byref(c), C.byref(d), C.byref(x)))
         return {"fused_post_rounds": int(a.value), "post_rounds": int(b.value), "fused_tx_blocks": int(c.value),
                 "post_epw4_launches": int(d.value), "lane_exact_launches": int(x.value)}
+
+    def screen_launch_info(self, B: int, f32: bool = False) -> dict:
+        g, r, c = _i64(), _i64(), _i64()
+        check(lib().pscl_screen_launch_info(self._h, int(B), 1 if f32 else 0, C.byref(g), C.byref(r), C.byref(c)))
+        return {"grid": int(g.value), "resident": int(r.value), "count_slots": int(c.value)}
 
     def launch_info(self, B: int):
         w, g, lds = C.c_int(), _i64(), C.c_int()
@@ -722,6 +737,16 @@
 _CACHE_LOCK = threading.Lock()
 
 
+def screen_grid_rule(groups: int, resident: int, knob: int) -> int:
+    return int(lib().pscl_screen_grid_rule(int(groups), int(resident), int(knob)))
+
+
+def lane_walk(B: int, grid: int, F: int):
+    visits = np.zeros(int(B), np.int32)
+    bad = int(lib().pscl_lane_walk(int(B), int(grid), int(F), visits.ctypes.data))
+    return visits, bad
+
+
 def get_decoder(N: int, info_set, L: int, crc=None, device: int = 0, E: int = 0, slot: int = 0) -> Decoder:
     info = np.asarray(info_set).astype(np.int64).ravel()
     cpu = isinstance(device, str) and device == "cpu"
diff --git a/polar_code_amd/csrc/capi.cpp b/polar_code_amd/csrc/capi.cpp
--- a/polar_code_amd/csrc/capi.cpp
+++ b/polar_code_amd/csrc/capi.cpp
@@ -135,7 +135,10 @@
     bool screen = true;
     bool screened = false;
     int screened_slot = 36;
+    int screened_list = -1;
+    int screened_word = 0;
     bool pipelined = false;
+    bool cur_clean[2] = {false, false};
     hipStream_t pipe_stream = nullptr;
     hipEvent_t ev_pscr[2] = {nullptr, nullptr}, ev_px[2] = {nullptr, nullptr};
     bool px_pending[2] = {false, false};
@@ -161,6 +164,8 @@
     hipEvent_t ev_adc[2] = {nullptr, nullptr}, ev_ad[2] = {nullptr, nullptr};
     bool ad_pending[2] = {false, false};
     int ad_par = 0;
+    int64_t scr_resident[2] = {0, 0};
+    int scr_res_E[2] = {-1, -1};
     int64_t n_regrow = 0;
     int64_t n_ad_screened = 0, n_ad_exact = 0, n_ad_waits = 0;
 };
@@ -301,6 +306,31 @@
     return PSCL_OK;
 }
 
+#ifndef PSCL_SCR_GRID_DEFAULT
+#define PSCL_SCR_GRID_DEFAULT 0
+#endif
+int screen_grid_cap(pscl_handle* h, const pscl_decode_params& S, bool rows32, int64_t* cap, int64_t* resident = nullptr) {
+    *cap = 0;
+    if (resident) *resident = 0;
+    const int64_t knob = h->tune[PSCL_TUNE_SCR_GRID] ? h->tune[PSCL_TUNE_SCR_GRID] : PSCL_SCR_GRID_DEFAULT;
+    if (!pscl_lane_available(S) || S.tx || pscl_rowlist(S) || S.grid_cap > 0) return PSCL_OK;
+    const int t = rows32 ? 1 : 0;
+    if ((knob == 1 || resident) && h->scr_res_E[t] != h->rm_E) {
+        hipDeviceProp_t prop;
+        HIP_TRY(hipGetDeviceProperties(&prop, h->device));
+        const int per_cu = rows32 ? pscl_lane_resident_blocks_f32(S) : pscl_lane_resident_blocks(S);
+        h->scr_resident[t] = (int64_t)prop.multiProcessorCount * per_cu;
+        h->scr_res_E[t] = h->rm_E;
+    }
+    if (resident) *resident = h->scr_resident[t];
+    if (!knob) return PSCL_OK;
+    const int fw = pscl_lane_frames_per_wg(S.L);
+    const int64_t groups = (S.B + fw - 1) / fw;
+    const int64_t g = pscl_screen_grid(groups, h->scr_resident[t], knob);
+    if (g < groups) *cap = g;
+    return PSCL_OK;
+}
+
 #ifndef PSCL_LANE_EXACT_DEFAULT
 #define PSCL_LANE_EXACT_DEFAULT 0
 #endif
@@ -385,14 +415,21 @@
             }
             h->pipe_par ^= 1;
         }
-        if ((rc = ensure(h, s_cnt, 4, &d_cnt))) return rc;
+        const bool two_word = pipe && !tl;
+        const size_t had_cnt = h->scratch[s_cnt].n;
+        if ((rc = ensure(h, s_cnt, two_word ? 8 : 4, &d_cnt))) return rc;
         if ((rc = ensure(h, s_list, (size_t)P.B * 8, &d_list))) return rc;
-        HIP_TRY(hipMemsetAsync(d_cnt, 0, 4, st));
+        if (!tl && (!pipe || h->scratch[s_cnt].n != had_cnt)) h->cur_clean[p] = false;
+        if (!two_word || !h->cur_clean[p]) HIP_TRY(hipMemsetAsync(d_cnt, 0, two_word ? 8 : 4, st));
+        if (two_word) h->cur_clean[p] = false;
         pscl_decode_params S = P;
         S.apx = 1;
         pscl_decode_layout(S, hist);
         S.amb_list = (int64_t*)d_list;
         S.amb_count = (int32_t*)d_cnt;
+        int64_t scap = 0;
+        if ((rc = screen_grid_cap(h, S, S.f32 != 0, &scap))) return rc;
+        if (scap > 0) S.grid_cap = scap;
         if ((rc = with_count_slots(h, S, hist, tl ? 70 + tail_par : (pipe ? 92 + p : 92), st))) return rc;
         S.tx_upart = nullptr;
         if (S.tx && S.tx_unc_counters) {
@@ -410,6 +447,8 @@
             err = pscl_launch_tx_rows(S, (const int64_t*)d_list, (const int32_t*)d_cnt, S.B, S.tx_rows, S.tx_frame0, st);
         h->screened = true;
         h->screened_slot = s_cnt;
+        h->screened_word = 0;
+        h->screened_list = s_list;
 #ifdef PSCL_APX_ABLATE
         static const bool screen_only = getenv("PSCL_DIAG_SCREEN_ONLY") && atoi(getenv("PSCL_DIAG_SCREEN_ONLY")) == 1;
 #else
@@ -442,11 +481,16 @@
                 HIP_TRY(hipStreamWaitEvent(h->pipe_stream, h->ev_pscr[p], 0));
                 if (!hist && pscl_lane_exact_available(X)) h->n_lane_exact++;
                 err = pscl_launch_decode(X, hist, h->pipe_stream);
-                if (err == hipSuccess && S.cpart)
-                    err = pscl_launch_count_reduce(S.cpart, pscl_decode_count_slots(S, hist), S.counters, h->pipe_stream);
+                const int64_t cslots = S.cpart ? pscl_decode_count_slots(S, hist) : 0;
+                if (err == hipSuccess && cslots > 0)
+                    err = pscl_launch_count_reduce(S.cpart, cslots, S.counters, h->pipe_stream, (int32_t*)d_cnt);
+                else if (err == hipSuccess)
+                    err = pscl_launch_publish_count((int32_t*)d_cnt, h->pipe_stream);
                 if (err != hipSuccess) return fail(PSCL_EDEVICE, "decode kernel launch: %s", hipGetErrorString(err));
                 HIP_TRY(hipEventRecord(h->ev_px[p], h->pipe_stream));
                 h->px_pending[p] = true;
+                h->cur_clean[p] = true;
+                h->screened_word = 1;
                 return PSCL_OK;
             }
             if (!hist && pscl_lane_exact_available(X)) h->n_lane_exact++;
@@ -1080,6 +1124,8 @@
             return fail(PSCL_EDEVICE, "row-list decode launch: %s", hipGetErrorString(e));
         h->screened = true;
         h->screened_slot = base;
+        h->screened_word = 0;
+        h->screened_list = -1;
         h->n_ad_screened++;
     } else {
         h->n_ad_exact++;
@@ -1189,7 +1235,7 @@
     if (!h) return fail(PSCL_EINVAL, "NULL handle");
     static const int64_t lim[PSCL_TUNE_COUNT][2] = {{0, 0}, {0, 2}, {0, 64}, {0, 2}, {0, 1}, {0, 4096}, {0, PSCL_MAX_WAVES_PER_WG}, {0, 2},
                                                     {0, (int64_t)1 << 30}, {0, 2}, {0, 32}, {0, 3}, {0, 2}, {0, 2}, {0, 4}, {0, 3}, {0, 2}, {0, 1},
-                                                    {0, (int64_t)1 << 20}};
+                                                    {0, (int64_t)1 << 20}, {-1, (int64_t)1 << 20}};
     if (knob < 1 || knob >= PSCL_TUNE_COUNT) return fail(PSCL_EINVAL, "unknown tuning knob %d", knob);
     if (value < lim[knob][0] || value > lim[knob][1] || (knob == PSCL_TUNE_POST_GRID && value && value < 16))
         return fail(PSCL_EINVAL, "tuning knob %d: value %lld out of range", knob, (long long)value);
@@ -2446,9 +2492,22 @@
     int rc = enter(h);
     if (rc) return rc;
     int32_t c = 0;
-    HIP_TRY(hipMemcpyAsync(&c, h->scratch[h->screened_slot].p, 4, hipMemcpyDeviceToHost, h->stream));
+    HIP_TRY(hipMemcpyAsync(&c, (const int32_t*)h->scratch[h->screened_slot].p + h->screened_word, 4, hipMemcpyDeviceToHost,
+                           h->stream));
     HIP_TRY(hipStreamSynchronize(h->stream));
     *count = c;
+    return PSCL_OK;
+}
+
+int pscl_screening_list(pscl_handle* h, int64_t* list, int64_t cap, int64_t* count) {
+    if (!h || !count || cap < 0 || (cap > 0 && !list)) return fail(PSCL_EINVAL, "bad arguments");
+    int rc = pscl_screening_count(h, count);
+    if (rc) return rc;
+    if (*count == 0 || cap == 0) return PSCL_OK;
+    if (h->screened_list < 0 || !h->scratch[h->screened_list].p) return fail(PSCL_EUNSUP, "the last decode kept no deferred-frame list");
+    const int64_t n = *count < cap ? *count : cap;
+    HIP_TRY(hipMemcpyAsync(list, h->scratch[h->screened_list].p, (size_t)n * 8, hipMemcpyDeviceToHost, h->stream));
+    HIP_TRY(hipStreamSynchronize(h->stream));
     return PSCL_OK;
 }
 
@@ -2561,4 +2620,52 @@
     return PSCL_OK;
 }
 
-}
+int pscl_screen_launch_info(pscl_handle* h, int64_t B, int f32, int64_t* grid, int64_t* resident, int64_t* count_slots) {
+    if (!h) return fail(PSCL_EINVAL, "NULL handle");
+    if (B < 1) return fail(PSCL_EINVAL, "B must be >= 1");
+    int rc = set_device(h);
+    if (rc) return rc;
+    pscl_decode_params S;
+    fill_decode_params(h, S, 0);
+    S.B = B;
+    S.apx = 1;
+    pscl_decode_layout(S, 0);
+    int64_t cap = 0, res = 0;
+    if ((rc = screen_grid_cap(h, S, f32 != 0, &cap, &res))) return rc;
+    if (cap > 0) S.grid_cap = cap;
+    S.ref = reinterpret_cast<const uint64_t*>(16);
+    const int64_t slots = pscl_decode_count_slots(S, 0);
+    if (grid) *grid = pscl_lane_available(S) ? slots : pscl_decode_grid(S);
+    if (resident) *resident = res;
+    if (count_slots) *count_slots = slots;
+    return PSCL_OK;
+}
+
+int64_t pscl_screen_grid_rule(int64_t groups, int64_t resident, int64_t knob) { return pscl_screen_grid(groups, resident, knob); }
+
+int64_t pscl_lane_walk(int64_t B, int64_t grid, int F, int32_t* visits) {
+    if (B < 1 || grid < 1 || F < 1 || !visits) return -1;
+    int64_t bad = 0;
+    const int64_t stride = grid * F;
+    auto rows_ok = [&](int64_t g0) {
+        for (int fl = 0; fl < F; ++fl) {
+            const int64_t r = pscl_lane_row(g0, fl, B);
+            if (r < 0 || r >= B) ++bad;
+        }
+    };
+    for (int64_t w = 0; w < grid; ++w) {
+        bool loaded = w * F < B;
+        if (loaded) rows_ok(w * F);
+        for (int64_t f0 = w * F; f0 < B; f0 += stride) {
+            if (!loaded) ++bad;
+            for (int fl = 0; fl < F; ++fl)
+                if (f0 + fl < B) visits[f0 + fl] += 1;
+            loaded = pscl_lane_has_next(f0, stride, B);
+            if (loaded) rows_ok(f0 + stride);
+        }
+        if (loaded) ++bad;
+    }
+    return bad;
+}
+
+}
diff --git a/polar_code_amd/csrc/scl128_lane.hip b/polar_code_amd/csrc/scl128_lane.hip
--- a/polar_code_amd/csrc/scl128_lane.hip
+++ b/polar_code_amd/csrc/scl128_lane.hip
@@ -66,6 +66,10 @@
 #endif
 #ifndef PSCL_LANE_GSPLIT
 #define PSCL_LANE_GSPLIT 1
+#endif
+
+#ifndef PSCL_LANE_PREFETCH
+#define PSCL_LANE_PREFETCH 1
 #endif
 
 __device__ __forceinline__ void tx_frame_words(const pscl_decode_params& P, uint64_t fr, uint64_t (&m)[2],
@@ -101,6 +105,19 @@
 #ifndef PSCL_TX_WAVES
 #define PSCL_TX_WAVES 3
 #endif
+template <int CODE, int G>
+__device__ __forceinline__ void lane_fetch_rows(const double* llr, const int32_t* rm_src, int rm_E, double* v, int64_t g0, int fl,
+                                                int p, int64_t Bn) {
+    const lane_llr_t* row = reinterpret_cast<const lane_llr_t*>(llr) + pscl_lane_row(g0, fl, Bn) * (CODE == 2 ? (int64_t)rm_E : (int64_t)kN);
+#pragma unroll
+    for (int k = 0; k < 16 / G; ++k)
+#pragma unroll
+        for (int m = 0; m < 8; ++m) {
+            const int i = p + G * k + 16 * m;
+            v[8 * k + m] = CODE == 2 ? nr_stage(row, rm_src[i], rm_E, kN) : (double)row[i];
+        }
+}
+
 template <int LMAX, int CODE, bool FS = false, bool TXF = false, bool FP = false, bool EX = false, bool RL = false>
 __global__ void __launch_bounds__(64, TXF ? (LMAX == 8 ? PSCL_TX_WAVES : 2)
                                            : (FS && !FP && !EX && LMAX == 8) ? PSCL_FS_WAVES : PSCL_LANE_WAVES_PER_EU)
@@ -159,6 +176,11 @@
     } else if constexpr (RL) {
         Bn = *P.d_count < P.B ? (int64_t)*P.d_count : P.B;
     }
+    constexpr bool PF = PLAIN && !RL && (G == 8 || PSCL_LANE_CREG4) && PSCL_LANE_PREFETCH;
+    double cn[PF ? 8 * EPL : 1];
+    if constexpr (PF) {
+        if ((int64_t)blockIdx.x * F < Bn) lane_fetch_rows<CODE, G>(P.llr, P.rm_src, P.rm_E, cn, (int64_t)blockIdx.x * F, fl, p, Bn);
+    }
     for (int64_t f0 = (int64_t)blockIdx.x * F; f0 < Bn; f0 += (int64_t)gridDim.x * F) {
         const int64_t fi = f0 + fl;
         const bool fvalid = fi < Bn;
@@ -213,7 +235,12 @@
                                                                     : chan_at(p + G * k + 16 * m);
             }
         };
-        load_chan();
+        if constexpr (PF) {
+#pragma unroll
+            for (int m = 0; m < 8 * EPL; ++m) c[m] = BITS ? cn[m] * PSCL_LOG2E_F64 : cn[m];
+        } else {
+            load_chan();
+        }
         uint32_t ah[4 * EPL];
 #pragma unroll
         for (int m = 0; m < 4 * EPL; ++m) {
@@ -700,6 +727,19 @@
                 case 6: seg(integral_constant<int, 6>{}); [[fallthrough]];
                 default: seg(integral_constant<int, 7>{});
             }
+        } else if constexpr (PF) {
+            static_for<113>([&](auto PC) { phase(PC); });
+            using karg_t = const __attribute__((address_space(4))) pscl_decode_params;
+            karg_t* Q = (karg_t*)__builtin_amdgcn_kernarg_segment_ptr();
+            asm volatile("" : "+s"(Q));
+            const int64_t gstride = (int64_t)gridDim.x * F, Bq = Q->B;
+            if (pscl_lane_has_next(f0, gstride, Bq)) {
+                lane_fetch_rows<CODE, G>(Q->llr, Q->rm_src, Q->rm_E, cn, f0 + gstride, fl, p, Bq);
+            } else {
+#pragma unroll
+                for (int m = 0; m < 8 * EPL; ++m) asm volatile("" : "=v"(cn[m]));
+            }
+            static_for<kN - 113>([&](auto PC) { phase(std::integral_constant<int, 113 + decltype(PC)::value>{}); });
         } else {
             static_for<kN>([&](auto PC) { phase(PC); });
         }
@@ -1094,6 +1134,23 @@
     return hipGetLastError();
 }
 #elif defined(PSCL_LANE_F32_UNIT)
+int pscl_lane_resident_blocks_f32(const pscl_decode_params& P) {
+    const int lds8 = LaneLayout<8>::F * LaneLayout<8>::FSTRIDE * 8 + PSCL_LANE_LDS_PAD,
+              lds4 = LaneLayout<4>::F * LaneLayout<4>::FSTRIDE * 8 + PSCL_LANE_LDS_PAD;
+    if (P.tx || pscl_rowlist(P)) return 0;
+    int n = 0;
+    hipError_t e = hipErrorInvalidValue;
+    if (P.L == 8 && !P.rm_E)
+        e = hipOccupancyMaxActiveBlocksPerMultiprocessor(&n, scl_lane_kernel<8, 1>, 64, lds8);
+    else if (P.L == 8)
+        e = hipOccupancyMaxActiveBlocksPerMultiprocessor(&n, scl_lane_kernel<8, 2>, 64, lds8);
+    else if (P.L == 4 && !P.rm_E)
+        e = hipOccupancyMaxActiveBlocksPerMultiprocessor(&n, scl_lane_kernel<4, 1>, 64, lds4);
+    else if (P.L == 4)
+        e = hipOccupancyMaxActiveBlocksPerMultiprocessor(&n, scl_lane_kernel<4, 2>, 64, lds4);
+    return e == hipSuccess && n > 0 ? n : 0;
+}
+
 hipError_t pscl_launch_lane_f32(const pscl_decode_params& P, int64_t grid, hipStream_t s) {
     const int lds8 = LaneLayout<8>::F * LaneLayout<8>::FSTRIDE * 8 + PSCL_LANE_LDS_PAD,
               lds4 = LaneLayout<4>::F * LaneLayout<4>::FSTRIDE * 8 + PSCL_LANE_LDS_PAD;
@@ -1112,6 +1169,23 @@
     return hipGetLastError();
 }
 #else
+
+int pscl_lane_resident_blocks(const pscl_decode_params& P) {
+    const int lds8 = LaneLayout<8>::F * LaneLayout<8>::FSTRIDE * 8 + PSCL_LANE_LDS_PAD,
+              lds4 = LaneLayout<4>::F * LaneLayout<4>::FSTRIDE * 8 + PSCL_LANE_LDS_PAD;
+    if (P.tx || pscl_rowlist(P)) return 0;
+    int n = 0;
+    hipError_t e = hipErrorInvalidValue;
+    if (P.L == 8 && !P.rm_E)
+        e = hipOccupancyMaxActiveBlocksPerMultiprocessor(&n, scl_lane_kernel<8, 1>, 64, lds8);
+    else if (P.L == 8)
+        e = hipOccupancyMaxActiveBlocksPerMultiprocessor(&n, scl_lane_kernel<8, 2>, 64, lds8);
+    else if (P.L == 4 && !P.rm_E)
+        e = hipOccupancyMaxActiveBlocksPerMultiprocessor(&n, scl_lane_kernel<4, 1>, 64, lds4);
+    else if (P.L == 4)
+        e = hipOccupancyMaxActiveBlocksPerMultiprocessor(&n, scl_lane_kernel<4, 2>, 64, lds4);
+    return e == hipSuccess && n > 0 ? n : 0;
+}
 
 int pscl_lane_frames_per_wg(int L) { return 64 / L; }
 
diff --git a/polar_code_amd/csrc/scl_kernels.h b/polar_code_amd/csrc/scl_kernels.h
--- a/polar_code_amd/csrc/scl_kernels.h
+++ b/polar_code_amd/csrc/scl_kernels.h
@@ -274,6 +274,22 @@
 hipError_t pscl_launch_lane_f32(const pscl_decode_params& P, int64_t grid, hipStream_t s);
 hipError_t pscl_launch_lane_rowlist_f32(const pscl_decode_params& P, int64_t grid, hipStream_t s);
 int pscl_f32_decode_available(const pscl_decode_params& P);
+#if defined(__HIPCC__)
+#define PSCL_WALK_FN __host__ __device__ inline
+#else
+#define PSCL_WALK_FN inline
+#endif
+PSCL_WALK_FN bool pscl_lane_has_next(int64_t f0, int64_t stride, int64_t Bn) { return f0 + stride < Bn; }
+PSCL_WALK_FN int64_t pscl_lane_row(int64_t f0, int fl, int64_t Bn) { return f0 + fl < Bn ? f0 + fl : f0; }
+inline int64_t pscl_screen_grid(int64_t groups, int64_t resident, int64_t knob) {
+    if (groups < 1) groups = 1;
+    if (knob == -1) return 1;
+    if (knob > 1) return knob < groups ? knob : groups;
+    if (knob == 1 && resident > 0 && groups >= 4 * resident) return resident;
+    return groups;
+}
+int pscl_lane_resident_blocks(const pscl_decode_params& P);
+int pscl_lane_resident_blocks_f32(const pscl_decode_params& P);
 #ifndef PSCL_LANE_COUNT_GRID
 #define PSCL_LANE_COUNT_GRID 32768
 #endif
@@ -281,7 +297,9 @@
 #define PSCL_COUNT_GRID 8192
 #endif
 int64_t pscl_decode_count_slots(const pscl_decode_params& P, int hist);
-hipError_t pscl_launch_count_reduce(int32_t* cpart, int64_t slots, int64_t* counters, hipStream_t s);
+hipError_t pscl_launch_count_reduce(int32_t* cpart, int64_t slots, int64_t* counters, hipStream_t s,
+                                    int32_t* publish = nullptr);
+hipError_t pscl_launch_publish_count(int32_t* cnt2, hipStream_t s);
 #ifndef PSCL_DL_LANE_DEFAULT
 #define PSCL_DL_LANE_DEFAULT 1
 #endif
diff --git a/polar_code_amd/csrc/scl_kernels.hip b/polar_code_amd/csrc/scl_kernels.hip
--- a/polar_code_amd/csrc/scl_kernels.hip
+++ b/polar_code_amd/csrc/scl_kernels.hip
@@ -536,20 +536,22 @@
 
 int pscl_lane_long128_available(const pscl_decode_params& P) { return lane_long128(P) ? 1 : 0; }
 
+static int64_t lane_grid(const pscl_decode_params& P) {
+    const int fw = pscl_lane_frames_per_wg(P.L);
+    const int64_t g = (P.B + fw - 1) / fw;
+    int64_t cap = P.ref && !P.cpart ? PSCL_LANE_COUNT_GRID : (1 << 20);
+    if (P.grid_cap > 0 && P.grid_cap < cap) cap = P.grid_cap;
+    return g < 1 ? 1 : (g > cap ? cap : g);
+}
+
 hipError_t pscl_launch_decode(const pscl_decode_params& P, int hist, hipStream_t s) {
     if (P.f32 && (hist || P.long_mode || !P.fast || !pscl_f32_decode_available(P))) return hipErrorInvalidValue;
     if (P.long_mode) {
         if (!hist && P.apx) return pscl_launch_lane_long(P, s);
         return pscl_launch_long(P, hist, s);
     }
-    if (!hist && pscl_lane_available(P)) {
-        const int fw = pscl_lane_frames_per_wg(P.L);
-        const int64_t g = (P.B + fw - 1) / fw;
-        int64_t cap = P.ref && !P.cpart ? PSCL_LANE_COUNT_GRID : (1 << 20);
-        if (P.grid_cap > 0 && P.grid_cap < cap) cap = P.grid_cap;
-        return P.f32 ? pscl_launch_lane_f32(P, g < 1 ? 1 : (g > cap ? cap : g), s)
-                     : pscl_launch_lane(P, g < 1 ? 1 : (g > cap ? cap : g), s);
-    }
+    if (!hist && pscl_lane_available(P))
+        return P.f32 ? pscl_launch_lane_f32(P, lane_grid(P), s) : pscl_launch_lane(P, lane_grid(P), s);
     if (P.f32 && (P.apx || P.force || P.lane_exact)) return hipErrorInvalidValue;
     if (!hist && pscl_lane_fs_available(P)) {
         const int fw = pscl_lane_frames_per_wg(P.L);
@@ -578,11 +580,7 @@
     pscl_decode_params P = P0;
     P.cpart = reinterpret_cast<int32_t*>(16);
     if (P.long_mode) return P.apx && pscl_lane_long_available(P) ? pscl_lane_long_grid(P) : 0;
-    if (pscl_lane_available(P)) {
-        const int fw = pscl_lane_frames_per_wg(P.L);
-        const int64_t g = (P.B + fw - 1) / fw;
-        return g < 1 ? 1 : (g > (1 << 20) ? (1 << 20) : g);
-    }
+    if (pscl_lane_available(P)) return lane_grid(P);
     if (lane_long128(P)) return pscl_lane_long_grid(P);
     if (pscl_lane_exact_available(P)) return pscl_lane_exact_grid(P);
     if (!P.fast || pscl_decode_wpg(P) < 1) return 0;
@@ -590,8 +588,19 @@
 }
 
 namespace {
-__global__ void __launch_bounds__(256) count_reduce_kernel(int4* __restrict__ part, int64_t n, int64_t* counters) {
+__device__ __forceinline__ void publish_count(int32_t* cnt2) {
+    cnt2[1] = cnt2[0];
+    cnt2[0] = 0;
+}
+
+__global__ void publish_count_kernel(int32_t* cnt2) {
+    if (blockIdx.x == 0 && threadIdx.x == 0) publish_count(cnt2);
+}
+
+__global__ void __launch_bounds__(256) count_reduce_kernel(int4* __restrict__ part, int64_t n, int64_t* counters,
+                                                           int32_t* publish) {
     __shared__ long long acc[4][4];
+    if (publish && blockIdx.x == 0 && threadIdx.x == 0) publish_count(publish);
     long long a = 0, b = 0, c = 0, d = 0;
     for (int64_t i = (int64_t)blockIdx.x * 256 + threadIdx.x; i < n; i += (int64_t)gridDim.x * 256) {
         const int4 v = part[i];
@@ -624,12 +633,17 @@
 }
 }
 
-hipError_t pscl_launch_count_reduce(int32_t* cpart, int64_t slots, int64_t* counters, hipStream_t s) {
-    if (slots <= 0) return hipSuccess;
+hipError_t pscl_launch_publish_count(int32_t* cnt2, hipStream_t s) {
+    hipLaunchKernelGGL(publish_count_kernel, dim3(1), dim3(64), 0, s, cnt2);
+    return hipGetLastError();
+}
+
+hipError_t pscl_launch_count_reduce(int32_t* cpart, int64_t slots, int64_t* counters, hipStream_t s, int32_t* publish) {
+    if (slots <= 0) return publish ? pscl_launch_publish_count(publish, s) : hipSuccess;
     int64_t g = (slots + 2047) / 2048;
     if (g > 256) g = 256;
     hipLaunchKernelGGL(count_reduce_kernel, dim3((unsigned)g), dim3(256), 0, s, reinterpret_cast<int4*>(cpart), slots,
-                       counters);
+                       counters, publish);
     return hipGetLastError();
 }
 
```

New measurement: 601.5 million, median of 6. No clear change (+0.6%).
